# ziniuwan/maed

Hardware: AMD Instinct MI355X
Metric: video-clips/sec (BxT frames) train step (higher is better)
Workload: dtype bf16

## Files before the change

### include/maed_hip.h

```cpp
#ifndef MAED_HIP_H
#define MAED_HIP_H

#include <stddef.h>
#include <stdint.h>

#ifdef __cplusplus
extern "C" {
#endif

typedef enum { MAED_F32 = 0, MAED_BF16 = 1,
               MAED_F32X3 = 2, MAED_F32X6 = 3,
               MAED_F32X1 = 4 } maed_dtype;

typedef enum {
    MAED_OK = 0,
    MAED_ERR_ARG = -1,
    MAED_ERR_SHAPE = -2,
    MAED_ERR_ALIGN = -3,
    MAED_ERR_LAUNCH = -4,
    MAED_ERR_UNSUPPORTED = -5
} maed_status;

typedef enum {
    MAED_EPI_STORE = 0,
    MAED_EPI_GELU = 1,
    MAED_EPI_RESID_F32 = 2,
    MAED_EPI_MUL_DGELU = 3,
    MAED_EPI_ATOMIC_F32 = 4,
    MAED_EPI_STORE_F32 = 5,
    MAED_EPI_TANH = 6,
    MAED_EPI_ADD = 7
} maed_epilogue;

typedef enum { MAED_IMPL_AUTO = 0, MAED_IMPL_VALU = 1, MAED_IMPL_MFMA = 2,
               MAED_IMPL_MFMA_GLDS1 = 3, MAED_IMPL_MFMA_GLDS2 = 4,
               MAED_IMPL_MFMA_LONG = 5,
               MAED_IMPL_MFMA_256 = 6,
               MAED_IMPL_X1 = 9,
               MAED_IMPL_MFMA_SK = 10,
               MAED_IMPL_X3 = 7, MAED_IMPL_X6 = 8
} maed_impl;

const char* maed_last_error(void);
int maed_version(void);

typedef enum {
    MAED_OPT_F32_MATMUL = 0,
    MAED_OPT_SIDE_STREAM = 1,
    MAED_OPT_TN_TARGET_WGS = 2,
    MAED_OPT_ABLATE = 3,
    MAED_OPT_GN_BWD_ONEPASS = 4,
    MAED_OPT_F32_BWD_X1 = 5,
    MAED_OPT_ST_FUSED = 6,
    MAED_OPT_CONV3X3_ROWS_WGS = 7,
    MAED_OPT_STEM_WGRAD_WGS = 8,
    MAED_OPT_LBS_FRAMES = 9,
    MAED_OPT_TN_DMA = 10,
    MAED_OPT_X3_PLANES = 11,
    MAED_OPT_X3_PLANES_LN = 12,
    MAED_OPT_SK = 13,
    MAED_OPT_SK_GRID = 14,
    MAED_OPT_TN_SK = 15,
    MAED_OPT_CONV3X3_NARROW_WGS = 16,
    MAED_OPT_CONV3X3_FRAME = 17,
    MAED_OPT_COUNT
} maed_option;
int maed_init(int device);
int maed_device_faults(void);
int maed_device_faults_clear(void);
int maed_set_option(int key, int value);
int maed_get_option(int key);

int maed_layernorm_fwd(const float* x, int64_t x_row_stride, const float* gamma, const float* beta,
                       void* y, int dtype, float* mean, float* rstd,
                       int64_t rows, int C, float eps, void* stream);
int maed_layernorm_bwd(const void* dy, int dtype, const float* x, int64_t x_row_stride,
                       const float* gamma, const float* mean, const float* rstd,
                       const float* dres_in, float* dx_out, void* dx_twin, float* dgamma, float* dbeta,
                       int64_t rows, int C, void* stream);

int maed_gemm_nt(const void* A, int64_t lda, const void* B, int64_t ldb,
                 int64_t M, int64_t N, int64_t K, int dtype, int epilogue,
                 const float* bias, void* out, int64_t ldo, void* out2,
                 const void* aux, int64_t ldaux, int splitk, int impl, void* stream);

int maed_gemm_nt_planes(const void* a_hi, const void* a_lo, int64_t lda, const void* b_hi, const void* b_lo, int64_t ldb, int64_t M, int64_t N, int64_t K,
                        int epilogue, const float* bias, void* out, int64_t ldo, void* out2_bf16, const void* aux, int64_t ldaux, void* out_hi, void* out_lo,
                        int variant, void* stream);
int maed_split_planes(const float* x, void* hi, void* lo, int64_t n, void* stream);

int maed_gemm_tn_wgrad(const void* Y, int64_t ldy, const void* X, int64_t ldx, int64_t M, int N, int K,
                       float* dW, int64_t ldw, float* dbias, int dtype, void* stream);

int maed_transpose_cast(const void* in, int in_dtype, int64_t ldi, int64_t M, int64_t N,
                        void* out_t, int64_t ldt, void* out_c, int64_t ldc, float* colsum,
                        int dtype, void* stream);

int maed_attn_spatial_fwd(const void* qkv, void* o, float* lse, int F, int P, int H, float scale,
                          int dtype, int impl, void* stream);
int maed_attn_spatial_bwd(const void* qkv, const void* o, const void* d_o, const float* lse,
                          void* dqkv, int accumulate, int F, int P, int H, float scale,
                          int dtype, int impl, void* stream);

int maed_attn_temporal_fwd(const void* qkv, void* o, float* lse, int F, int P, int H, int T,
                           float scale, int dtype, void* stream);
int maed_attn_temporal_bwd(const void* qkv, const void* o, const void* d_o, const float* lse,
                           void* dqkv, int accumulate, int F, int P, int H, int T, float scale,
                           int dtype, void* stream);

int maed_st_colmean(const void* x_s, const void* x_t, void* means, float* ws, int F, int P, int C, int dtype, void* stream);
int maed_st_mix_fwd(const void* x_s, const void* x_t, const float* logits, void* mix,
                    int F, int P, int C, int dtype, void* stream);
int maed_st_mix_bwd_reduce(const void* dmix, const void* x_s, const void* x_t, const float* logits,
                           void* dlogits, float* ws, int F, int P, int C, int dtype, void* stream);
int maed_st_mix_bwd_apply(const void* dmix, const float* logits, const void* dmeans, void* dx_s, void* dx_t,
                          int F, int P, int C, int dtype, void* stream);
int maed_st_fused_supported(int P, int C, int dtype);
int maed_st_fused_fwd(const void* x_s, const void* x_t, const void* w_ts, const float* b_ts, void* means, float* logits, void* mix,
                      uint32_t* sync, float* ex, int F, int P, int C, int dtype, void* stream);
int maed_st_fused_bwd(const void* dmix, const void* x_s, const void* x_t, const float* logits, const void* wt_ts, void* dlogits, void* dx_s,
                      void* dx_t, uint32_t* sync, float* ex, int F, int P, int C, int dtype, void* stream);


int maed_embed_add_fwd(const void* patch, int dtype, const float* cls, const float* pos, const float* temp,
                       float* tokens, int F, int P, int C, int T, void* stream);
int maed_embed_add_bwd(const float* dtokens, void* dpatch, int dtype, float* dpos, float* dtemp, int F, int P, int C, int T, void* stream);

int maed_dropout(const float* x, float* y, int64_t n, float p, uint64_t seed, void* stream);
typedef struct { float lr, bias_corr1, bias_corr2, reserved0; uint64_t seed; uint64_t reserved1; } maed_train_state;
int maed_dropout_dev(const float* x, float* y, int64_t n, float p, const maed_train_state* state, uint64_t call_id, void* stream);
int maed_tanh_bwd(const float* dy, const void* y, void* dx, int64_t n, int dtype, void* stream);

typedef struct {
    int F, P, C, H, T, hidden;
    int dtype;
    int impl;
    float eps;
} maed_block_dims;

typedef struct {
    const float *ln1_g, *ln1_b, *ln2_g, *ln2_b;
    const void *w_qkv, *w_ts, *w_proj, *w_fc1, *w_fc2;
    const float *b_qkv, *b_ts, *b_proj, *b_fc1, *b_fc2;
    const void *wt_qkv, *wt_ts, *wt_proj, *wt_fc1, *wt_fc2;
} maed_block_params;

typedef struct {
    float *ln1_g, *ln1_b, *ln2_g, *ln2_b;
    float *w_qkv, *w_ts, *w_proj, *w_fc1, *w_fc2;
    float *b_qkv, *b_ts, *b_proj, *b_fc1, *b_fc2;
} maed_block_grads;

size_t maed_ste_block_saved_bytes(const maed_block_dims* d);
size_t maed_ste_block_scratch_bytes(const maed_block_dims* d);
int maed_ste_block_fwd(const maed_block_dims* d, const maed_block_params* p, const float* x_in,
                       float* x_out, void* saved, void* stream);
size_t maed_ste_block_twin_work_bytes(const maed_block_dims* d);
int maed_ste_block_fwd_twin(const maed_block_dims* d, const maed_block_params* p, const float* x_in, float* x_out, void* saved_bf16, void* work_f32, int work_slot,
                            void* stream);
int maed_ste_block_twin_join(void* stream);
int maed_ste_block_infer(const maed_block_dims* d, const maed_block_params* p, const float* x_in,
                         float* x_out, void* work, void* stream);
int maed_ste_block_bwd(const maed_block_dims* d, const maed_block_params* p, const maed_block_grads* g,
                       const float* x_in, const float* dx_out, float* dx_in, void* saved, void* scratch,
                       const void* dx_out_twin, void* dx_in_twin, void* stream);

int maed_stream_fence(void* from_stream, void* to_stream);

int maed_prof_enable(int on);
int maed_prof_ntags(void);
int maed_prof_collect(double* ms_total_host, int* count_host);
int maed_prof_flops(double* flops_host);
int maed_prof_records(int tag, double* us_host, double* flops_host, double* bytes_host, int cap);

int maed_ktd_chain_fwd(const float* base, const float* w_anc, float* pose, int F, void* stream);

int maed_rot6d_pose_fwd(const float* pose6d, float* rotmat, float* angle_axis, int64_t n_joints, void* stream);

typedef struct {
    const float* v_template;
    const float* shapedirs;
    const float* posedirs;
    const float* J_template;
    const float* J_shapedirs;
    const float* lbs_weights;
    const int32_t* parents;
} maed_smpl_params;
int maed_smpl_lbs_fwd(const maed_smpl_params* sp, const float* betas, const float* rotmat,
                      float* verts, float* joints24, float* scratch_A, float* v_posed, int F, void* stream);
int maed_joint_regress_fwd(const float* Jreg, int J, const float* verts, float* out, int F, void* stream);
int maed_joint_regress_csr_fwd(const int32_t* rowptr, const int32_t* cols, const float* vals, int J, const float* verts, float* out, int F, void* stream);
int maed_smpl_joints_project_fwd(const float* joints24, const float* verts, const int64_t* extra_vertex_ids,
                                 const float* extra9, const int64_t* joint_map, const float* cam,
                                 const float* joints_override, int Jo, float* kp3d, float* kp2d, int F, void* stream);


int maed_smpl_joints_project_bwd(const float* kp3d, const float* cam, const int64_t* joint_map, const float* d_kp3d,
                                 const float* d_kp2d, const float* d_cam_in, int64_t cam_in_stride, float* d_joints24,
                                 float* d_extra21, float* d_extra9, float* d_cam, int F, void* stream);
int maed_smpl_skin_bwd(const maed_smpl_params* sp, const float* A, const float* v_posed, const float* d_verts,
                       const float* d_extra21, const int64_t* extra_vertex_ids, const float* d_extra9, const float* Jextra,
                       float* d_vposed, float* dA, int F, void* stream);
int maed_smpl_skin_bwd_sparse(const maed_smpl_params* sp, const float* A, const float* v_posed, const int32_t* active, int n_active,
                              const float* d_extra21, const int64_t* extra_vertex_ids, const float* d_extra9, const float* Jextra,
                              float* d_vposed_active, float* dA, int F, void* stream);
int maed_smpl_chain_bwd(const maed_smpl_params* sp, const float* betas, const float* rotmat, const float* dA,
                        const float* d_joints24, const float* dpf_dbeta, const float* d_rotmat_in, const float* d_betas_in,
                        int64_t betas_in_stride, float* d_rotmat, float* d_betas, int F, void* stream);
int maed_rot6d_pose_bwd(const float* pose6d, const float* d_rotmat, const float* d_aa, int64_t aa_stride,
                        float* d_pose6d, int64_t n_joints, void* stream);
int maed_ktd_chain_bwd(const float* pose, const float* w_anc, const float* d_pose, const float* d_shape, const float* d_cam,
                       float* d_out, int64_t ld_out, float* d_w_anc, float* d_b_feat, int F, void* stream);
#define MAED_KTD_W_ANC 3420
typedef struct { const float* w[26]; const float* b[26]; float* gw[26]; float* gb[26]; } maed_ktd_ptrs;
int maed_ktd_pack(const maed_ktd_ptrs* t, int hidden, float* w_feat, float* b_feat, float* w_anc, void* stream);
int maed_ktd_unpack_add(const maed_ktd_ptrs* t, int hidden, const float* d_w_feat, const float* d_b_feat, const float* d_w_anc, void* stream);

typedef struct { float w_kp2d, w_kp3d, w_pose, w_shape, w_norm; } maed_loss_weights;
int maed_loss_fwd_bwd(const float* pred_kp2d, const float* gt_kp2d, int M2, const float* pred_kp3d, const float* gt_kp3d,
                      const float* pred_theta, const float* gt_theta, const uint8_t* w_smpl, int M3,
                      const maed_loss_weights* w, float* losses, float* d_kp2d, float* d_kp3d, float* d_theta,
                      double* partials, void* stream);

int maed_loss_accl_fwd_bwd(const float* pred_kp3d, const float* gt_kp3d, int N, int T, float weight, double* loss, float* d_kp3d, void* stream);

typedef struct {
    const float* w;
    float* gw;
    const void* gout;
    int64_t dst_off;
    int64_t dst_t_off;
    int32_t O, I, KHW, fstart;
    int32_t gout_f32;
    int32_t pad_;
} maed_ws_conv;
int maed_weight_std_fwd(const void* conv_table, int n_convs, int n_filters, void* out, int dtype, float* stats, float eps, int transpose_tiles, void* stream);
int maed_weight_std_bwd(const void* conv_table, int n_convs, int n_filters, int dtype, const float* stats, float eps, void* stream);
int maed_groupnorm_fwd(const void* x, const void* residual, const float* gamma, const float* beta, void* y, double* sums,
                       uint8_t* relu_mask, int N, int HW, int C, float eps, int relu, int dtype, int sums_zeroed, void* stream);
int maed_groupnorm_fwd_twin(const void* x, const void* residual, const float* gamma, const float* beta, void* y, double* sums,
                            uint8_t* relu_mask, int N, int HW, int C, float eps, int relu, int sums_zeroed, void* twin_x, void* twin_y, void* stream);
#define MAED_GN_SYNC_WORDS 80
int maed_groupnorm_bwd(const void* x, const uint8_t* relu_mask, const void* dy, const double* sums, const float* gamma, const float* beta,
                       void* dx, void* dres, float* dgamma, float* dbeta, float* ab_scratch, int N, int HW, int C, float eps,
                       int relu, int dtype, int ab_zeroed, uint32_t* frame_sync, void* aux_stream, void* stream);
typedef struct { const float* ab; float* dgamma; float* dbeta; int N; int C; } maed_gn_affine_item;
int maed_gn_affine_grad_batch(const maed_gn_affine_item* items, int count, void* stream);

int maed_maxpool3s2_same_fwd(const void* x, void* y, uint8_t* idx, int N, int H, int W, int C, int dtype, void* stream);
int maed_maxpool3s2_same_bwd(const void* dy, const uint8_t* idx, void* dx, int N, int H, int W, int C, int dtype, void* stream);

int maed_stem_input(const float* x, void* y, int N, int C, int H, int W, int pad_top, int pad_bottom, int pad_left, int pad_right, int c_stride, int dtype,
                    void* stream);

int maed_conv3x3_wgrad_rows64_scratch_floats(int F, int H, int W, int Cin, int Cout);
int maed_conv3x3_wgrad_rows64(const void* dy, const void* x, float* dW, void* scratch, int F, int H, int W, int dtype, void* stream);

int maed_stem7x7s2_supported(int H, int W);
int maed_stem7x7s2_fwd(const void* xp, const void* w, void* wimg, void* y, double* gn_sums, int F, int H, int W, int dtype, void* stream);
int maed_stem7x7s2_wgrad_scratch_floats(int F, int H, int W);
int maed_stem7x7s2_wgrad(const void* dy, const void* xp, float* dW, void* scratch, int F, int H, int W, int dtype, void* stream);

int maed_subsample2_fwd(const void* x, void* y, int F, int H, int W, int C, int dtype, void* stream);
int maed_subsample2_bwd(const void* g, void* dx, int F, int H, int W, int C, int dtype, void* stream);

typedef struct { const float* src; void* dst_c; void* dst_t; int32_t rows, cols, tile0, tiles_n; } maed_wt_entry;
int maed_weight_refresh(const void* table, int n_entries, int n_tiles, int dtype, void* stream);

int maed_adam_step(float* p, const float* g, float* m, float* v, void* shadow_bf16, int64_t n,
                   float lr, float beta1, float beta2, float eps, float weight_decay,
                   float bias_corr1, float bias_corr2, float gscale, void* stream);
int maed_adam_step_dev(float* p, const float* g, float* m, float* v, void* shadow_bf16, int64_t n, const maed_train_state* state,
                       float beta1, float beta2, float eps, float weight_decay, float gscale, void* stream);

#define MAED_COMM_ID_BYTES 128
int maed_comm_load(const char* librccl_path);
int maed_comm_unique_id(void* id128);
int maed_comm_init(int rank, int world, const void* unique_id);
int maed_comm_allreduce_async(void* buf, size_t n, int dtype, void* compute_stream);
int maed_comm_wait(void* compute_stream);
int maed_comm_world(void);
int maed_comm_destroy(void);

int maed_conv3x3_fwd(const void* x, const void* w_taps, const void* zero_page, void* y, int F, int H, int W, int Cin, int Cout,
                     int stride, int pad_top, int pad_left, int Ho, int Wo, const void* add, int w_layout, int dtype, double* gn_sums,
                     void* stream);

int maed_conv1x1_fwd(const void* x, int64_t ldx, const void* w, int64_t ldw, int64_t M, int Cout, int Cin, void* y, int64_t ldy, int hw,
                     double* gn_sums, int dtype, void* stream);

int maed_conv3x3_s2_dgrad(const void* dy, const void* wt_image, const void* zero_page, void* dx, int F, int H, int W, int Cin, int Cout,
                          int pad_top, int pad_left, int Ho, int Wo, int dtype, void* stream);
int maed_conv3x3_s2_tables(void* tapmask, int* rowtab, int F, int H, int W, int pad_top, int pad_left, int Ho, int Wo, void* stream);
int maed_conv3x3_s2_wgrad(const void* dy, const void* x, const void* tapmask, const int* rowtab, const void* zero_page, float* dW, int F, int H, int W,
                          int Cin, int Cout, int Ho, int Wo, int dtype, void* stream);
int maed_conv3x3_tapmask(void* tapmask, int F, int H, int W, void* stream);
int maed_conv3x3_wgrad(const void* dy, const void* x, const void* tapmask, const void* zero_page, float* dW, int F, int H, int W, int Cin,
                       int Cout, int dtype, void* stream);

int maed_eval_pose_errors(const float* pred, const float* target, int N, int J, float* mpjpe, float* pa_mpjpe,
                          float* pred_centred, float* target_centred, void* stream);
int maed_similarity_transform(const float* S1, const float* S2, int N, int J, float* S1_hat, void* stream);
int maed_eval_accel(const float* joints, const float* joints_gt, int N, int J, float* out, void* stream);
int maed_eval_vertex_error(const float* pred_verts, const float* target_verts, int N, int V, float* out, void* stream);

size_t maed_clip_preprocess_workspace(int F, int H, int W);
int maed_clip_preprocess(const uint8_t* src, int64_t src_bytes, const int32_t* frame_i, const float* frame_minv, const int32_t* clip_i,
                         const float* clip_f, int F, int N, int H, int W, const float* norm_host, int has_contrast, int form, float* out,
                         void* workspace, size_t workspace_bytes, void* stream);

#ifdef __cplusplus
}
#endif
#endif
```

### maed_amd/_lib.py

```python
import ctypes as C
import os

HERE = os.path.dirname(os.path.abspath(__file__))
LIB_PATH = os.environ.get("MAED_HIP_LIB") or os.path.join(HERE, "libmaed_hip.so")

F32, BF16 = 0, 1
F32X3, F32X6, F32X1 = 2, 3, 4
EPI_STORE, EPI_GELU, EPI_RESID_F32, EPI_MUL_DGELU, EPI_ATOMIC_F32, EPI_STORE_F32, EPI_TANH, EPI_ADD = range(8)
IMPL_AUTO, IMPL_VALU, IMPL_MFMA = 0, 1, 2
IMPL_MFMA_256 = 6
IMPL_MFMA_LONG = 5
IMPL_MFMA_SK = 10
IMPL_X3, IMPL_X6, IMPL_X1 = 7, 8, 9
(OPT_F32_MATMUL, OPT_SIDE_STREAM, OPT_TN_TARGET_WGS, OPT_ABLATE, OPT_GN_BWD_ONEPASS, OPT_F32_BWD_X1, OPT_ST_FUSED, OPT_CONV3X3_ROWS_WGS, OPT_STEM_WGRAD_WGS,
 OPT_LBS_FRAMES, OPT_TN_DMA, OPT_X3_PLANES, OPT_X3_PLANES_LN, OPT_SK, OPT_SK_GRID, OPT_TN_SK, OPT_CONV3X3_NARROW_WGS, OPT_CONV3X3_FRAME) = range(18)

vp, i64, i32, f32 = C.c_void_p, C.c_int64, C.c_int, C.c_float


class GnAffineItem(C.Structure):
    _fields_ = [("ab", C.c_void_p), ("dgamma", C.c_void_p), ("dbeta", C.c_void_p), ("N", C.c_int), ("C", C.c_int)]


class BlockDims(C.Structure):
    _fields_ = [("F", i32), ("P", i32), ("C", i32), ("H", i32), ("T", i32), ("hidden", i32),
                ("dtype", i32), ("impl", i32), ("eps", f32)]


_PARAM_FIELDS = ["ln1_g", "ln1_b", "ln2_g", "ln2_b", "w_qkv", "w_ts", "w_proj", "w_fc1", "w_fc2",
                 "b_qkv", "b_ts", "b_proj", "b_fc1", "b_fc2", "wt_qkv", "wt_ts", "wt_proj", "wt_fc1", "wt_fc2"]
_GRAD_FIELDS = _PARAM_FIELDS[:14]


class BlockParams(C.Structure):
    _fields_ = [(n, vp) for n in _PARAM_FIELDS]


class BlockGrads(C.Structure):
    _fields_ = [(n, vp) for n in _GRAD_FIELDS]


class SmplParams(C.Structure):
    _fields_ = [(n, vp) for n in ["v_template", "shapedirs", "posedirs", "J_template", "J_shapedirs", "lbs_weights", "parents"]]


class KtdPtrs(C.Structure):
    _fields_ = [("w", vp * 26), ("b", vp * 26), ("gw", vp * 26), ("gb", vp * 26)]


class LossWeights(C.Structure):
    _fields_ = [(n, f32) for n in ["w_kp2d", "w_kp3d", "w_pose", "w_shape", "w_norm"]]


KTD_W_ANC = 3420

SIGNATURES = {
    "maed_last_error": (C.c_char_p, []),
    "maed_version": (i32, []),
    "maed_init": (i32, [i32]),
    "maed_device_faults": (i32, []),
    "maed_device_faults_clear": (i32, []),
    "maed_set_option": (i32, [i32, i32]),
    "maed_get_option": (i32, [i32]),
    "maed_layernorm_fwd": (i32, [vp, i64, vp, vp, vp, i32, vp, vp, i64, i32, f32, vp]),
    "maed_layernorm_bwd": (i32, [vp, i32, vp, i64, vp, vp, vp, vp, vp, vp, vp, vp, i64, i32, vp]),
    "maed_gemm_tn_wgrad": (i32, [vp, i64, vp, i64, i64, i32, i32, vp, i64, vp, i32, vp]),
    "maed_gemm_nt": (i32, [vp, i64, vp, i64, i64, i64, i64, i32, i32, vp, vp, i64, vp, vp, i64, i32, i32, vp]),
    "maed_transpose_cast": (i32, [vp, i32, i64, i64, i64, vp, i64, vp, i64, vp, i32, vp]),
    "maed_attn_spatial_fwd": (i32, [vp, vp, vp, i32, i32, i32, f32, i32, i32, vp]),
    "maed_attn_spatial_bwd": (i32, [vp, vp, vp, vp, vp, i32, i32, i32, i32, f32, i32, i32, vp]),
    "maed_attn_temporal_fwd": (i32, [vp, vp, vp, i32, i32, i32, i32, f32, i32, vp]),
    "maed_attn_temporal_bwd": (i32, [vp, vp, vp, vp, vp, i32, i32, i32, i32, i32, f32, i32, vp]),
    "maed_st_colmean": (i32, [vp, vp, vp, vp, i32, i32, i32, i32, vp]),
    "maed_st_mix_fwd": (i32, [vp, vp, vp, vp, i32, i32, i32, i32, vp]),
    "maed_st_mix_bwd_reduce": (i32, [vp, vp, vp, vp, vp, vp, i32, i32, i32, i32, vp]),
    "maed_st_mix_bwd_apply": (i32, [vp, vp, vp, vp, vp, i32, i32, i32, i32, vp]),
    "maed_st_fused_supported": (i32, [i32, i32, i32]),
    "maed_st_fused_fwd": (i32, [vp, vp, vp, vp, vp, vp, vp, vp, vp, i32, i32, i32, i32, vp]),
    "maed_st_fused_bwd": (i32, [vp, vp, vp, vp, vp, vp, vp, vp, vp, vp, i32, i32, i32, i32, vp]),
    "maed_embed_add_fwd": (i32, [vp, i32, vp, vp, vp, vp, i32, i32, i32, i32, vp]),
    "maed_embed_add_bwd": (i32, [vp, vp, i32, vp, vp, i32, i32, i32, i32, vp]),
    "maed_ste_block_saved_bytes": (C.c_size_t, [C.POINTER(BlockDims)]),
    "maed_ste_block_scratch_bytes": (C.c_size_t, [C.POINTER(BlockDims)]),
    "maed_gemm_nt_planes": (i32, [vp, vp, i64, vp, vp, i64, i64, i64, i64, i32, vp, vp, i64, vp, vp, i64, vp, vp, i32, vp]),
    "maed_split_planes": (i32, [vp, vp, vp, i64, vp]),
    "maed_ste_block_twin_work_bytes": (C.c_size_t, [C.POINTER(BlockDims)]),
    "maed_ste_block_fwd_twin": (i32, [C.POINTER(BlockDims), C.POINTER(BlockParams), vp, vp, vp, vp, i32, vp]),
    "maed_ste_block_twin_join": (i32, [vp]),
    "maed_ste_block_fwd": (i32, [C.POINTER(BlockDims), C.POINTER(BlockParams), vp, vp, vp, vp]),
    "maed_ste_block_infer": (i32, [C.POINTER(BlockDims), C.POINTER(BlockParams), vp, vp, vp, vp]),
    "maed_ste_block_bwd": (i32, [C.POINTER(BlockDims), C.POINTER(BlockParams), C.POINTER(BlockGrads), vp, vp, vp, vp, vp, vp, vp, vp]),
    "maed_loss_accl_fwd_bwd": (i32, [vp, vp, i32, i32, f32, vp, vp, vp]),
    "maed_dropout": (i32, [vp, vp, i64, f32, C.c_uint64, vp]),
    "maed_dropout_dev": (i32, [vp, vp, i64, f32, vp, C.c_uint64, vp]),
    "maed_tanh_bwd": (i32, [vp, vp, vp, i64, i32, vp]),
    "maed_stream_fence": (i32, [vp, vp]),
    "maed_prof_enable": (i32, [i32]),
    "maed_prof_ntags": (i32, []),
    "maed_prof_collect": (i32, [C.POINTER(C.c_double), C.POINTER(i32)]),
    "maed_prof_flops": (i32, [C.POINTER(C.c_double)]),
    "maed_prof_records": (i32, [i32, C.POINTER(C.c_double), C.POINTER(C.c_double), C.POINTER(C.c_double), i32]),
    "maed_ktd_chain_fwd": (i32, [vp, vp, vp, i32, vp]),
    "maed_rot6d_pose_fwd": (i32, [vp, vp, vp, i64, vp]),
    "maed_smpl_lbs_fwd": (i32, [C.POINTER(SmplParams), vp, vp, vp, vp, vp, vp, i32, vp]),
    "maed_joint_regress_fwd": (i32, [vp, i32, vp, vp, i32, vp]),
    "maed_joint_regress_csr_fwd": (i32, [vp, vp, vp, i32, vp, vp, i32, vp]),
    "maed_smpl_joints_project_fwd": (i32, [vp, vp, vp, vp, vp, vp, vp, i32, vp, vp, i32, vp]),
    "maed_smpl_joints_project_bwd": (i32, [vp, vp, vp, vp, vp, vp, i64, vp, vp, vp, vp, i32, vp]),
    "maed_smpl_skin_bwd": (i32, [C.POINTER(SmplParams), vp, vp, vp, vp, vp, vp, vp, vp, vp, i32, vp]),
    "maed_smpl_skin_bwd_sparse": (i32, [C.POINTER(SmplParams), vp, vp, vp, i32, vp, vp, vp, vp, vp, vp, i32, vp]),
    "maed_smpl_chain_bwd": (i32, [C.POINTER(SmplParams), vp, vp, vp, vp, vp, vp, vp, i64, vp, vp, i32, vp]),
    "maed_rot6d_pose_bwd": (i32, [vp, vp, vp, i64, vp, i64, vp]),
    "maed_ktd_chain_bwd": (i32, [vp, vp, vp, vp, vp, vp, i64, vp, vp, i32, vp]),
    "maed_ktd_pack": (i32, [C.POINTER(KtdPtrs), i32, vp, vp, vp, vp]),
    "maed_ktd_unpack_add": (i32, [C.POINTER(KtdPtrs), i32, vp, vp, vp, vp]),
    "maed_loss_fwd_bwd": (i32, [vp, vp, i32, vp, vp, vp, vp, vp, i32, C.POINTER(LossWeights), vp, vp, vp, vp, vp, vp]),
    "maed_weight_std_fwd": (i32, [vp, i32, i32, vp, i32, vp, f32, i32, vp]),
    "maed_weight_std_bwd": (i32, [vp, i32, i32, i32, vp, f32, vp]),
    "maed_groupnorm_fwd": (i32, [vp, vp, vp, vp, vp, vp, vp, i32, i32, i32, f32, i32, i32, i32, vp]),
    "maed_groupnorm_fwd_twin": (i32, [vp, vp, vp, vp, vp, vp, vp, i32, i32, i32, f32, i32, i32, vp, vp, vp]),
    "maed_groupnorm_bwd": (i32, [vp, vp, vp, vp, vp, vp, vp, vp, vp, vp, vp, i32, i32, i32, f32, i32, i32, i32, vp, vp, vp]),
    "maed_gn_affine_grad_batch": (i32, [vp, i32, vp]),
    "maed_comm_load": (i32, [C.c_char_p]),
    "maed_comm_unique_id": (i32, [vp]),
    "maed_comm_init": (i32, [i32, i32, vp]),
    "maed_comm_allreduce_async": (i32, [vp, C.c_size_t, i32, vp]),
    "maed_comm_wait": (i32, [vp]),
    "maed_comm_world": (i32, []),
    "maed_comm_destroy": (i32, []),
    "maed_conv3x3_fwd": (i32, [vp, vp, vp, vp, i32, i32, i32, i32, i32, i32, i32, i32, i32, i32, vp, i32, i32, vp, vp]),
    "maed_conv1x1_fwd": (i32, [vp, i64, vp, i64, i64, i32, i32, vp, i64, i32, vp, i32, vp]),
    "maed_conv3x3_tapmask": (i32, [vp, i32, i32, i32, vp]),
    "maed_conv3x3_s2_dgrad": (i32, [vp, vp, vp, vp, i32, i32, i32, i32, i32, i32, i32, i32, i32, i32, vp]),
    "maed_conv3x3_s2_tables": (i32, [vp, vp, i32, i32, i32, i32, i32, i32, i32, vp]),
    "maed_conv3x3_s2_wgrad": (i32, [vp, vp, vp, vp, vp, vp, i32, i32, i32, i32, i32, i32, i32, i32, vp]),
    "maed_conv3x3_wgrad": (i32, [vp, vp, vp, vp, vp, i32, i32, i32, i32, i32, i32, vp]),
    "maed_eval_pose_errors": (i32, [vp, vp, i32, i32, vp, vp, vp, vp, vp]),
    "maed_similarity_transform": (i32, [vp, vp, i32, i32, vp, vp]),
    "maed_eval_accel": (i32, [vp, vp, i32, i32, vp, vp]),
    "maed_eval_vertex_error": (i32, [vp, vp, i32, i32, vp, vp]),
    "maed_maxpool3s2_same_fwd": (i32, [vp, vp, vp, i32, i32, i32, i32, i32, vp]),
    "maed_maxpool3s2_same_bwd": (i32, [vp, vp, vp, i32, i32, i32, i32, i32, vp]),
    "maed_stem_input": (i32, [vp, vp, i32, i32, i32, i32, i32, i32, i32, i32, i32, i32, vp]),
    "maed_conv3x3_wgrad_rows64_scratch_floats": (i32, [i32, i32, i32, i32, i32]),
    "maed_conv3x3_wgrad_rows64": (i32, [vp, vp, vp, vp, i32, i32, i32, i32, vp]),
    "maed_stem7x7s2_supported": (i32, [i32, i32]),
    "maed_stem7x7s2_fwd": (i32, [vp, vp, vp, vp, vp, i32, i32, i32, i32, vp]),
    "maed_stem7x7s2_wgrad_scratch_floats": (i32, [i32, i32, i32]),
    "maed_stem7x7s2_wgrad": (i32, [vp, vp, vp, vp, i32, i32, i32, i32, vp]),
    "maed_subsample2_fwd": (i32, [vp, vp, i32, i32, i32, i32, i32, vp]),
    "maed_subsample2_bwd": (i32, [vp, vp, i32, i32, i32, i32, i32, vp]),
    "maed_weight_refresh": (i32, [vp, i32, i32, i32, vp]),
    "maed_adam_step": (i32, [vp, vp, vp, vp, vp, i64, f32, f32, f32, f32, f32, f32, f32, f32, vp]),
    "maed_adam_step_dev": (i32, [vp, vp, vp, vp, vp, i64, vp, f32, f32, f32, f32, f32, vp]),
    "maed_clip_preprocess_workspace": (C.c_size_t, [i32, i32, i32]),
    "maed_clip_preprocess": (i32, [vp, i64, vp, vp, vp, vp, i32, i32, i32, i32, C.POINTER(f32), i32, i32, vp, vp, C.c_size_t, vp]),
}

_lib = None
_init_pending = False


class MaedHipError(RuntimeError):
    pass


def lib():
    global _lib, _init_pending
    if _lib is None:
        if not os.path.exists(LIB_PATH):
            raise MaedHipError(f"{LIB_PATH} is missing: build it with `python -m maed_amd.build` "
                               "(hipcc --offload-arch=gfx950).  maed_amd has no non-HIP fallback.")
        handle = C.CDLL(LIB_PATH)
        for name, (res, args) in SIGNATURES.items():
            fn = getattr(handle, name)
            fn.restype, fn.argtypes = res, args
        _lib = handle
        apply_options(handle)
        _init_pending = True
    if _init_pending:
        import torch
        if torch.cuda.is_available() and torch.cuda.is_initialized():
            _init_pending = False
            check(_lib.maed_init(torch.cuda.current_device()), "maed_init")
    return _lib


_OPTIONS = {
    OPT_F32_MATMUL: {"exact": 0, "0": 0, "bf16x3": 1, "1": 1, "bf16x6": 2, "2": 2}[os.environ.get("MAED_F32_MATMUL", "exact")],
    OPT_SIDE_STREAM: int(os.environ.get("MAED_WGRAD_SIDE_STREAM", "1") == "1"),
    OPT_TN_TARGET_WGS: int(os.environ.get("MAED_TN_TARGET_WGS", "0")),
    OPT_ABLATE: int(os.environ.get("MAED_GEMM_ABLATE", "0")),
    OPT_F32_BWD_X1: int(os.environ.get("MAED_F32_BWD", "") == "bf16x1"),
    OPT_ST_FUSED: int(os.environ.get("MAED_ST_FUSED", "1")),
    OPT_GN_BWD_ONEPASS: int(os.environ.get("MAED_GN_BWD_ONEPASS", "1")),
    OPT_CONV3X3_ROWS_WGS: 0 if os.environ.get("MAED_CONV3X3_WGRAD_ROWS", "1") == "0" else int(os.environ.get("MAED_CONV3X3_ROWS_WGS", "256")),
    OPT_STEM_WGRAD_WGS: int(os.environ.get("MAED_STEM_WGS", "512")),
    OPT_LBS_FRAMES: int(os.environ.get("MAED_LBS_FB", "0")),
    OPT_TN_DMA: int(os.environ.get("MAED_TN_DMA", "1")),
    OPT_X3_PLANES: int(os.environ.get("MAED_X3_PLANES", "6")),
    OPT_SK: int(os.environ.get("MAED_SK", "1")),
    OPT_SK_GRID: int(os.environ.get("MAED_SK_GRID", "0")),
    OPT_CONV3X3_FRAME: int(os.environ.get("MAED_CONV3X3_FRAME", "1")),
    OPT_CONV3X3_NARROW_WGS: int(os.environ.get("MAED_CONV3X3_NARROW_WGS", "0")),
    OPT_TN_SK: int(os.environ.get("MAED_TN_SK", "1")),
    OPT_X3_PLANES_LN: int(os.environ.get("MAED_X3_PLANES_LN", "0")),
}


def apply_options(handle):
    for k, v in _OPTIONS.items():
        if handle.maed_set_option(k, v) != 0:
            raise MaedHipError(f"maed_set_option({k}, {v}) failed")


def set_option(key, value):
    _OPTIONS[key] = int(value)
    if _lib is not None:
        check(_lib.maed_set_option(key, int(value)), "set_option")


def get_option(key):
    return _OPTIONS[key]


def check(rc, what=""):
    if rc != 0:
        msg = lib().maed_last_error().decode("utf-8", "replace")
        raise MaedHipError(f"{what or 'libmaed_hip'} failed with status {rc}: {msg}")


def device_faults():
    return 0 if _lib is None else int(_lib.maed_device_faults())


def loaded_path():
    return LIB_PATH if _lib is not None else None
```

### maed_amd/csrc/attn_long.hip

```cpp
#include "attn_mfma.cuh"

#define D HEAD_DIM

namespace {

constexpr int LT = 64;
constexpr int LVLD = LT + 4;
constexpr int WG_ROWS = 128;

__device__ __forceinline__ int long_xcd_remap(int bid, int nwg) {
    const int xcd = bid & 7, q = nwg >> 3, r = nwg & 7;
    const int base = (xcd < r) ? xcd * (q + 1) : r * (q + 1) + (xcd - r) * q;
    return base + (bid >> 3);
}

struct TileRegs { uint4 a, b; };

__device__ __forceinline__ uint4 tile_load1(const bf16* src, int64_t ld, int r0, int L, int idx) {
    int row = r0 + (idx >> 3);
    if (row > L - 1) row = L - 1;
    return *reinterpret_cast<const uint4*>(src + (int64_t)row * ld + (idx & 7) * 8);
}
__device__ __forceinline__ void tile_load(TileRegs& t, const bf16* src, int64_t ld, int r0, int L, int tid) {
    t.a = tile_load1(src, ld, r0, L, tid);
    t.b = tile_load1(src, ld, r0, L, tid + 256);
}

__device__ __forceinline__ void tile_store1(const uint4 v, unsigned short* rows, unsigned short* tr, int idx) {
    const int p = idx >> 3, c8 = (idx & 7) * 8;
    if (rows) *reinterpret_cast<uint4*>(rows + p * KLD + c8) = v;
    if (tr) {
        tr[(c8 + 0) * LVLD + p] = (unsigned short)(v.x & 0xffffu); tr[(c8 + 1) * LVLD + p] = (unsigned short)(v.x >> 16);
        tr[(c8 + 2) * LVLD + p] = (unsigned short)(v.y & 0xffffu); tr[(c8 + 3) * LVLD + p] = (unsigned short)(v.y >> 16);
        tr[(c8 + 4) * LVLD + p] = (unsigned short)(v.z & 0xffffu); tr[(c8 + 5) * LVLD + p] = (unsigned short)(v.z >> 16);
        tr[(c8 + 6) * LVLD + p] = (unsigned short)(v.w & 0xffffu); tr[(c8 + 7) * LVLD + p] = (unsigned short)(v.w >> 16);
    }
}
__device__ __forceinline__ void tile_store(const TileRegs& t, unsigned short* rows, unsigned short* tr, int tid) {
    tile_store1(t.a, rows, tr, tid);
    tile_store1(t.b, rows, tr, tid + 256);
}

__global__ __launch_bounds__(256, 4) void attn_long_fwd_mfma(const bf16* __restrict__ qkv, bf16* __restrict__ o, float* __restrict__ lse,
                                                          int L, int H, int ntile, float scale_log2e) {
    __shared__ __attribute__((aligned(16))) unsigned short Ks[LT * KLD];
    __shared__ __attribute__((aligned(16))) unsigned short Vs[LT * KLD];
    const int bid = long_xcd_remap(blockIdx.x, gridDim.x);
    const int item = bid / ntile, tile = bid - item * ntile;
    const int f = item / H, h = item - f * H, C = H * D;
    const int64_t ld = 3 * (int64_t)C;
    const bf16* base = qkv + (int64_t)f * L * ld + h * D;
    const int tid = threadIdx.x, lane = tid & 63, wave = tid >> 6, l31 = lane & 31, hi = lane >> 5;
    const int q0 = tile * WG_ROWS + wave * 32, q = q0 + l31;
    const bool active = q0 < L;
    const int qc = q < L ? q : L - 1;
    bf16x8_t qf[4];
#pragma unroll
    for (int t = 0; t < 4; ++t) qf[t] = *reinterpret_cast<const bf16x8_t*>(base + (int64_t)qc * ld + t * 16 + hi * 8);
    f32x16_t oacc[2];
#pragma unroll
    for (int r = 0; r < 16; ++r) { oacc[0][r] = 0.f; oacc[1][r] = 0.f; }
    float m = -INFINITY, l = 0.f;
    const int nkt = (L + LT - 1) / LT;
    TileRegs kreg, vreg;
    tile_load(kreg, base + C, ld, 0, L, tid);
    tile_load(vreg, base + 2 * C, ld, 0, L, tid);
    for (int kt = 0; kt < nkt; ++kt) {
        __syncthreads();
        tile_store(kreg, Ks, nullptr, tid);
        tile_store(vreg, Vs, nullptr, tid);
        __syncthreads();
        if (kt + 1 < nkt) {
            tile_load(kreg, base + C, ld, (kt + 1) * LT, L, tid);
            tile_load(vreg, base + 2 * C, ld, (kt + 1) * LT, L, tid);
        }
        if (!active) continue;
#pragma unroll
        for (int sub = 0; sub < 2; ++sub) {
            const int k0 = kt * LT + sub * 32;
            if (k0 >= L) break;
            f32x16_t s;
#pragma unroll
            for (int r = 0; r < 16; ++r) s[r] = 0.f;
            const unsigned short* kp = Ks + (sub * 32 + l31) * KLD + hi * 8;
#pragma unroll
            for (int t = 0; t < 4; ++t)
                s = __builtin_amdgcn_mfma_f32_32x32x16_bf16(*reinterpret_cast<const bf16x8_t*>(kp + t * 16), qf[t], s, 0, 0, 0);
            if (k0 + 32 > L) {
#pragma unroll
                for (int r = 0; r < 16; ++r) s[r] = (k0 + (r & 3) + 8 * (r >> 2) + 4 * hi < L) ? s[r] : -INFINITY;
            }
            float mt = s[0];
#pragma unroll
            for (int r = 1; r < 16; ++r) mt = fmaxf(mt, s[r]);
            mt = fmaxf(mt, __shfl_xor(mt, 32, 64)) * scale_log2e;
            const bool grow = mt > m + 8.0f;
            if (__any(grow)) {
                const float mn = grow ? mt : m;
                const float alpha = __builtin_amdgcn_exp2f(m - mn);
                l *= alpha;
                m = mn;
#pragma unroll
                for (int r = 0; r < 16; ++r) { oacc[0][r] *= alpha; oacc[1][r] *= alpha; }
            }
            float ps = 0.f;
#pragma unroll
            for (int r = 0; r < 16; ++r) { s[r] = __builtin_amdgcn_exp2f(fmaf(s[r], scale_log2e, -m)); ps += s[r]; }
            l += ps;
#pragma unroll
            for (int st = 0; st < 2; ++st) {
                const bf16x8_t pf = pack_frag(s, st);
#pragma unroll
                for (int et = 0; et < 2; ++et)
                    oacc[et] = __builtin_amdgcn_mfma_f32_32x32x16_bf16(lds_frag_tr_rm(Vs, sub * 32 + 16 * st, et * 32, lane), pf, oacc[et], 0, 0, 0);
            }
        }
    }
    l += __shfl_xor(l, 32, 64);
    __syncthreads();
    if (active) {
        const float inv = 1.f / l;
#pragma unroll
        for (int r = 0; r < 16; ++r) { oacc[0][r] *= inv; oacc[1][r] *= inv; }
        store_tile_lines((wave < 2 ? Ks : Vs) + (wave & 1) * 2048, o + ((int64_t)f * L + q0) * C + h * D, C, L - q0, oacc, lane, 0);
    }
    if (active && q < L) {
        if (hi == 0) lse[((int64_t)f * H + h) * L + q] = (m + log2f(l)) * 0.69314718055994530942f;
    }
}

__global__ __launch_bounds__(256, 3) void attn_long_bwd_dq_mfma(const bf16* __restrict__ qkv, const bf16* __restrict__ o, const bf16* __restrict__ d_o,
                                                             const float* __restrict__ lse, bf16* __restrict__ dqkv, int accumulate, int L, int H,
                                                             int ntile, float scale) {
    __shared__ __attribute__((aligned(16))) unsigned short Ks[LT * KLD];
    __shared__ __attribute__((aligned(16))) unsigned short Vs[LT * KLD];
    const int bid = long_xcd_remap(blockIdx.x, gridDim.x);
    const int item = bid / ntile, tile = bid - item * ntile;
    const int f = item / H, h = item - f * H, C = H * D;
    const int64_t ld = 3 * (int64_t)C;
    const bf16* base = qkv + (int64_t)f * L * ld + h * D;
    const int tid = threadIdx.x, lane = tid & 63, wave = tid >> 6, l31 = lane & 31, hi = lane >> 5;
    const int q0 = tile * WG_ROWS + wave * 32, q = q0 + l31;
    const bool active = q0 < L;
    const int qc = q < L ? q : L - 1;
    const bf16* orow = o + ((int64_t)f * L + qc) * C + h * D;
    const bf16* dorow = d_o + ((int64_t)f * L + qc) * C + h * D;
    bf16x8_t qf[4], dof[4];
    float Dq = 0.f;
#pragma unroll
    for (int t = 0; t < 4; ++t) {
        qf[t] = *reinterpret_cast<const bf16x8_t*>(base + (int64_t)qc * ld + t * 16 + hi * 8);
        dof[t] = *reinterpret_cast<const bf16x8_t*>(dorow + t * 16 + hi * 8);
        float a[8], b[8];
        ld8(dorow + t * 16 + hi * 8, a); ld8(orow + t * 16 + hi * 8, b);
#pragma unroll
        for (int j = 0; j < 8; ++j) Dq = fmaf(a[j], b[j], Dq);
    }
    Dq += __shfl_xor(Dq, 32, 64);
    const float l2e = 1.44269504088896340736f;
    const float L2 = lse[((int64_t)f * H + h) * L + qc] * l2e, sl2e = scale * l2e;
    f32x16_t dq[2];
#pragma unroll
    for (int r = 0; r < 16; ++r) { dq[0][r] = 0.f; dq[1][r] = 0.f; }
    const int nkt = (L + LT - 1) / LT;
    TileRegs kreg, vreg;
    tile_load(kreg, base + C, ld, 0, L, tid);
    tile_load(vreg, base + 2 * C, ld, 0, L, tid);
    for (int kt = 0; kt < nkt; ++kt) {
        __syncthreads();
        tile_store(kreg, Ks, nullptr, tid);
        tile_store(vreg, Vs, nullptr, tid);
        __syncthreads();
        if (kt + 1 < nkt) {
            tile_load(kreg, base + C, ld, (kt + 1) * LT, L, tid);
            tile_load(vreg, base + 2 * C, ld, (kt + 1) * LT, L, tid);
        }
        if (!active) continue;
#pragma unroll
        for (int sub = 0; sub < 2; ++sub) {
            const int k0 = kt * LT + sub * 32;
            if (k0 >= L) break;
            f32x16_t s, dp;
#pragma unroll
            for (int r = 0; r < 16; ++r) { s[r] = 0.f; dp[r] = -Dq; }
            const int off = (sub * 32 + l31) * KLD + hi * 8;
#pragma unroll
            for (int t = 0; t < 4; ++t) {
                s = __builtin_amdgcn_mfma_f32_32x32x16_bf16(*reinterpret_cast<const bf16x8_t*>(Ks + off + t * 16), qf[t], s, 0, 0, 0);
                dp = __builtin_amdgcn_mfma_f32_32x32x16_bf16(*reinterpret_cast<const bf16x8_t*>(Vs + off + t * 16), dof[t], dp, 0, 0, 0);
            }
#pragma unroll
            for (int r = 0; r < 16; ++r) s[r] = __builtin_amdgcn_exp2f(fmaf(s[r], sl2e, -L2)) * dp[r];
            if (k0 + 32 > L) {
#pragma unroll
                for (int r = 0; r < 16; ++r) s[r] = (k0 + (r & 3) + 8 * (r >> 2) + 4 * hi < L) ? s[r] : 0.f;
            }
#pragma unroll
            for (int st = 0; st < 2; ++st) {
                const bf16x8_t dsf = pack_frag(s, st);
#pragma unroll
                for (int et = 0; et < 2; ++et)
                    dq[et] = __builtin_amdgcn_mfma_f32_32x32x16_bf16(lds_frag_tr_rm(Ks, sub * 32 + 16 * st, et * 32, lane), dsf, dq[et], 0, 0, 0);
            }
        }
    }
#pragma unroll
    for (int r = 0; r < 16; ++r) { dq[0][r] *= scale; dq[1][r] *= scale; }
    __syncthreads();
    if (active) store_tile_lines((wave < 2 ? Ks : Vs) + (wave & 1) * 2048, dqkv + ((int64_t)f * L + q0) * ld + h * D, ld, L - q0, dq, lane, accumulate);
}

__global__ __launch_bounds__(256, 2) void attn_long_bwd_dkv_mfma(const bf16* __restrict__ qkv, const bf16* __restrict__ o, const bf16* __restrict__ d_o,
                                                              const float* __restrict__ lse, bf16* __restrict__ dqkv, int accumulate, int L, int H,
                                                              int ntile, float scale) {
    __shared__ __attribute__((aligned(16))) unsigned short Qs[LT * KLD];
    __shared__ __attribute__((aligned(16))) unsigned short dOs[LT * KLD];
    __shared__ float Ls[LT], Ds[LT];
    const int bid = long_xcd_remap(blockIdx.x, gridDim.x);
    const int item = bid / ntile, tile = bid - item * ntile;
    const int f = item / H, h = item - f * H, C = H * D;
    const int64_t ld = 3 * (int64_t)C;
    const bf16* base = qkv + (int64_t)f * L * ld + h * D;
    const bf16* obase = o + (int64_t)f * L * C + h * D;
    const bf16* dobase = d_o + (int64_t)f * L * C + h * D;
    const int tid = threadIdx.x, lane = tid & 63, wave = tid >> 6, l31 = lane & 31, hi = lane >> 5;
    const int k0w = tile * WG_ROWS + wave * 32, k = k0w + l31;
    const bool active = k0w < L;
    const int kc = k < L ? k : L - 1;
    bf16x8_t kf[4], vf[4];
#pragma unroll
    for (int t = 0; t < 4; ++t) {
        kf[t] = *reinterpret_cast<const bf16x8_t*>(base + C + (int64_t)kc * ld + t * 16 + hi * 8);
        vf[t] = *reinterpret_cast<const bf16x8_t*>(base + 2 * C + (int64_t)kc * ld + t * 16 + hi * 8);
    }
    const float l2e = 1.44269504088896340736f, sl2e = scale * l2e;
    f32x16_t dk[2], dv[2];
#pragma unroll
    for (int r = 0; r < 16; ++r) { dk[0][r] = 0.f; dk[1][r] = 0.f; dv[0][r] = 0.f; dv[1][r] = 0.f; }
    const int nqt = (L + LT - 1) / LT;
    TileRegs qreg, doreg, oreg;
    float lreg = 0.f;
    auto load_stats = [&](int qt_) {
        tile_load(oreg, obase, C, qt_ * LT, L, tid);
        if (tid < LT) { int qi = qt_ * LT + tid; if (qi > L - 1) qi = L - 1; lreg = lse[((int64_t)f * H + h) * L + qi] * l2e; }
    };
    auto chunk_dot = [](const uint4& a, const uint4& b) {
        const uint32_t x[4] = {a.x, a.y, a.z, a.w}, y[4] = {b.x, b.y, b.z, b.w};
        float d = 0.f;
#pragma unroll
        for (int j = 0; j < 4; ++j) {
            d = fmaf(__uint_as_float(x[j] << 16), __uint_as_float(y[j] << 16), d);
            d = fmaf(__uint_as_float(x[j] & 0xffff0000u), __uint_as_float(y[j] & 0xffff0000u), d);
        }
        return d;
    };
    tile_load(qreg, base, ld, 0, L, tid);
    tile_load(doreg, dobase, C, 0, L, tid);
    load_stats(0);
    for (int qt = 0; qt < nqt; ++qt) {
        __syncthreads();
        tile_store(qreg, Qs, nullptr, tid);
        tile_store(doreg, dOs, nullptr, tid);
        {
            float d0 = chunk_dot(doreg.a, oreg.a), d1 = chunk_dot(doreg.b, oreg.b);
#pragma unroll
            for (int m = 1; m < 8; m <<= 1) { d0 += __shfl_xor(d0, m, 64); d1 += __shfl_xor(d1, m, 64); }
            if ((tid & 7) == 0) { Ds[tid >> 3] = d0; Ds[32 + (tid >> 3)] = d1; }
            if (tid < LT) Ls[tid] = lreg;
        }
        __syncthreads();
        if (qt + 1 < nqt) {
            tile_load(qreg, base, ld, (qt + 1) * LT, L, tid);
            tile_load(doreg, dobase, C, (qt + 1) * LT, L, tid);
            load_stats(qt + 1);
        }
        if (!active) continue;
#pragma unroll
        for (int sub = 0; sub < 2; ++sub) {
            const int q0 = qt * LT + sub * 32;
            if (q0 >= L) break;
            f32x16_t s, dp;
#pragma unroll
            for (int r = 0; r < 16; ++r) { s[r] = 0.f; dp[r] = -Ds[sub * 32 + (r & 3) + 8 * (r >> 2) + 4 * hi]; }
            const int off = (sub * 32 + l31) * KLD + hi * 8;
#pragma unroll
            for (int t = 0; t < 4; ++t) {
                s = __builtin_amdgcn_mfma_f32_32x32x16_bf16(*reinterpret_cast<const bf16x8_t*>(Qs + off + t * 16), kf[t], s, 0, 0, 0);
                dp = __builtin_amdgcn_mfma_f32_32x32x16_bf16(*reinterpret_cast<const bf16x8_t*>(dOs + off + t * 16), vf[t], dp, 0, 0, 0);
            }
#pragma unroll
            for (int r = 0; r < 16; ++r) {
                const int ql = sub * 32 + (r & 3) + 8 * (r >> 2) + 4 * hi;
                s[r] = __builtin_amdgcn_exp2f(fmaf(s[r], sl2e, -Ls[ql]));
                dp[r] *= s[r];
            }
            if (q0 + 32 > L) {
#pragma unroll
                for (int r = 0; r < 16; ++r) {
                    const bool ok = q0 + (r & 3) + 8 * (r >> 2) + 4 * hi < L;
                    s[r] = ok ? s[r] : 0.f; dp[r] = ok ? dp[r] : 0.f;
                }
            }
#pragma unroll
            for (int st = 0; st < 2; ++st) {
                const bf16x8_t pf = pack_frag(s, st), dsf = pack_frag(dp, st);
#pragma unroll
                for (int et = 0; et < 2; ++et) {
                    dv[et] = __builtin_amdgcn_mfma_f32_32x32x16_bf16(lds_frag_tr_rm(dOs, sub * 32 + 16 * st, et * 32, lane), pf, dv[et], 0, 0, 0);
                    dk[et] = __builtin_amdgcn_mfma_f32_32x32x16_bf16(lds_frag_tr_rm(Qs, sub * 32 + 16 * st, et * 32, lane), dsf, dk[et], 0, 0, 0);
                }
            }
        }
    }
#pragma unroll
    for (int r = 0; r < 16; ++r) { dk[0][r] *= scale; dk[1][r] *= scale; }
    __syncthreads();
    if (active) {
        unsigned short* patch = (wave < 2 ? Qs : dOs) + (wave & 1) * 2048;
        bf16* drow0 = dqkv + ((int64_t)f * L + k0w) * ld + h * D;
        store_tile_lines(patch, drow0 + C, ld, L - k0w, dk, lane, accumulate);
        store_tile_lines(patch, drow0 + 2 * C, ld, L - k0w, dv, lane, accumulate);
    }
}

constexpr int VT = 64;
constexpr int VLDF = 65;
constexpr int VROWS = 256;

template <typename T>
__device__ __forceinline__ void stage_tile_f32(float* dst, const T* src, int64_t ld, int r0, int L, int tid) {
    for (int idx = tid; idx < VT * (D / 4); idx += 256) {
        const int p = idx / (D / 4), c = (idx % (D / 4)) * 4;
        int row = r0 + p;
        if (row > L - 1) row = L - 1;
        float v[4];
        ld4(src + (int64_t)row * ld + c, v);
#pragma unroll
        for (int j = 0; j < 4; ++j) dst[p * VLDF + c + j] = v[j];
    }
}

template <typename T>
__global__ __launch_bounds__(256) void attn_long_fwd_valu(const T* __restrict__ qkv, T* __restrict__ o, float* __restrict__ lse, int L, int H,
                                                          int ntile, float scale) {
    __shared__ float Ks[VT * VLDF], Vs[VT * VLDF];
    const int item = blockIdx.x / ntile, tile = blockIdx.x - item * ntile;
    const int f = item / H, h = item - f * H, C = H * D;
    const int64_t ld = 3 * (int64_t)C;
    const T* base = qkv + (int64_t)f * L * ld + h * D;
    const int tid = threadIdx.x, q = tile * VROWS + tid;
    const int qc = q < L ? q : L - 1;
    float qv[D], acc[D];
#pragma unroll
    for (int c = 0; c < D; c += 4) { float v[4]; ld4(base + (int64_t)qc * ld + c, v); qv[c] = v[0]; qv[c + 1] = v[1]; qv[c + 2] = v[2]; qv[c + 3] = v[3]; }
#pragma unroll
    for (int c = 0; c < D; ++c) acc[c] = 0.f;
    float m = -INFINITY, l = 0.f;
    for (int k0 = 0; k0 < L; k0 += VT) {
        __syncthreads();
        stage_tile_f32(Ks, base + C, ld, k0, L, tid);
        stage_tile_f32(Vs, base + 2 * C, ld, k0, L, tid);
        __syncthreads();
        const int kn = (L - k0 < VT) ? L - k0 : VT;
        for (int k = 0; k < kn; ++k) {
            float s = 0.f;
#pragma unroll
            for (int c = 0; c < D; ++c) s = fmaf(qv[c], Ks[k * VLDF + c], s);
            s *= scale;
            const float mn = fmaxf(m, s);
            const float a = __expf(m - mn), p = __expf(s - mn);
            l = l * a + p;
#pragma unroll
            for (int c = 0; c < D; ++c) acc[c] = fmaf(p, Vs[k * VLDF + c], acc[c] * a);
            m = mn;
        }
    }
    if (q < L) {
        const float inv = 1.f / l;
        T* orow = o + ((int64_t)f * L + q) * C + h * D;
#pragma unroll
        for (int c = 0; c < D; c += 4) { float v[4] = {acc[c] * inv, acc[c + 1] * inv, acc[c + 2] * inv, acc[c + 3] * inv}; st4(orow + c, v); }
        lse[((int64_t)f * H + h) * L + q] = m + __logf(l);
    }
}

template <typename T>
__device__ __forceinline__ void store_row_acc(T* dst, const float (&acc)[D], int accumulate) {
#pragma unroll
    for (int c = 0; c < D; c += 4) {
        float v[4] = {acc[c], acc[c + 1], acc[c + 2], acc[c + 3]};
        if (accumulate) { float old[4]; ld4(dst + c, old); v[0] += old[0]; v[1] += old[1]; v[2] += old[2]; v[3] += old[3]; }
        st4(dst + c, v);
    }
}

template <typename T>
__global__ __launch_bounds__(256) void attn_long_bwd_dq_valu(const T* __restrict__ qkv, const T* __restrict__ o, const T* __restrict__ d_o,
                                                             const float* __restrict__ lse, T* __restrict__ dqkv, int accumulate, int L, int H,
                                                             int ntile, float scale) {
    __shared__ float Ks[VT * VLDF], Vs[VT * VLDF];
    const int item = blockIdx.x / ntile, tile = blockIdx.x - item * ntile;
    const int f = item / H, h = item - f * H, C = H * D;
    const int64_t ld = 3 * (int64_t)C;
    const T* base = qkv + (int64_t)f * L * ld + h * D;
    const int tid = threadIdx.x, q = tile * VROWS + tid;
    const int qc = q < L ? q : L - 1;
    const T* orow = o + ((int64_t)f * L + qc) * C + h * D;
    const T* dorow = d_o + ((int64_t)f * L + qc) * C + h * D;
    float qv[D], dov[D], dq[D];
    float Dq = 0.f;
#pragma unroll
    for (int c = 0; c < D; c += 4) {
        float v[4], w[4], u[4];
        ld4(base + (int64_t)qc * ld + c, v); ld4(dorow + c, w); ld4(orow + c, u);
#pragma unroll
        for (int j = 0; j < 4; ++j) { qv[c + j] = v[j]; dov[c + j] = w[j]; Dq = fmaf(w[j], u[j], Dq); dq[c + j] = 0.f; }
    }
    const float Lq = lse[((int64_t)f * H + h) * L + qc];
    for (int k0 = 0; k0 < L; k0 += VT) {
        __syncthreads();
        stage_tile_f32(Ks, base + C, ld, k0, L, tid);
        stage_tile_f32(Vs, base + 2 * C, ld, k0, L, tid);
        __syncthreads();
        const int kn = (L - k0 < VT) ? L - k0 : VT;
        for (int k = 0; k < kn; ++k) {
            float s = 0.f, dp = 0.f;
#pragma unroll
            for (int c = 0; c < D; ++c) { s = fmaf(qv[c], Ks[k * VLDF + c], s); dp = fmaf(dov[c], Vs[k * VLDF + c], dp); }
            const float ds = __expf(s * scale - Lq) * (dp - Dq) * scale;
#pragma unroll
            for (int c = 0; c < D; ++c) dq[c] = fmaf(ds, Ks[k * VLDF + c], dq[c]);
        }
    }
    if (q < L) store_row_acc(dqkv + ((int64_t)f * L + q) * ld + h * D, dq, accumulate);
}

template <typename T>
__global__ __launch_bounds__(256) void attn_long_bwd_dkv_valu(const T* __restrict__ qkv, const T* __restrict__ o, const T* __restrict__ d_o,
                                                              const float* __restrict__ lse, T* __restrict__ dqkv, int accumulate, int L, int H,
                                                              int ntile, float scale) {
    __shared__ float Qs[VT * VLDF], dOs[VT * VLDF], Ls[VT], Ds[VT];
    const int item = blockIdx.x / ntile, tile = blockIdx.x - item * ntile;
    const int f = item / H, h = item - f * H, C = H * D;
    const int64_t ld = 3 * (int64_t)C;
    const T* base = qkv + (int64_t)f * L * ld + h * D;
    const T* obase = o + (int64_t)f * L * C + h * D;
    const T* dobase = d_o + (int64_t)f * L * C + h * D;
    const int tid = threadIdx.x, k = tile * VROWS + tid;
    const int kc = k < L ? k : L - 1;
    float kv[D], vv[D], acc[D];
#pragma unroll
    for (int c = 0; c < D; c += 4) {
        float a[4], b[4];
        ld4(base + C + (int64_t)kc * ld + c, a); ld4(base + 2 * C + (int64_t)kc * ld + c, b);
#pragma unroll
        for (int j = 0; j < 4; ++j) { kv[c + j] = a[j]; vv[c + j] = b[j]; }
    }
    for (int sweep = 0; sweep < 2; ++sweep) {
#pragma unroll
        for (int c = 0; c < D; ++c) acc[c] = 0.f;
        for (int q0 = 0; q0 < L; q0 += VT) {
            __syncthreads();
            stage_tile_f32(Qs, base, ld, q0, L, tid);
            stage_tile_f32(dOs, dobase, (int64_t)C, q0, L, tid);
            if (tid < VT) {
                int qi = q0 + tid;
                if (qi > L - 1) qi = L - 1;
                float dsum = 0.f;
#pragma unroll
                for (int c = 0; c < D; c += 4) {
                    float a[4], b[4];
                    ld4(dobase + (int64_t)qi * C + c, a); ld4(obase + (int64_t)qi * C + c, b);
#pragma unroll
                    for (int j = 0; j < 4; ++j) dsum = fmaf(a[j], b[j], dsum);
                }
                Ds[tid] = dsum;
                Ls[tid] = lse[((int64_t)f * H + h) * L + qi];
            }
            __syncthreads();
            const int qn = (L - q0 < VT) ? L - q0 : VT;
            for (int qq = 0; qq < qn; ++qq) {
                float s = 0.f, dp = 0.f;
#pragma unroll
                for (int c = 0; c < D; ++c) { s = fmaf(Qs[qq * VLDF + c], kv[c], s); dp = fmaf(dOs[qq * VLDF + c], vv[c], dp); }
                const float p = __expf(s * scale - Ls[qq]);
                const float w = sweep == 0 ? p : p * (dp - Ds[qq]) * scale;
                const float* src = sweep == 0 ? dOs + qq * VLDF : Qs + qq * VLDF;
#pragma unroll
                for (int c = 0; c < D; ++c) acc[c] = fmaf(w, src[c], acc[c]);
            }
        }
        if (k < L) store_row_acc(dqkv + ((int64_t)f * L + k) * ld + (sweep == 0 ? 2 * C : C) + h * D, acc, accumulate);
    }
}

}

int maed_attn_long_fwd_launch(const void* qkv, void* o, float* lse, int F, int L, int H, float scale, hipStream_t s) {
    const int ntile = (L + WG_ROWS - 1) / WG_ROWS;
    MAED_CHECK_ARG((int64_t)F * H * ntile < (1ll << 31), MAED_ERR_SHAPE, "attn_long_fwd: grid too large");
    hipLaunchKernelGGL(attn_long_fwd_mfma, dim3((unsigned)(F * H * ntile)), dim3(256), 0, s, (const bf16*)qkv, (bf16*)o, lse, L, H, ntile,
                       scale * 1.44269504088896340736f);
    MAED_CHECK_LAUNCH("attn_long_fwd");
    return MAED_OK;
}

int maed_attn_long_bwd_launch(const void* qkv, const void* o, const void* d_o, const float* lse, void* dqkv, int accumulate, int F, int L, int H,
                              float scale, hipStream_t s) {
    const int ntile = (L + WG_ROWS - 1) / WG_ROWS;
    MAED_CHECK_ARG((int64_t)F * H * ntile < (1ll << 31), MAED_ERR_SHAPE, "attn_long_bwd: grid too large");
    const dim3 grid((unsigned)(F * H * ntile));
    hipLaunchKernelGGL(attn_long_bwd_dq_mfma, grid, dim3(256), 0, s, (const bf16*)qkv, (const bf16*)o, (const bf16*)d_o, lse, (bf16*)dqkv, accumulate,
                       L, H, ntile, scale);
    hipLaunchKernelGGL(attn_long_bwd_dkv_mfma, grid, dim3(256), 0, s, (const bf16*)qkv, (const bf16*)o, (const bf16*)d_o, lse, (bf16*)dqkv, accumulate,
                       L, H, ntile, scale);
    MAED_CHECK_LAUNCH("attn_long_bwd");
    return MAED_OK;
}

int maed_attn_long_fwd_valu_launch(const void* qkv, void* o, float* lse, int F, int L, int H, float scale, int dtype, hipStream_t s) {
    const int ntile = (L + VROWS - 1) / VROWS;
    const dim3 grid((unsigned)(F * H * ntile));
    MAED_DISPATCH_DTYPE(dtype, T, hipLaunchKernelGGL((attn_long_fwd_valu<T>), grid, dim3(256), 0, s, (const T*)qkv, (T*)o, lse, L, H, ntile, scale));
    MAED_CHECK_LAUNCH("attn_long_fwd(valu)");
    return MAED_OK;
}

int maed_attn_long_bwd_valu_launch(const void* qkv, const void* o, const void* d_o, const float* lse, void* dqkv, int accumulate, int F, int L,
                                   int H, float scale, int dtype, hipStream_t s) {
    const int ntile = (L + VROWS - 1) / VROWS;
    const dim3 grid((unsigned)(F * H * ntile));
    MAED_DISPATCH_DTYPE(dtype, T, {
        hipLaunchKernelGGL((attn_long_bwd_dq_valu<T>), grid, dim3(256), 0, s, (const T*)qkv, (const T*)o, (const T*)d_o, lse, (T*)dqkv, accumulate, L, H,
                           ntile, scale);
        hipLaunchKernelGGL((attn_long_bwd_dkv_valu<T>), grid, dim3(256), 0, s, (const T*)qkv, (const T*)o, (const T*)d_o, lse, (T*)dqkv, accumulate, L, H,
                           ntile, scale);
    });
    MAED_CHECK_LAUNCH("attn_long_bwd(valu)");
    return MAED_OK;
}
```

### maed_amd/csrc/attn_temporal.hip

```cpp
#include "common.cuh"
#include "attn_mfma.cuh"
#include "gemm_x3.h"
#include <stdlib.h>

#define D HEAD_DIM

template <typename T>
__device__ __forceinline__ void load_row(const T* p, float (&v)[D]) {
#pragma unroll
    for (int c = 0; c < D; c += 8) {
        float t[8];
        ld8(p + c, t);
#pragma unroll
        for (int j = 0; j < 8; ++j) v[c + j] = t[j];
    }
}
template <typename T>
__device__ __forceinline__ float dot_row(const T* p, const float (&v)[D]) {
    float s = 0.f;
#pragma unroll
    for (int c = 0; c < D; c += 8) {
        float t[8];
        ld8(p + c, t);
#pragma unroll
        for (int j = 0; j < 8; ++j) s = fmaf(v[c + j], t[j], s);
    }
    return s;
}
template <typename T>
__device__ __forceinline__ void axpy_row(const T* p, float a, float (&acc)[D]) {
#pragma unroll
    for (int c = 0; c < D; c += 8) {
        float t[8];
        ld8(p + c, t);
#pragma unroll
        for (int j = 0; j < 8; ++j) acc[c + j] = fmaf(a, t[j], acc[c + j]);
    }
}
template <typename T>
__device__ __forceinline__ void store_row(T* p, const float (&v)[D], float mul, int accumulate) {
#pragma unroll
    for (int c = 0; c < D; c += 8) {
        float t[8];
#pragma unroll
        for (int j = 0; j < 8; ++j) t[j] = v[c + j] * mul;
        if (accumulate) { float o[8]; ld8(p + c, o);
#pragma unroll
            for (int j = 0; j < 8; ++j) t[j] += o[j]; }
        st8(p + c, t);
    }
}

template <typename T>
__global__ __launch_bounds__(256) void attn_tm_fwd_kernel(const T* __restrict__ qkv, T* __restrict__ o, float* __restrict__ lse,
                                                          int64_t total, int P, int H, int Tn, float scale) {
    const int64_t gid = (int64_t)blockIdx.x * 256 + threadIdx.x;
    if (gid >= total) return;
    const int t = (int)(gid % Tn); int64_t r = gid / Tn;
    const int p = (int)(r % P); r /= P;
    const int h = (int)(r % H); const int64_t n = r / H;
    const int C = H * D; const int64_t ld = 3 * (int64_t)C;
    const int64_t f = n * Tn + t;
    const T* qrow = qkv + (f * P + p) * ld + h * D;
    float qv[D], acc[D];
    load_row(qrow, qv);
#pragma unroll
    for (int c = 0; c < D; ++c) acc[c] = 0.f;
    float m = -INFINITY, l = 0.f;
    for (int t2 = 0; t2 < Tn; ++t2) {
        const T* krow = qkv + ((n * Tn + t2) * P + p) * ld + C + h * D;
        const float s = dot_row(krow, qv) * scale;
        const float mn = fmaxf(m, s);
        const float a = __expf(m - mn), pr = __expf(s - mn);
        l = l * a + pr;
#pragma unroll
        for (int c = 0; c < D; ++c) acc[c] *= a;
        axpy_row(krow + C, pr, acc);
        m = mn;
    }
    store_row(o + (f * P + p) * C + h * D, acc, 1.f / l, 0);
    lse[(f * H + h) * P + p] = m + __logf(l);
}

template <typename T>
__global__ __launch_bounds__(256) void attn_tm_bwd_kernel(const T* __restrict__ qkv, const T* __restrict__ o, const T* __restrict__ d_o,
                                                          const float* __restrict__ lse, T* __restrict__ dqkv, int accumulate,
                                                          int64_t total, int P, int H, int Tn, float scale) {
    const int64_t gid = (int64_t)blockIdx.x * 256 + threadIdx.x;
    if (gid >= total) return;
    const int t = (int)(gid % Tn); int64_t r = gid / Tn;
    const int p = (int)(r % P); r /= P;
    const int h = (int)(r % H); const int64_t n = r / H;
    const int C = H * D; const int64_t ld = 3 * (int64_t)C;
    const int64_t f = n * Tn + t;
    const int64_t row = f * P + p;
    float a[D], b[D], acc[D];
    load_row(qkv + row * ld + h * D, a);
    load_row(d_o + row * C + h * D, b);
    const float Dq = dot_row(o + row * C + h * D, b);
    const float L = lse[(f * H + h) * P + p];
#pragma unroll
    for (int c = 0; c < D; ++c) acc[c] = 0.f;
    for (int t2 = 0; t2 < Tn; ++t2) {
        const T* krow = qkv + ((n * Tn + t2) * P + p) * ld + C + h * D;
        const float pr = __expf(dot_row(krow, a) * scale - L);
        const float ds = pr * (dot_row(krow + C, b) - Dq) * scale;
        axpy_row(krow, ds, acc);
    }
    store_row(dqkv + row * ld + h * D, acc, 1.f, accumulate);
    load_row(qkv + row * ld + C + h * D, a);
#pragma unroll
    for (int c = 0; c < D; ++c) acc[c] = 0.f;
    for (int t1 = 0; t1 < Tn; ++t1) {
        const int64_t row1 = (n * Tn + t1) * P + p;
        const float pr = __expf(dot_row(qkv + row1 * ld + h * D, a) * scale - lse[((n * Tn + t1) * H + h) * P + p]);
        axpy_row(d_o + row1 * C + h * D, pr, acc);
    }
    store_row(dqkv + row * ld + 2 * C + h * D, acc, 1.f, accumulate);
    const T* vrow = qkv + row * ld + 2 * C + h * D;
#pragma unroll
    for (int c = 0; c < D; ++c) acc[c] = 0.f;
    for (int t1 = 0; t1 < Tn; ++t1) {
        const int64_t row1 = (n * Tn + t1) * P + p;
        const T* q1 = qkv + row1 * ld + h * D;
        const T* do1 = d_o + row1 * C + h * D;
        const float pr = __expf(dot_row(q1, a) * scale - lse[((n * Tn + t1) * H + h) * P + p]);
        float d1[D];
        load_row(do1, d1);
        const float dp = dot_row(vrow, d1);
        const float D1 = dot_row(o + row1 * C + h * D, d1);
        const float ds = pr * (dp - D1) * scale;
        axpy_row(q1, ds, acc);
    }
    store_row(dqkv + row * ld + C + h * D, acc, 1.f, accumulate);
}

template <typename T> struct RowGeom { static constexpr int RS = D * (int)sizeof(T); };

template <typename T>
__device__ __forceinline__ T* lds_row(char* base, int r, int gp) { return reinterpret_cast<T*>(base + (size_t)r * RowGeom<T>::RS + gp * 16); }

template <typename T>
__device__ __forceinline__ void stage_group_rows(char* dst, const T* src_base, int64_t ld, int64_t n, int Tn, int P, int p0, int GP, int nthr) {
    constexpr int CH = RowGeom<T>::RS / 16;
    constexpr int EPC = 16 / (int)sizeof(T);
    const int c = threadIdx.x % CH, rstep = nthr / CH;
    int r = threadIdx.x / CH;
    int gp = r / Tn, t = r - gp * Tn;
    for (; r < GP * Tn; r += rstep) {
        int p = p0 + gp; if (p > P - 1) p = P - 1;
        const uint4 v = *reinterpret_cast<const uint4*>(src_base + ((n * Tn + t) * P + p) * ld + c * EPC);
        *reinterpret_cast<uint4*>(reinterpret_cast<char*>(lds_row<T>(dst, r, gp)) + c * 16) = v;
        t += rstep;
        while (t >= Tn) { t -= Tn; ++gp; }
    }
}

template <typename T>
__global__ __launch_bounds__(256) void attn_tm_fwd_lds(const T* __restrict__ qkv, T* __restrict__ o, float* __restrict__ lse,
                                                       int P, int H, int Tn, int GP, float scale) {
    MAED_DYN_SHARED(char, sm);
    const int C = H * D; const int64_t ld = 3 * (int64_t)C;
    const int chunks = (P + GP - 1) / GP;
    const int pc = blockIdx.x % chunks; int r0 = blockIdx.x / chunks;
    const int h = r0 % H; const int64_t n = r0 / H;
    const int p0 = pc * GP, nthr = GP * Tn;
    const size_t arr = (size_t)GP * Tn * RowGeom<T>::RS + GP * 16;
    char* Ks = sm; char* Vs = sm + arr;
    stage_group_rows<T>(Ks, qkv + C + h * D, ld, n, Tn, P, p0, GP, nthr);
    stage_group_rows<T>(Vs, qkv + 2 * C + h * D, ld, n, Tn, P, p0, GP, nthr);
    __syncthreads();
    const int gp = threadIdx.x / Tn, t = threadIdx.x % Tn;
    const int p = p0 + gp;
    if (p >= P) return;
    const int64_t f = n * Tn + t;
    float qv[D], acc[D];
    load_row(qkv + (f * P + p) * ld + h * D, qv);
#pragma unroll
    for (int c = 0; c < D; ++c) acc[c] = 0.f;
    float m = -INFINITY, l = 0.f;
    for (int t2 = 0; t2 < Tn; ++t2) {
        const float s = dot_row(lds_row<T>(Ks, gp * Tn + t2, gp), qv) * scale;
        const float mn = fmaxf(m, s);
        const float a = __expf(m - mn), pr = __expf(s - mn);
        l = l * a + pr;
#pragma unroll
        for (int c = 0; c < D; ++c) acc[c] *= a;
        axpy_row(lds_row<T>(Vs, gp * Tn + t2, gp), pr, acc);
        m = mn;
    }
    store_row(o + (f * P + p) * C + h * D, acc, 1.f / l, 0);
    lse[(f * H + h) * P + p] = m + __logf(l);
}

#define DH 32
template <typename T>
__device__ __forceinline__ void load_half(const T* p, float (&v)[DH]) {
#pragma unroll
    for (int c = 0; c < DH; c += 8) { float t[8]; ld8(p + c, t);
#pragma unroll
        for (int j = 0; j < 8; ++j) v[c + j] = t[j]; }
}
template <typename T>
__device__ __forceinline__ float dot_half(const T* p, const float (&v)[DH]) {
    float s = 0.f;
#pragma unroll
    for (int c = 0; c < DH; c += 8) { float t[8]; ld8(p + c, t);
#pragma unroll
        for (int j = 0; j < 8; ++j) s = fmaf(v[c + j], t[j], s); }
    return s + __shfl_xor(s, 1, 64);
}
template <typename T>
__device__ __forceinline__ void axpy_half(const T* p, float a, float (&acc)[DH]) {
#pragma unroll
    for (int c = 0; c < DH; c += 8) { float t[8]; ld8(p + c, t);
#pragma unroll
        for (int j = 0; j < 8; ++j) acc[c + j] = fmaf(a, t[j], acc[c + j]); }
}
template <typename T>
__device__ __forceinline__ void store_half(T* p, const float (&v)[DH], int accumulate) {
#pragma unroll
    for (int c = 0; c < DH; c += 8) {
        float t[8];
#pragma unroll
        for (int j = 0; j < 8; ++j) t[j] = v[c + j];
        if (accumulate) { float o[8]; ld8(p + c, o);
#pragma unroll
            for (int j = 0; j < 8; ++j) t[j] += o[j]; }
        st8(p + c, t);
    }
}

template <typename T>
__global__ __launch_bounds__(256) void attn_tm_bwd_lds(const T* __restrict__ qkv, const T* __restrict__ o, const T* __restrict__ d_o,
                                                       const float* __restrict__ lse, T* __restrict__ dqkv, int accumulate,
                                                       int P, int H, int Tn, int GP, float scale) {
    MAED_DYN_SHARED(char, sm);
    const int C = H * D; const int64_t ld = 3 * (int64_t)C;
    const int chunks = (P + GP - 1) / GP;
    const int pc = blockIdx.x % chunks; int r0 = blockIdx.x / chunks;
    const int h = r0 % H; const int64_t n = r0 / H;
    const int p0 = pc * GP, nrows = GP * Tn;
    const size_t arr = (size_t)nrows * RowGeom<T>::RS + GP * 16;
    char* Qs = sm; char* Ks = sm + arr; char* Vs = sm + 2 * arr; char* dOs = sm + 3 * arr;
    float* Ls = reinterpret_cast<float*>(sm + 4 * arr); float* Ds = Ls + nrows;
    stage_group_rows<T>(Qs, qkv + h * D, ld, n, Tn, P, p0, GP, 256);
    stage_group_rows<T>(Ks, qkv + C + h * D, ld, n, Tn, P, p0, GP, 256);
    stage_group_rows<T>(Vs, qkv + 2 * C + h * D, ld, n, Tn, P, p0, GP, 256);
    stage_group_rows<T>(dOs, d_o + h * D, (int64_t)C, n, Tn, P, p0, GP, 256);
    const int h2 = threadIdx.x & 1, rt = threadIdx.x >> 1;
    const int gp = rt / Tn, t = rt - gp * Tn;
    const int p = p0 + gp;
    const int pcl = p < P ? p : P - 1;
    const int64_t f = n * Tn + t;
    const int64_t row = f * P + pcl;
    const int g0 = gp * Tn, ho = h2 * DH;
    float a[DH], b[DH], acc[DH];
    load_half(d_o + row * C + h * D + ho, b);
    const float Dq = dot_half(o + row * C + h * D + ho, b);
    const float L = lse[(f * H + h) * P + pcl];
    if (h2 == 0) { Ds[rt] = Dq; Ls[rt] = L; }
    __syncthreads();
    if (p >= P) return;
    load_half(lds_row<T>(Qs, g0 + t, gp) + ho, a);
#pragma unroll
    for (int c = 0; c < DH; ++c) acc[c] = 0.f;
    for (int t2 = 0; t2 < Tn; ++t2) {
        const T* kr = lds_row<T>(Ks, g0 + t2, gp) + ho;
        const float pr = __expf(dot_half(kr, a) * scale - L);
        const float ds = pr * (dot_half(lds_row<T>(Vs, g0 + t2, gp) + ho, b) - Dq) * scale;
        axpy_half(kr, ds, acc);
    }
    store_half(dqkv + row * ld + h * D + ho, acc, accumulate);
    load_half(lds_row<T>(Ks, g0 + t, gp) + ho, a);
#pragma unroll
    for (int c = 0; c < DH; ++c) acc[c] = 0.f;
    for (int t1 = 0; t1 < Tn; ++t1) {
        const float pr = __expf(dot_half(lds_row<T>(Qs, g0 + t1, gp) + ho, a) * scale - Ls[g0 + t1]);
        axpy_half(lds_row<T>(dOs, g0 + t1, gp) + ho, pr, acc);
    }
    store_half(dqkv + row * ld + 2 * C + h * D + ho, acc, accumulate);
    load_half(lds_row<T>(Vs, g0 + t, gp) + ho, b);
#pragma unroll
    for (int c = 0; c < DH; ++c) acc[c] = 0.f;
    for (int t1 = 0; t1 < Tn; ++t1) {
        const T* q1 = lds_row<T>(Qs, g0 + t1, gp) + ho;
        const float pr = __expf(dot_half(q1, a) * scale - Ls[g0 + t1]);
        const float ds = pr * (dot_half(lds_row<T>(dOs, g0 + t1, gp) + ho, b) - Ds[g0 + t1]) * scale;
        axpy_half(q1, ds, acc);
    }
    store_half(dqkv + row * ld + C + h * D + ho, acc, accumulate);
}

template <typename T>
static bool launch_tm_fwd_lds(const void* qkv, void* o, float* lse, int F, int P, int H, int Tn, float scale, hipStream_t s) {
    if (Tn > 256 || 256 % Tn != 0) return false;
    const int GP = 256 / Tn;
    const size_t lds = 2 * ((size_t)256 * RowGeom<T>::RS + GP * 16);
    if (lds > 160 * 1024) return false;
    static bool attr = false;
    if (!attr) { (void)hipFuncSetAttribute((const void*)attn_tm_fwd_lds<T>, hipFuncAttributeMaxDynamicSharedMemorySize, 160 * 1024); attr = true; }
    const int chunks = (P + GP - 1) / GP;
    hipLaunchKernelGGL((attn_tm_fwd_lds<T>), dim3((unsigned)((F / Tn) * H * chunks)), dim3(256), lds, s, (const T*)qkv, (T*)o, lse, P, H, Tn, GP, scale);
    return true;
}
template <typename T>
static bool launch_tm_bwd_lds(const void* qkv, const void* o, const void* d_o, const float* lse, void* dqkv, int accumulate, int F, int P,
                              int H, int Tn, float scale, hipStream_t s) {
    if (Tn > 128 || 128 % Tn != 0) return false;
    const int GP = 128 / Tn;
    const size_t lds = 4 * ((size_t)128 * RowGeom<T>::RS + GP * 16) + 2 * 128 * sizeof(float);
    if (lds > 160 * 1024) return false;
    static bool attr = false;
    if (!attr) { (void)hipFuncSetAttribute((const void*)attn_tm_bwd_lds<T>, hipFuncAttributeMaxDynamicSharedMemorySize, 160 * 1024); attr = true; }
    const int chunks = (P + GP - 1) / GP;
    hipLaunchKernelGGL((attn_tm_bwd_lds<T>), dim3((unsigned)((F / Tn) * H * chunks)), dim3(256), lds, s, (const T*)qkv, (const T*)o, (const T*)d_o,
                       lse, (T*)dqkv, accumulate, P, H, Tn, GP, scale);
    return true;
}

__global__ __launch_bounds__(1024) void attn_tm_fwd_mfma(const bf16* __restrict__ qkv, bf16* __restrict__ o, float* __restrict__ lse,
                                                         int P, int H, int Tn, int G, int ngroups, float scale_log2e) {
    MAED_DYN_SHARED(unsigned short, smem);
    const int L = G * Tn, Lk = (L + 31) & ~31, VLD = Lk + 4;
    unsigned short* Ks = smem;
    unsigned short* Vt = smem + (size_t)Lk * 64;
    const int C = H * D;
    const int64_t ld = 3 * (int64_t)C;
    const int tid = threadIdx.x, nthr = blockDim.x;
    const int lane = tid & 63, wave = tid >> 6, l31 = lane & 31, hi = lane >> 5;
    int bid = blockIdx.x;
    const int tg = bid % ngroups; bid /= ngroups;
    const int h = bid % H, n = bid / H;
    const int p0 = tg * G;
#define TM_ROW_OK(r) ((r) < L && p0 + (r) / Tn < P)
#define TM_ROW_OFF(r) ((((int64_t)n * Tn + (r) % Tn) * P + p0 + (r) / Tn) * ld + h * D)
    const int q = wave * 32 + l31;
    const bool q_ok = TM_ROW_OK(q);
    const int qg = q / Tn;
    bf16x8_t qf[4];
    {
        const int qc = q_ok ? q : 0;
        const bf16* qp = qkv + TM_ROW_OFF(qc);
#pragma unroll
        for (int t = 0; t < 4; ++t) qf[t] = *reinterpret_cast<const bf16x8_t*>(qp + t * 16 + hi * 8);
    }
    for (int idx = tid; idx < Lk * 8; idx += nthr) {
        const int r = idx >> 3, c8 = (idx & 7) * 8;
        uint4 kv = make_uint4(0u, 0u, 0u, 0u), vv = kv;
        if (TM_ROW_OK(r)) {
            const bf16* rp = qkv + TM_ROW_OFF(r);
            kv = *reinterpret_cast<const uint4*>(rp + C + c8);
            vv = *reinterpret_cast<const uint4*>(rp + 2 * C + c8);
        }
        *reinterpret_cast<uint4*>(Ks + r * 64 + (((c8 >> 3) ^ ((r >> 1) & 7)) << 3)) = kv;
        const uint32_t w[4] = {vv.x, vv.y, vv.z, vv.w};
#pragma unroll
        for (int j = 0; j < 4; ++j) {
            Vt[(c8 + 2 * j) * VLD + r] = (unsigned short)(w[j] & 0xffffu);
            Vt[(c8 + 2 * j + 1) * VLD + r] = (unsigned short)(w[j] >> 16);
        }
    }
    for (int i = tid; i < D * 4; i += nthr) Vt[(i >> 2) * VLD + Lk + (i & 3)] = 0;
    __syncthreads();

    f32x16_t oacc[2];
#pragma unroll
    for (int r = 0; r < 16; ++r) { oacc[0][r] = 0.f; oacc[1][r] = 0.f; }
    float m = -INFINITY, l = 0.f;
    const int nkt = Lk / 32;
    for (int kt = 0; kt < nkt; ++kt) {
        f32x16_t s;
#pragma unroll
        for (int r = 0; r < 16; ++r) s[r] = 0.f;
        const int krow = kt * 32 + l31;
        const unsigned short* kp = Ks + krow * 64;
        const int swz = (krow >> 1) & 7;
#pragma unroll
        for (int t = 0; t < 4; ++t) {
            const bf16x8_t kf = *reinterpret_cast<const bf16x8_t*>(kp + (((2 * t + hi) ^ swz) << 3));
            s = __builtin_amdgcn_mfma_f32_32x32x16_bf16(kf, qf[t], s, 0, 0, 0);
        }
        bool any = false;
#pragma unroll
        for (int r = 0; r < 16; ++r) {
            const int k = kt * 32 + (r & 3) + 8 * (r >> 2) + 4 * hi;
            const bool ok = TM_ROW_OK(k) && (k / Tn == qg);
            s[r] = ok ? s[r] : -INFINITY;
            any |= ok;
        }
        float mt = s[0];
#pragma unroll
        for (int r = 1; r < 16; ++r) mt = fmaxf(mt, s[r]);
        mt = fmaxf(mt, __shfl_xor(mt, 32, 64)) * scale_log2e;
        const float mn = fmaxf(m, mt);
        const float msafe = (mn == -INFINITY) ? 0.f : mn;
        const float alpha = (m == -INFINITY) ? 0.f : __builtin_amdgcn_exp2f(m - msafe);
        float ps = 0.f;
#pragma unroll
        for (int r = 0; r < 16; ++r) { s[r] = __builtin_amdgcn_exp2f(fmaf(s[r], scale_log2e, -msafe)); ps += s[r]; }
        l = l * alpha + ps;
        m = mn;
#pragma unroll
        for (int r = 0; r < 16; ++r) { oacc[0][r] *= alpha; oacc[1][r] *= alpha; }
#pragma unroll
        for (int st = 0; st < 2; ++st) {
            union { bf16x8_t v; uint32_t u[4]; } pf;
#pragma unroll
            for (int j = 0; j < 4; ++j) pf.u[j] = pack_bf2(s[8 * st + 2 * j], s[8 * st + 2 * j + 1]);
#pragma unroll
            for (int et = 0; et < 2; ++et) {
                const unsigned short* vp = Vt + (et * 32 + l31) * VLD + kt * 32 + 16 * st + 4 * hi;
                union { bf16x8_t v; uint2 u[2]; } vf;
                vf.u[0] = *reinterpret_cast<const uint2*>(vp);
                vf.u[1] = *reinterpret_cast<const uint2*>(vp + 8);
                oacc[et] = __builtin_amdgcn_mfma_f32_32x32x16_bf16(vf.v, pf.v, oacc[et], 0, 0, 0);
            }
        }
        (void)any;
    }
    l += __shfl_xor(l, 32, 64);
    if (Lk == 32) {
        const float inv = q_ok ? 1.f / l : 0.f;
#pragma unroll
        for (int r = 0; r < 16; ++r) { oacc[0][r] *= inv; oacc[1][r] *= inv; }
        store_tile_lines_at(Ks, [&](int r) -> bf16* { return TM_ROW_OK(r) ? o + (((int64_t)n * Tn + r % Tn) * P + p0 + r / Tn) * C + h * D : nullptr; }, oacc, lane, 0);
        if (q_ok && hi == 0) lse[(((int64_t)n * Tn + q % Tn) * H + h) * P + p0 + qg] = (m + log2f(l)) * 0.69314718055994530942f;
    } else if (q_ok) {
        const float inv = 1.f / l;
        const int t = q % Tn, p = p0 + qg;
        const int64_t f = (int64_t)n * Tn + t;
        bf16* orow = o + (f * P + p) * C + h * D;
#pragma unroll
        for (int et = 0; et < 2; ++et)
#pragma unroll
            for (int g = 0; g < 4; ++g) {
                const int e0 = et * 32 + 8 * g + 4 * hi;
                const uint2 w = make_uint2(pack_bf2(oacc[et][4 * g] * inv, oacc[et][4 * g + 1] * inv),
                                           pack_bf2(oacc[et][4 * g + 2] * inv, oacc[et][4 * g + 3] * inv));
                *reinterpret_cast<uint2*>(orow + e0) = w;
            }
        if (hi == 0) lse[(f * H + h) * P + p] = (m + log2f(l)) * 0.69314718055994530942f;
    }
#undef TM_ROW_OK
#undef TM_ROW_OFF
}

template <int MAX_THREADS, int MIN_BLOCKS>
__global__ __launch_bounds__(MAX_THREADS, MIN_BLOCKS) void attn_tm_bwd_mfma(const bf16* __restrict__ qkv, const bf16* __restrict__ o, const bf16* __restrict__ d_o,
                                                         const float* __restrict__ lse, bf16* __restrict__ dqkv, int accumulate, int P, int H,
                                                         int Tn, int G, int ngroups, float scale) {
    MAED_DYN_SHARED(unsigned short, smem);
    const int L = G * Tn, Lk = (L + 31) & ~31, VLD = Lk + 4;
    unsigned short* Qs = smem;
    unsigned short* Ks = Qs + (size_t)Lk * KLD;
    unsigned short* Vs = Ks + (size_t)Lk * KLD;
    unsigned short* dOs = Vs + (size_t)Lk * KLD;
    unsigned short* Qt = dOs + (size_t)Lk * KLD;
    unsigned short* Kt = Qt + (size_t)D * VLD;
    unsigned short* dOt = Kt + (size_t)D * VLD;
    float* Ls = reinterpret_cast<float*>(dOt + (size_t)D * VLD);
    float* Ds = Ls + Lk;
    const int C = H * D;
    const int64_t ld = 3 * (int64_t)C;
    const int tid = threadIdx.x, nthr = blockDim.x;
    const int lane = tid & 63, wave = tid >> 6, l31 = lane & 31, hi = lane >> 5;
    int bid = blockIdx.x;
    const int tg = bid % ngroups; bid /= ngroups;
    const int h = bid % H, n = bid / H;
    const int p0 = tg * G;
#define TM_ROW_OK(r) ((r) < L && p0 + (r) / Tn < P)
#define TM_TOK(r) (((int64_t)n * Tn + (r) % Tn) * P + p0 + (r) / Tn)
    const float l2e = 1.44269504088896340736f;
    for (int idx = tid; idx < Lk * 8; idx += nthr) {
        const int r = idx >> 3, c8 = (idx & 7) * 8;
        uint4 qv = make_uint4(0u, 0u, 0u, 0u), kv = qv, vv = qv, gv = qv;
        if (TM_ROW_OK(r)) {
            const int64_t tok = TM_TOK(r);
            const bf16* rp = qkv + tok * ld + h * D;
            qv = *reinterpret_cast<const uint4*>(rp + c8);
            kv = *reinterpret_cast<const uint4*>(rp + C + c8);
            vv = *reinterpret_cast<const uint4*>(rp + 2 * C + c8);
            gv = *reinterpret_cast<const uint4*>(d_o + tok * C + h * D + c8);
        }
        *reinterpret_cast<uint4*>(Qs + r * KLD + c8) = qv;
        *reinterpret_cast<uint4*>(Ks + r * KLD + c8) = kv;
        *reinterpret_cast<uint4*>(Vs + r * KLD + c8) = vv;
        *reinterpret_cast<uint4*>(dOs + r * KLD + c8) = gv;
        const uint32_t wq[4] = {qv.x, qv.y, qv.z, qv.w}, wk[4] = {kv.x, kv.y, kv.z, kv.w}, wg[4] = {gv.x, gv.y, gv.z, gv.w};
#pragma unroll
        for (int j = 0; j < 4; ++j) {
            const int e0 = (c8 + 2 * j) * VLD + r, e1 = (c8 + 2 * j + 1) * VLD + r;
            Qt[e0] = (unsigned short)(wq[j] & 0xffffu); Qt[e1] = (unsigned short)(wq[j] >> 16);
            Kt[e0] = (unsigned short)(wk[j] & 0xffffu); Kt[e1] = (unsigned short)(wk[j] >> 16);
            dOt[e0] = (unsigned short)(wg[j] & 0xffffu); dOt[e1] = (unsigned short)(wg[j] >> 16);
        }
    }
    for (int i = tid; i < D * 4; i += nthr) {
        const int e = (i >> 2) * VLD + Lk + (i & 3);
        Qt[e] = 0; Kt[e] = 0; dOt[e] = 0;
    }
    for (int r = tid; r < Lk; r += nthr) {
        float dsum = 0.f, Lv = 0.f;
        if (TM_ROW_OK(r)) {
            const int64_t tok = TM_TOK(r);
#pragma unroll
            for (int c = 0; c < D; c += 8) {
                float a[8], b[8];
                ld8(d_o + tok * C + h * D + c, a); ld8(o + tok * C + h * D + c, b);
#pragma unroll
                for (int j = 0; j < 8; ++j) dsum = fmaf(a[j], b[j], dsum);
            }
            Lv = lse[(((int64_t)n * Tn + r % Tn) * H + h) * P + p0 + r / Tn] * l2e;
        }
        Ds[r] = dsum; Ls[r] = Lv;
    }
    __syncthreads();

    const int row = wave * 32 + l31;
    const bool row_ok = TM_ROW_OK(row);
    const int rg = row / Tn;
    const float sl2e = scale * l2e;
    const int nt = Lk / 32;
    bf16* drow = dqkv + (row_ok ? TM_TOK(row) : 0) * ld + h * D;
    {
        bf16x8_t qf[4], dof[4];
#pragma unroll
        for (int t = 0; t < 4; ++t) {
            qf[t] = *reinterpret_cast<const bf16x8_t*>(Qs + row * KLD + t * 16 + hi * 8);
            dof[t] = *reinterpret_cast<const bf16x8_t*>(dOs + row * KLD + t * 16 + hi * 8);
        }
        const float Dq = Ds[row], L2 = Ls[row];
        f32x16_t dq[2];
#pragma unroll
        for (int r = 0; r < 16; ++r) { dq[0][r] = 0.f; dq[1][r] = 0.f; }
        for (int kt = 0; kt < nt; ++kt) {
            f32x16_t sa, dp;
#pragma unroll
            for (int r = 0; r < 16; ++r) { sa[r] = 0.f; dp[r] = 0.f; }
            const int krow = kt * 32 + l31;
#pragma unroll
            for (int t = 0; t < 4; ++t) {
                const bf16x8_t kf = *reinterpret_cast<const bf16x8_t*>(Ks + krow * KLD + t * 16 + hi * 8);
                const bf16x8_t vf = *reinterpret_cast<const bf16x8_t*>(Vs + krow * KLD + t * 16 + hi * 8);
                sa = __builtin_amdgcn_mfma_f32_32x32x16_bf16(kf, qf[t], sa, 0, 0, 0);
                dp = __builtin_amdgcn_mfma_f32_32x32x16_bf16(vf, dof[t], dp, 0, 0, 0);
            }
#pragma unroll
            for (int r = 0; r < 16; ++r) {
                const int k = kt * 32 + (r & 3) + 8 * (r >> 2) + 4 * hi;
                const bool ok = row_ok && TM_ROW_OK(k) && (k / Tn == rg);
                const float pr = ok ? __builtin_amdgcn_exp2f(fmaf(sa[r], sl2e, -L2)) : 0.f;
                sa[r] = pr * (dp[r] - Dq) * scale;
            }
#pragma unroll
            for (int st = 0; st < 2; ++st) {
                const bf16x8_t dsf = pack_frag(sa, st);
#pragma unroll
                for (int et = 0; et < 2; ++et) {
                    const bf16x8_t ktf = lds_frag_tr(Kt + (et * 32 + l31) * VLD + kt * 32 + 16 * st + 4 * hi);
                    dq[et] = __builtin_amdgcn_mfma_f32_32x32x16_bf16(ktf, dsf, dq[et], 0, 0, 0);
                }
            }
        }
        if (row_ok) store_rowT(drow, dq, hi, accumulate);
    }
    {
        bf16x8_t kf[4], vf[4];
#pragma unroll
        for (int t = 0; t < 4; ++t) {
            kf[t] = *reinterpret_cast<const bf16x8_t*>(Ks + row * KLD + t * 16 + hi * 8);
            vf[t] = *reinterpret_cast<const bf16x8_t*>(Vs + row * KLD + t * 16 + hi * 8);
        }
        f32x16_t dk[2], dv[2];
#pragma unroll
        for (int r = 0; r < 16; ++r) { dk[0][r] = 0.f; dk[1][r] = 0.f; dv[0][r] = 0.f; dv[1][r] = 0.f; }
        for (int qt = 0; qt < nt; ++qt) {
            f32x16_t sb, dp;
#pragma unroll
            for (int r = 0; r < 16; ++r) { sb[r] = 0.f; dp[r] = 0.f; }
            const int qrow = qt * 32 + l31;
#pragma unroll
            for (int t = 0; t < 4; ++t) {
                const bf16x8_t qfr = *reinterpret_cast<const bf16x8_t*>(Qs + qrow * KLD + t * 16 + hi * 8);
                const bf16x8_t dofr = *reinterpret_cast<const bf16x8_t*>(dOs + qrow * KLD + t * 16 + hi * 8);
                sb = __builtin_amdgcn_mfma_f32_32x32x16_bf16(qfr, kf[t], sb, 0, 0, 0);
                dp = __builtin_amdgcn_mfma_f32_32x32x16_bf16(dofr, vf[t], dp, 0, 0, 0);
            }
#pragma unroll
            for (int r = 0; r < 16; ++r) {
                const int qq = qt * 32 + (r & 3) + 8 * (r >> 2) + 4 * hi;
                const bool ok = row_ok && TM_ROW_OK(qq) && (qq / Tn == rg);
                const float pr = ok ? __builtin_amdgcn_exp2f(fmaf(sb[r], sl2e, -Ls[qq])) : 0.f;
                dp[r] = pr * (dp[r] - Ds[qq]) * scale;
                sb[r] = pr;
            }
#pragma unroll
            for (int st = 0; st < 2; ++st) {
                const bf16x8_t pf = pack_frag(sb, st), dsf = pack_frag(dp, st);
#pragma unroll
                for (int et = 0; et < 2; ++et) {
                    const int off = (et * 32 + l31) * VLD + qt * 32 + 16 * st + 4 * hi;
                    dv[et] = __builtin_amdgcn_mfma_f32_32x32x16_bf16(lds_frag_tr(dOt + off), pf, dv[et], 0, 0, 0);
                    dk[et] = __builtin_amdgcn_mfma_f32_32x32x16_bf16(lds_frag_tr(Qt + off), dsf, dk[et], 0, 0, 0);
                }
            }
        }
        if (row_ok) {
            store_rowT(drow + C, dk, hi, accumulate);
            store_rowT(drow + 2 * C, dv, hi, accumulate);
        }
    }
#undef TM_ROW_OK
#undef TM_TOK
}

__global__ __launch_bounds__(64, 3) void attn_tm_bwd_mfma_l32(const bf16* __restrict__ qkv, const bf16* __restrict__ o, const bf16* __restrict__ d_o,
                                                               const float* __restrict__ lse, bf16* __restrict__ dqkv, int accumulate, int P, int H,
                                                               int Tn, int G, int ngroups, float scale) {
    __shared__ __attribute__((aligned(16))) unsigned short Qs[32 * KLD], Ks[32 * KLD], dOs[32 * KLD];
    __shared__ float Ls[32], Ds[32];
    const int L = G * Tn, C = H * D;
    const int64_t ld = 3 * (int64_t)C;
    const int lane = threadIdx.x, l31 = lane & 31, hi = lane >> 5;
    int bid = blockIdx.x;
    const int tg = bid % ngroups; bid /= ngroups;
    const int h = bid % H, n = bid / H;
    const int p0 = tg * G;
#define TM_ROW_OK(r) ((r) < L && p0 + (r) / Tn < P)
#define TM_TOK(r) (((int64_t)n * Tn + (r) % Tn) * P + p0 + (r) / Tn)
    const int row = l31;
    const bool row_ok = TM_ROW_OK(row);
    const int64_t tok = row_ok ? TM_TOK(row) : 0;
    const bf16* rp = qkv + tok * ld + h * D;
    const bf16* gp = d_o + tok * C + h * D;
    const bf16* op = o + tok * C + h * D;
    const float l2e = 1.44269504088896340736f;
    union Frag { bf16x8_t v; uint4 u; };
    Frag qf[4], kf[4], vf[4], dof[4];
    float dsum = 0.f;
#pragma unroll
    for (int t = 0; t < 4; ++t) {
        const int e0 = t * 16 + hi * 8;
        qf[t].u = kf[t].u = vf[t].u = dof[t].u = make_uint4(0u, 0u, 0u, 0u);
        if (row_ok) {
            qf[t].u = *reinterpret_cast<const uint4*>(rp + e0);
            kf[t].u = *reinterpret_cast<const uint4*>(rp + C + e0);
            vf[t].u = *reinterpret_cast<const uint4*>(rp + 2 * C + e0);
            dof[t].u = *reinterpret_cast<const uint4*>(gp + e0);
            float a[8], b[8];
            ld8(gp + e0, a); ld8(op + e0, b);
#pragma unroll
            for (int j = 0; j < 8; ++j) dsum = fmaf(a[j], b[j], dsum);
        }
        *reinterpret_cast<uint4*>(Qs + row * KLD + e0) = qf[t].u;
        *reinterpret_cast<uint4*>(Ks + row * KLD + e0) = kf[t].u;
        *reinterpret_cast<uint4*>(dOs + row * KLD + e0) = dof[t].u;
    }
    dsum += __shfl_xor(dsum, 32, 64);
    const float Dq = dsum;
    const float L2 = row_ok ? lse[(((int64_t)n * Tn + row % Tn) * H + h) * P + p0 + row / Tn] * l2e : 0.f;
    if (hi == 0) { Ds[row] = Dq; Ls[row] = L2; }
    __syncthreads();

    const int rg = row / Tn;
    const float sl2e = scale * l2e;
    bf16* drow = dqkv + tok * ld + h * D;
    {
        f32x16_t sa, dp, dq[2];
#pragma unroll
        for (int r = 0; r < 16; ++r) { sa[r] = 0.f; dp[r] = -Dq; dq[0][r] = 0.f; dq[1][r] = 0.f; }
#pragma unroll
        for (int t = 0; t < 4; ++t) {
            sa = __builtin_amdgcn_mfma_f32_32x32x16_bf16(kf[t].v, qf[t].v, sa, 0, 0, 0);
            dp = __builtin_amdgcn_mfma_f32_32x32x16_bf16(vf[t].v, dof[t].v, dp, 0, 0, 0);
        }
#pragma unroll
        for (int r = 0; r < 16; ++r) {
            const int k = (r & 3) + 8 * (r >> 2) + 4 * hi;
            const bool ok = row_ok && TM_ROW_OK(k) && (k / Tn == rg);
            const float pr = ok ? __builtin_amdgcn_exp2f(fmaf(sa[r], sl2e, -L2)) : 0.f;
            sa[r] = pr * dp[r];
        }
#pragma unroll
        for (int st = 0; st < 2; ++st) {
            const bf16x8_t dsf = pack_frag(sa, st);
#pragma unroll
            for (int et = 0; et < 2; ++et)
                dq[et] = __builtin_amdgcn_mfma_f32_32x32x16_bf16(lds_frag_tr_rm(Ks, 16 * st, et * 32, lane), dsf, dq[et], 0, 0, 0);
        }
#pragma unroll
        for (int r = 0; r < 16; ++r) { dq[0][r] *= scale; dq[1][r] *= scale; }
        store_tile_lines_at(Ks, [&](int r) -> bf16* { return TM_ROW_OK(r) ? dqkv + TM_TOK(r) * ld + h * D : nullptr; }, dq, lane, accumulate);
    }
    {
        f32x16_t sb, dp, dk[2], dv[2];
#pragma unroll
        for (int r = 0; r < 16; ++r) { sb[r] = 0.f; dp[r] = -Ds[(r & 3) + 8 * (r >> 2) + 4 * hi]; dk[0][r] = 0.f; dk[1][r] = 0.f; dv[0][r] = 0.f; dv[1][r] = 0.f; }
#pragma unroll
        for (int t = 0; t < 4; ++t) {
            sb = __builtin_amdgcn_mfma_f32_32x32x16_bf16(qf[t].v, kf[t].v, sb, 0, 0, 0);
            dp = __builtin_amdgcn_mfma_f32_32x32x16_bf16(dof[t].v, vf[t].v, dp, 0, 0, 0);
        }
#pragma unroll
        for (int r = 0; r < 16; ++r) {
            const int qq = (r & 3) + 8 * (r >> 2) + 4 * hi;
            const bool ok = row_ok && TM_ROW_OK(qq) && (qq / Tn == rg);
            const float pr = ok ? __builtin_amdgcn_exp2f(fmaf(sb[r], sl2e, -Ls[qq])) : 0.f;
            dp[r] *= pr;
            sb[r] = pr;
        }
#pragma unroll
        for (int st = 0; st < 2; ++st) {
            const bf16x8_t pf = pack_frag(sb, st), dsf = pack_frag(dp, st);
#pragma unroll
            for (int et = 0; et < 2; ++et) {
                dv[et] = __builtin_amdgcn_mfma_f32_32x32x16_bf16(lds_frag_tr_rm(dOs, 16 * st, et * 32, lane), pf, dv[et], 0, 0, 0);
                dk[et] = __builtin_amdgcn_mfma_f32_32x32x16_bf16(lds_frag_tr_rm(Qs, 16 * st, et * 32, lane), dsf, dk[et], 0, 0, 0);
            }
        }
#pragma unroll
        for (int r = 0; r < 16; ++r) { dk[0][r] *= scale; dk[1][r] *= scale; }
        store_tile_lines_at(Ks, [&](int r) -> bf16* { return TM_ROW_OK(r) ? dqkv + TM_TOK(r) * ld + h * D + C : nullptr; }, dk, lane, accumulate);
        store_tile_lines_at(Ks, [&](int r) -> bf16* { return TM_ROW_OK(r) ? dqkv + TM_TOK(r) * ld + h * D + 2 * C : nullptr; }, dv, lane, accumulate);
    }
#undef TM_ROW_OK
#undef TM_TOK
}


static bool launch_tm_bwd_mfma(const void* qkv, const void* o, const void* d_o, const float* lse, void* dqkv, int accumulate, int F, int P, int H,
                               int Tn, float scale, hipStream_t s) {
    const int G = Tn >= 32 ? 1 : 32 / Tn;
    const int L = G * Tn, Lk = (L + 31) & ~31;
    if (Lk / 32 > 16) return false;
    const size_t lds = ((size_t)4 * Lk * KLD + (size_t)3 * D * (Lk + 4)) * 2 + (size_t)2 * Lk * sizeof(float);
    if (lds > 160 * 1024) return false;
    static bool attr = false;
    if (!attr) {
        (void)hipFuncSetAttribute((const void*)attn_tm_bwd_mfma<256, 2>, hipFuncAttributeMaxDynamicSharedMemorySize, 160 * 1024);
        (void)hipFuncSetAttribute((const void*)attn_tm_bwd_mfma<1024, 1>, hipFuncAttributeMaxDynamicSharedMemorySize, 160 * 1024);
        attr = true;
    }
    const int ngroups = (P + G - 1) / G;
    const dim3 grid((unsigned)((F / Tn) * H * ngroups)), block(64 * (Lk / 32));
    if (Lk == 32) {
        hipLaunchKernelGGL(attn_tm_bwd_mfma_l32, grid, dim3(64), 0, s, (const bf16*)qkv, (const bf16*)o, (const bf16*)d_o, lse, (bf16*)dqkv, accumulate,
                           P, H, Tn, G, ngroups, scale);
// ... 72 lines not shown
```

### maed_amd/csrc/block.hip

```cpp
#include "common.cuh"
#include "gemm_x3.h"
#include "prof.h"
#include <hip/hip_runtime.h>
#include <atomic>
#include <mutex>
#include <utility>
#include <vector>

static bool g_prof = false;
struct ProfRec { hipEvent_t a, b; double flops, bytes; };
static std::vector<ProfRec> g_prof_ev[PROF_NTAGS];
bool maed_prof_on() { return g_prof; }
void maed_prof_open(int tag, hipStream_t s, hipEvent_t* a) { (void)tag; (void)hipEventCreate(a); (void)hipEventRecord(*a, s); }
void maed_prof_close(int tag, hipStream_t s, hipEvent_t a, double flops, double bytes) {
    hipEvent_t b;
    (void)hipEventCreate(&b); (void)hipEventRecord(b, s);
    g_prof_ev[tag].push_back(ProfRec{a, b, flops, bytes});
}
extern "C" int maed_prof_enable(int on) { g_prof = on != 0; return MAED_OK; }
extern "C" int maed_prof_ntags(void) { return PROF_NTAGS; }
extern "C" int maed_prof_flops(double* flops) {
    for (int t = 0; t < PROF_NTAGS; ++t) {
        double tot = 0.0;
        for (auto& r : g_prof_ev[t]) tot += r.flops;
        if (flops) flops[t] = tot;
    }
    return MAED_OK;
}
extern "C" int maed_prof_records(int tag, double* us, double* flops, double* bytes, int cap) {
    if (tag < 0 || tag >= PROF_NTAGS) return 0;
    int i = 0;
    for (auto& r : g_prof_ev[tag]) {
        if (i < cap) {
            (void)hipEventSynchronize(r.b);
            float ms = 0.f;
            (void)hipEventElapsedTime(&ms, r.a, r.b);
            if (us) us[i] = 1e3 * (double)ms;
            if (flops) flops[i] = r.flops;
            if (bytes) bytes[i] = r.bytes;
        }
        ++i;
    }
    return i;
}
extern "C" int maed_prof_collect(double* ms_total, int* count) {
    for (int t = 0; t < PROF_NTAGS; ++t) {
        double tot = 0.0;
        for (auto& r : g_prof_ev[t]) {
            (void)hipEventSynchronize(r.b);
            float ms = 0.f;
            (void)hipEventElapsedTime(&ms, r.a, r.b);
            tot += ms;
            (void)hipEventDestroy(r.a); (void)hipEventDestroy(r.b);
        }
        if (ms_total) ms_total[t] = tot;
        if (count) count[t] = (int)g_prof_ev[t].size();
        g_prof_ev[t].clear();
    }
    return MAED_OK;
}
#define PROF(tag, expr) do { ProfScope ps__(tag, stream); MAED_PROPAGATE(expr); } while (0)

struct SideStream {
    hipStream_t s = nullptr;
    hipStream_t s2 = nullptr;
    hipEvent_t ev[64];
    hipEvent_t cast_ev[2];
    bool cast_pending[2] = {false, false};
    int next = 0;
    bool ok = false;
    void fence(hipStream_t from, hipStream_t to) {
        hipEvent_t e = ev[next]; next = (next + 1) % 62;
        (void)hipEventRecord(e, from);
        (void)hipStreamWaitEvent(to, e, 0);
    }
};
static SideStream g_side;
static hipEvent_t g_fence_ring[64];
static bool g_fence_ok = false;
static std::once_flag g_runtime_once;
int maed_sk_init(void);
int maed_init_runtime(void) {
    std::call_once(g_runtime_once, [] {
        SideStream& ss = g_side;
        bool ok = hipStreamCreateWithFlags(&ss.s, hipStreamNonBlocking) == hipSuccess && hipStreamCreateWithFlags(&ss.s2, hipStreamNonBlocking) == hipSuccess;
        for (int i = 0; ok && i < 64; ++i) ok = hipEventCreateWithFlags(&ss.ev[i], hipEventDisableTiming) == hipSuccess;
        for (int i = 0; ok && i < 2; ++i) ok = hipEventCreateWithFlags(&ss.cast_ev[i], hipEventDisableTiming) == hipSuccess;
        ss.ok = ok;
        g_fence_ok = true;
        for (int i = 0; i < 64; ++i) if (hipEventCreateWithFlags(&g_fence_ring[i], hipEventDisableTiming) != hipSuccess) { g_fence_ok = false; break; }
        if (!ok || !g_fence_ok) (void)hipGetLastError();
        (void)maed_sk_init();
    });
    return (g_side.ok && g_fence_ok) ? MAED_OK : MAED_ERR_LAUNCH;
}
static SideStream* side_stream() {
    if (!maed_opt(MAED_OPT_SIDE_STREAM) || g_prof) return nullptr;
    (void)maed_init_runtime();
    return g_side.ok ? &g_side : nullptr;
}

extern "C" int maed_ste_block_twin_join(void* stream) {
    (void)maed_init_runtime();
    SideStream& ss = g_side;
    if (!ss.ok) return MAED_OK;
    for (int k = 0; k < 2; ++k)
        if (ss.cast_pending[k]) { MAED_HIP(hipStreamWaitEvent((hipStream_t)stream, ss.cast_ev[k], 0), "ste_block_twin_join: stream wait"); ss.cast_pending[k] = false; }
    return MAED_OK;
}

extern "C" int maed_stream_fence(void* from_stream, void* to_stream) {
    static std::atomic<unsigned> next{0};
    (void)maed_init_runtime();
    MAED_CHECK_ARG(g_fence_ok, MAED_ERR_LAUNCH, "stream_fence: event ring could not be created");
    if (from_stream == to_stream) return MAED_OK;
    hipEvent_t e = g_fence_ring[next.fetch_add(1, std::memory_order_relaxed) & 63];
    MAED_HIP(hipEventRecord(e, (hipStream_t)from_stream), "stream_fence: record");
    MAED_HIP(hipStreamWaitEvent((hipStream_t)to_stream, e, 0), "stream_fence: wait");
    return MAED_OK;
}

namespace {

inline size_t al(size_t x) { return (x + 255) & ~(size_t)255; }

struct SavedLayout {
    size_t ln1, mean1, rstd1, qkv, xs, xt, lse_s, lse_t, means, logits, mix, xmid, mean2, rstd2, ln2, hpre, hact, st_sync, st_ex, total;
};
struct ScratchLayout {
    size_t dyc, dyt, bigA, bigT, xT, act, dxs, dxt, dxmid, dlog, dmeans, dlogT, meansT, ws, total;
    int64_t Mp, Fp;
};

SavedLayout saved_layout(const maed_block_dims& d) {
    const size_t es = dtype_size(d.dtype);
    const size_t M = (size_t)d.F * d.P, C = d.C, Hd = d.hidden;
    SavedLayout s{};
    size_t o = 0;
    auto take = [&](size_t bytes) { size_t r = o; o += al(bytes); return r; };
    s.ln1 = take(M * C * es); s.mean1 = take(M * 4); s.rstd1 = take(M * 4);
    s.qkv = take(M * 3 * C * es); s.xs = take(M * C * es); s.xt = take(M * C * es);
    s.lse_s = take((size_t)d.F * d.H * d.P * 4); s.lse_t = take((size_t)d.F * d.H * d.P * 4);
    s.means = take((size_t)d.F * 2 * C * es); s.logits = take((size_t)d.F * 2 * C * 4);
    s.mix = take(M * C * es); s.xmid = take(M * C * 4);
    s.mean2 = take(M * 4); s.rstd2 = take(M * 4); s.ln2 = take(M * C * es);
    s.hpre = take(M * Hd * es); s.hact = take(M * Hd * es);
    s.st_sync = take((size_t)d.F * 16 * 4); s.st_ex = take((size_t)d.F * 2 * C * 4);
    s.total = o;
    return s;
}

ScratchLayout scratch_layout(const maed_block_dims& d) {
    const size_t es = dtype_size(d.dtype);
    const size_t M = (size_t)d.F * d.P, C = d.C, Hd = d.hidden;
    ScratchLayout s{};
    s.Mp = (int64_t)((M + 63) / 64 * 64);
    s.Fp = (int64_t)(((size_t)d.F + 63) / 64 * 64);
    const size_t big = Hd > 3 * C ? Hd : 3 * C;
    size_t o = 0;
    auto take = [&](size_t bytes) { size_t r = o; o += al(bytes); return r; };
    s.dyc = take(M * C * es); s.dyt = take(C * (size_t)s.Mp * es);
    s.bigA = take(M * big * es); s.bigT = take(big * (size_t)s.Mp * es);
    s.xT = take(C * (size_t)s.Mp * es); s.act = take(M * C * es);
    s.dxs = take(M * C * es); s.dxt = take(M * C * es); s.dxmid = take(M * C * 4);
    s.dlog = take((size_t)d.F * 2 * C * es); s.dmeans = take((size_t)d.F * 2 * C * es);
    s.dlogT = take(2 * C * (size_t)s.Fp * es); s.meansT = take(2 * C * (size_t)s.Fp * es);
    s.ws = take((size_t)d.F * 2 * C * 4);
    s.total = o;
    return s;
}

}
size_t maed_layernorm_bwd_partials_bytes(int64_t rows, int C);
int maed_layernorm_bwd_ws(const void* dy, int dtype, const float* x, int64_t x_row_stride, const float* gamma, const float* mean, const float* rstd,
                          const float* dres_in, float* dx_out, void* dx_twin, float* dgamma, float* dbeta, int64_t rows, int C, float* partials,
                          void* stream, bool finish = true, uint32_t* clear = nullptr, int clear_words = 0);
int maed_layernorm_affine_finish(const float* partials, int64_t rows, int C, float* dgamma, float* dbeta, void* stream);
int maed_layernorm_fwd_ws(const float* x, int64_t x_row_stride, const float* gamma, const float* beta, void* y, int dtype, float* mean, float* rstd, int64_t rows,
                          int C, float eps, uint32_t* clear, int clear_words, void* stream, void* y_lo = nullptr);
int maed_st_fused_fwd_ws(const void* x_s, const void* x_t, const void* w_ts, const float* b_ts, void* means, float* logits, void* mix,
                         uint32_t* sync, float* ex, int F, int P, int C, int dtype, bool clear_sync, uint32_t arrive_base, void* stream);
int maed_st_fused_bwd_ws(const void* dmix, const void* x_s, const void* x_t, const float* logits, const void* wt_ts, void* dlogits, void* dx_s,
                         void* dx_t, uint32_t* sync, float* ex, int F, int P, int C, int dtype, bool clear_sync, uint32_t arrive_base, void* stream);
namespace {

int check_dims(const maed_block_dims* d, const char* who) {
    MAED_CHECK_ARG(d, MAED_ERR_ARG, "%s: null dims", who);
    MAED_CHECK_ARG(d->dtype == MAED_F32 || d->dtype == MAED_BF16, MAED_ERR_ARG, "%s: bad dtype %d", who, d->dtype);
    MAED_CHECK_ARG(d->F > 0 && d->P > 0 && d->H > 0 && d->T > 0 && d->hidden > 0, MAED_ERR_SHAPE, "%s: non-positive extent", who);
    MAED_CHECK_ARG(d->C == d->H * HEAD_DIM, MAED_ERR_SHAPE, "%s: C=%d must equal 64*H (H=%d)", who, d->C, d->H);
    MAED_CHECK_ARG(d->F % d->T == 0, MAED_ERR_SHAPE, "%s: F=%d not a multiple of T=%d", who, d->F, d->T);
    MAED_CHECK_ARG(d->hidden % 64 == 0, MAED_ERR_SHAPE, "%s: hidden=%d must be a multiple of 64", who, d->hidden);
    return MAED_OK;
}

bool st_fused(const maed_block_dims& d) {
    return d.impl != MAED_IMPL_VALU && maed_opt(MAED_OPT_ST_FUSED) && d.P <= 224 && maed_st_fused_supported(d.P, d.C, d.dtype);
}

int pick_splitk(int64_t Mo, int64_t No, int64_t K, int dtype) {
    const int64_t tile = (dtype == MAED_BF16) ? 128 : 64;
    const int64_t kt = (dtype == MAED_BF16) ? 64 : 16;
    const int64_t tiles = ((Mo + tile - 1) / tile) * ((No + tile - 1) / tile);
    int64_t s = (1024 + tiles - 1) / tiles;
    const int64_t maxs = K / (kt * 4) > 0 ? K / (kt * 4) : 1;
    if (s > maxs) s = maxs;
    if (s < 1) s = 1;
    return (int)s;
}

int wgrad(const void* Yt, const void* Xt, int64_t No, int64_t Ko, int64_t Mp, float* dW, const maed_block_dims& d, void* st) {
    return maed_gemm_nt(Yt, Mp, Xt, Mp, No, Ko, Mp, d.dtype, MAED_EPI_ATOMIC_F32, nullptr, dW, Ko, nullptr, nullptr, 0,
                        pick_splitk(No, Ko, Mp, d.dtype), d.impl == MAED_IMPL_VALU ? MAED_IMPL_VALU : MAED_IMPL_AUTO, st);
}

}

extern "C" size_t maed_ste_block_saved_bytes(const maed_block_dims* d) { return d ? saved_layout(*d).total : 0; }
extern "C" size_t maed_ste_block_scratch_bytes(const maed_block_dims* d) { return d ? scratch_layout(*d).total : 0; }

struct FwdBufs { char *ln1, *mean1, *rstd1, *qkv, *xs, *xt, *lse_s, *lse_t, *means, *logits, *mix, *xmid, *mean2, *rstd2, *ln2, *hpre, *hact, *st_sync, *st_ex;
                 char *tw_qkv = nullptr, *tw_hact = nullptr; bool hpre_bf16 = false;
                 char *hact_lo = nullptr, *wfc2_hi = nullptr, *wfc2_lo = nullptr; int planes_variant = 0;
                 char *ln1_hi = nullptr, *ln1_lo = nullptr, *ln2_hi = nullptr, *ln2_lo = nullptr, *wqkv_hi = nullptr, *wqkv_lo = nullptr, *wfc1_hi = nullptr, *wfc1_lo = nullptr; };
static FwdBufs fwd_bufs(char* act_base, const SavedLayout& A, char* f32_base, const SavedLayout& Fl) {
    FwdBufs b;
    b.ln1 = act_base + A.ln1; b.qkv = act_base + A.qkv; b.xs = act_base + A.xs; b.xt = act_base + A.xt; b.means = act_base + A.means; b.mix = act_base + A.mix;
    b.ln2 = act_base + A.ln2; b.hpre = act_base + A.hpre; b.hact = act_base + A.hact;
    b.mean1 = f32_base + Fl.mean1; b.rstd1 = f32_base + Fl.rstd1; b.lse_s = f32_base + Fl.lse_s; b.lse_t = f32_base + Fl.lse_t; b.logits = f32_base + Fl.logits;
    b.xmid = f32_base + Fl.xmid; b.mean2 = f32_base + Fl.mean2; b.rstd2 = f32_base + Fl.rstd2; b.st_sync = f32_base + Fl.st_sync; b.st_ex = f32_base + Fl.st_ex;
    return b;
}

int maed_gemm_nt_twin(const void* A, int64_t lda, const void* B, int64_t ldb, int64_t M, int64_t N, int64_t K, int dtype, int epilogue, const float* bias, void* out,
                      int64_t ldo, void* out2, const void* aux, int64_t ldaux, int splitk, int impl, void* stream, void* twin, bool out2_bf16, void* lo);
static int block_fwd_bufs(const maed_block_dims* d, const maed_block_params* p, const float* x_in, float* x_out, const FwdBufs& B, bool for_backward, void* stream) {
    const int64_t M = (int64_t)d->F * d->P;
    const int C = d->C, Hd = d->hidden, dt = d->dtype;
    const int gi = d->impl == MAED_IMPL_VALU ? MAED_IMPL_VALU : MAED_IMPL_AUTO;
    const float scale = 1.0f / sqrtf((float)HEAD_DIM);
    float* logits = (float*)B.logits;

    const bool stf = st_fused(*d);
    const bool piggy = stf && maed_opt(MAED_OPT_ST_FUSED) != 2 && (int64_t)d->F * 16 <= 256 * ((M + 31) / 32);
    if (B.ln1_lo) {
        const float* wsrc[3] = {(const float*)p->w_fc2, (const float*)p->w_qkv, (const float*)p->w_fc1};
        void* wh[3] = {B.wfc2_hi, B.wqkv_hi, B.wfc1_hi}; void* wl[3] = {B.wfc2_lo, B.wqkv_lo, B.wfc1_lo};
        const int64_t wn[3] = {(int64_t)C * Hd, (int64_t)3 * C * C, (int64_t)C * Hd};
        MAED_PROPAGATE(maed_split_planes_launch(3, wsrc, wh, wl, wn, (hipStream_t)stream));
        MAED_CHECK_LAUNCH("ste_block_fwd_twin: weight planes");
        MAED_PROPAGATE(maed_layernorm_fwd_ws(x_in, C, p->ln1_g, p->ln1_b, B.ln1_hi, MAED_BF16, (float*)(B.mean1), (float*)(B.rstd1), M, C, d->eps,
                                             piggy ? (uint32_t*)(B.st_sync) : nullptr, piggy ? d->F * 16 : 0, stream, B.ln1_lo));
        EpiArgs eq{};
        eq.bias = p->b_qkv; eq.out = B.qkv; eq.ldo = 3 * C; eq.twin = B.tw_qkv;
        PROF(PROF_GEMM_QKV, maed_gemm_nt_x3p_launch(MAED_EPI_STORE, 2, B.ln1_hi, B.ln1_lo, C, B.wqkv_hi, B.wqkv_lo, C, M, 3 * C, C, eq, (hipStream_t)stream));
        MAED_CHECK_LAUNCH("ste_block_fwd_twin: qkv on planes");
    } else {
    MAED_PROPAGATE(maed_layernorm_fwd_ws(x_in, C, p->ln1_g, p->ln1_b, B.ln1, dt, (float*)(B.mean1), (float*)(B.rstd1), M, C, d->eps,
                                         piggy ? (uint32_t*)(B.st_sync) : nullptr, piggy ? d->F * 16 : 0, stream));
    PROF(PROF_GEMM_QKV, maed_gemm_nt_twin(B.ln1, C, p->w_qkv, C, M, 3 * C, C, dt, MAED_EPI_STORE, p->b_qkv, B.qkv, 3 * C, nullptr, nullptr, 0, 1, gi, stream, B.tw_qkv, false, nullptr));
    }
    {
        SideStream* ss = (d->impl != MAED_IMPL_VALU && (dt == MAED_BF16 || maed_x3_planes())) ? side_stream() : nullptr;
        void* tst = ss ? (void*)ss->s : stream;
        if (ss) ss->fence((hipStream_t)stream, ss->s);
        { ProfScope ps__(PROF_ATTN_TM_FWD, tst); MAED_PROPAGATE(maed_attn_temporal_fwd(B.qkv, B.xt, (float*)(B.lse_t), d->F, d->P, d->H, d->T, scale, dt, tst)); }
        PROF(PROF_ATTN_SP_FWD, maed_attn_spatial_fwd(B.qkv, B.xs, (float*)(B.lse_s), d->F, d->P, d->H, scale, dt, d->impl, stream));
        if (ss) ss->fence(ss->s, (hipStream_t)stream);
    }
    if (stf) {
        PROF(PROF_ST_FWD, maed_st_fused_fwd_ws(B.xs, B.xt, p->w_ts, p->b_ts, B.means, logits, B.mix, (uint32_t*)(B.st_sync), (float*)(B.st_ex),
                                               d->F, d->P, C, dt, !piggy, 0u, stream));
    } else {
        MAED_PROPAGATE(maed_st_colmean(B.xs, B.xt, B.means, logits , d->F, d->P, C, dt, stream));
        MAED_PROPAGATE(maed_gemm_nt(B.means, 2 * C, p->w_ts, 2 * C, d->F, 2 * C, 2 * C, dt, MAED_EPI_STORE_F32, p->b_ts, logits, 2 * C, nullptr, nullptr, 0, 1, gi, stream));
        MAED_PROPAGATE(maed_st_mix_fwd(B.xs, B.xt, logits, B.mix, d->F, d->P, C, dt, stream));
    }
    PROF(PROF_GEMM_PROJ, maed_gemm_nt(B.mix, C, p->w_proj, C, M, C, C, dt, MAED_EPI_RESID_F32, p->b_proj, B.xmid, C, nullptr, x_in, C, 1, gi, stream));
    if (B.ln2_lo) MAED_PROPAGATE(maed_layernorm_fwd_ws((const float*)(B.xmid), C, p->ln2_g, p->ln2_b, B.ln2_hi, MAED_BF16, (float*)(B.mean2), (float*)(B.rstd2), M, C, d->eps,
                                                       nullptr, 0, stream, B.ln2_lo));
    else MAED_PROPAGATE(maed_layernorm_fwd((const float*)(B.xmid), C, p->ln2_g, p->ln2_b, B.ln2, dt, (float*)(B.mean2), (float*)(B.rstd2), M, C, d->eps, stream));
    if (B.hact_lo) {
        if (!B.ln1_lo) {
            const float* wsrc[1] = {(const float*)p->w_fc2}; void* wh[1] = {B.wfc2_hi}; void* wl[1] = {B.wfc2_lo}; const int64_t wn[1] = {(int64_t)C * Hd};
            MAED_PROPAGATE(maed_split_planes_launch(1, wsrc, wh, wl, wn, (hipStream_t)stream));
            MAED_CHECK_LAUNCH("ste_block_fwd_twin: weight planes");
        }
        if (B.ln2_lo) {
            EpiArgs e1{};
            e1.bias = p->b_fc1; e1.ldo = Hd; e1.out2 = B.hpre; e1.out2_bf16 = true; e1.twin = B.tw_hact; e1.lo = B.hact_lo;
            PROF(PROF_GEMM_FC1, maed_gemm_nt_x3p_launch(MAED_EPI_GELU, 2, B.ln2_hi, B.ln2_lo, C, B.wfc1_hi, B.wfc1_lo, C, M, Hd, C, e1, (hipStream_t)stream));
            MAED_CHECK_LAUNCH("ste_block_fwd_twin: fc1 on planes");
        } else
        PROF(PROF_GEMM_FC1, maed_gemm_nt_twin(B.ln2, C, p->w_fc1, C, M, Hd, C, dt, MAED_EPI_GELU, p->b_fc1, nullptr, Hd, B.hpre, nullptr, 0, 1, gi, stream, B.tw_hact, true, B.hact_lo));
        EpiArgs e2{};
        e2.bias = p->b_fc2; e2.out = x_out; e2.ldo = C; e2.aux = B.xmid; e2.ldaux = C;
        PROF(PROF_GEMM_FC2, maed_gemm_nt_x3p_launch(MAED_EPI_RESID_F32, B.planes_variant, B.tw_hact, B.hact_lo, Hd, B.wfc2_hi, B.wfc2_lo, Hd, M, C, Hd, e2, (hipStream_t)stream));
        MAED_CHECK_LAUNCH("ste_block_fwd_twin: fc2 on planes");
        return MAED_OK;
    }
    PROF(PROF_GEMM_FC1, maed_gemm_nt_twin(B.ln2, C, p->w_fc1, C, M, Hd, C, dt, MAED_EPI_GELU, p->b_fc1, B.hact, Hd, for_backward ? B.hpre : nullptr , nullptr, 0, 1, gi,
                                          stream, B.tw_hact, B.hpre_bf16, nullptr));
    PROF(PROF_GEMM_FC2, maed_gemm_nt(B.hact, Hd, p->w_fc2, Hd, M, C, Hd, dt, MAED_EPI_RESID_F32, p->b_fc2, x_out, C, nullptr, B.xmid, C, 1, gi, stream));
    return MAED_OK;
}

static int block_fwd(const maed_block_dims* d, const maed_block_params* p, const float* x_in, float* x_out, void* saved, bool for_backward, void* stream) {
    MAED_PROPAGATE(check_dims(d, "ste_block_fwd"));
    MAED_CHECK_ARG(p && x_in && x_out && saved, MAED_ERR_ARG, "ste_block_fwd: null pointer");
    MAED_CHECK_ARG(is_aligned(saved, 256), MAED_ERR_ALIGN, "ste_block_fwd: saved buffer must be 256-B aligned");
    const SavedLayout L = saved_layout(*d);
    return block_fwd_bufs(d, p, x_in, x_out, fwd_bufs((char*)saved, L, (char*)saved, L), for_backward, stream);
}

struct CastTab { const float* src[12]; bf16* dst[12]; long long n8[12]; };
__global__ __launch_bounds__(256) void cast_table_kernel(CastTab t) {
    const float* __restrict__ src = t.src[blockIdx.y];
    bf16* __restrict__ dst = t.dst[blockIdx.y];
    const long long n8 = t.n8[blockIdx.y];
    for (long long i = (long long)blockIdx.x * 256 + threadIdx.x; i < n8; i += (long long)gridDim.x * 256) {
        float v[8];
        ld8(src + i * 8, v);
        st8_nt(dst + i * 8, v);
    }
}

extern "C" size_t maed_ste_block_twin_work_bytes(const maed_block_dims* d) {
    if (!d) return 0;
    maed_block_dims d32 = *d; d32.dtype = MAED_F32;
    return saved_layout(d32).total + ((size_t)2 * d->C * d->hidden + (size_t)3 * d->C * d->C) * 4;
}

extern "C" int maed_ste_block_fwd_twin(const maed_block_dims* d, const maed_block_params* p, const float* x_in, float* x_out, void* saved_bf16, void* work_f32,
                                       int work_slot, void* stream) {
    MAED_PROPAGATE(check_dims(d, "ste_block_fwd_twin"));
    MAED_CHECK_ARG(d->dtype == MAED_F32, MAED_ERR_ARG, "ste_block_fwd_twin: dims describe the FORWARD (dtype MAED_F32); the arena is laid out for MAED_BF16");
    MAED_CHECK_ARG(p && x_in && x_out && saved_bf16 && work_f32, MAED_ERR_ARG, "ste_block_fwd_twin: null pointer");
    MAED_CHECK_ARG(is_aligned(saved_bf16, 256) && is_aligned(work_f32, 256), MAED_ERR_ALIGN, "ste_block_fwd_twin: buffers must be 256-B aligned");
    MAED_CHECK_ARG(d->C % 8 == 0 && d->hidden % 8 == 0, MAED_ERR_SHAPE, "ste_block_fwd_twin: C and hidden must be multiples of 8");
    MAED_CHECK_ARG(work_slot == 0 || work_slot == 1, MAED_ERR_ARG, "ste_block_fwd_twin: work_slot must be 0 or 1");
    maed_block_dims d16 = *d; d16.dtype = MAED_BF16;
    const SavedLayout L32 = saved_layout(*d), L16 = saved_layout(d16);
    char* w = (char*)work_f32; char* sv = (char*)saved_bf16;
    SideStream* ss = side_stream();
    if (ss && ss->cast_pending[work_slot]) MAED_HIP(hipStreamWaitEvent((hipStream_t)stream, ss->cast_ev[work_slot], 0), "ste_block_fwd_twin: stream wait");
    FwdBufs fb = fwd_bufs(w, L32, sv, L16);
    fb.tw_qkv = sv + L16.qkv; fb.tw_hact = sv + L16.hact; fb.hpre = sv + L16.hpre; fb.hpre_bf16 = true;
    const int pv = maed_opt(MAED_OPT_X3_PLANES);
    char* const wpl = w + L32.total;
    if (pv && maed_x3_planes() == 2 && d->impl != MAED_IMPL_VALU
        && maed_x3p_shape_ok(fb.tw_hact, w + L32.hact, d->hidden, wpl, wpl + (size_t)d->C * d->hidden * 2, d->hidden, (int64_t)d->F * d->P, d->C, d->hidden)) {
        fb.hact_lo = w + L32.hact; fb.wfc2_hi = wpl; fb.wfc2_lo = wpl + (size_t)d->C * d->hidden * 2; fb.planes_variant = pv;
        if (maed_opt(MAED_OPT_X3_PLANES_LN) && d->C % 32 == 0) {
            const size_t CH2 = (size_t)d->C * d->hidden * 2, CC2 = (size_t)3 * d->C * d->C * 2;
            fb.ln1_hi = sv + L16.ln1; fb.ln1_lo = w + L32.ln1; fb.ln2_hi = sv + L16.ln2; fb.ln2_lo = w + L32.ln2;
            fb.wqkv_hi = wpl + 2 * CH2; fb.wqkv_lo = fb.wqkv_hi + CC2; fb.wfc1_hi = fb.wqkv_lo + CC2; fb.wfc1_lo = fb.wfc1_hi + CH2;
        }
    }
    MAED_PROPAGATE(block_fwd_bufs(d, p, x_in, x_out, fb, true, stream));
    const long long M = (long long)d->F * d->P, C = d->C;
    CastTab t{};
    int k = 0;
    auto add = [&](size_t o32, size_t o16, long long n) { t.src[k] = (const float*)(w + o32); t.dst[k] = (bf16*)(sv + o16); t.n8[k] = n / 8; ++k; };
    if (!fb.ln1_lo) add(L32.ln1, L16.ln1, M * C);
    add(L32.xs, L16.xs, M * C); add(L32.xt, L16.xt, M * C);
    add(L32.means, L16.means, (long long)d->F * 2 * C); add(L32.mix, L16.mix, M * C);
    if (!fb.ln2_lo) add(L32.ln2, L16.ln2, M * C);
    hipStream_t cs = (hipStream_t)stream;
    if (ss) { ss->fence((hipStream_t)stream, ss->s2); cs = ss->s2; }
    hipLaunchKernelGGL(cast_table_kernel, dim3(1024, k), dim3(256), 0, cs, t);
    MAED_CHECK_LAUNCH("ste_block_fwd_twin: cast");
    if (ss) { MAED_HIP(hipEventRecord(ss->cast_ev[work_slot], ss->s2), "ste_block_fwd_twin: event"); ss->cast_pending[work_slot] = true; }
    return MAED_OK;
}

extern "C" int maed_ste_block_fwd(const maed_block_dims* d, const maed_block_params* p, const float* x_in, float* x_out, void* saved, void* stream) {
    return block_fwd(d, p, x_in, x_out, saved, true, stream);
}
extern "C" int maed_ste_block_infer(const maed_block_dims* d, const maed_block_params* p, const float* x_in, float* x_out, void* work, void* stream) {
    return block_fwd(d, p, x_in, x_out, work, false, stream);
}

extern "C" int maed_ste_block_bwd(const maed_block_dims* d, const maed_block_params* p, const maed_block_grads* g,
                                  const float* x_in, const float* dx_out, float* dx_in, void* saved, void* scratch,
                                  const void* dx_out_twin, void* dx_in_twin, void* stream) {
    MAED_PROPAGATE(check_dims(d, "ste_block_bwd"));
    MAED_CHECK_ARG(p && g && x_in && dx_out && dx_in && saved && scratch, MAED_ERR_ARG, "ste_block_bwd: null pointer");
    MAED_CHECK_ARG(p->wt_qkv && p->wt_ts && p->wt_proj && p->wt_fc1 && p->wt_fc2, MAED_ERR_ARG, "ste_block_bwd: transposed weights missing");
    MAED_CHECK_ARG(is_aligned(saved, 256) && is_aligned(scratch, 256), MAED_ERR_ALIGN, "ste_block_bwd: saved/scratch must be 256-B aligned");
    const SavedLayout L = saved_layout(*d);
    const ScratchLayout S = scratch_layout(*d);
    char* sv = (char*)saved; char* sc = (char*)scratch;
    if (d->dtype == MAED_BF16) {
        SideStream* ssc = side_stream();
        for (int k = 0; ssc && k < 2; ++k)
            if (ssc->cast_pending[k]) { MAED_HIP(hipStreamWaitEvent((hipStream_t)stream, ssc->cast_ev[k], 0), "ste_block_bwd: stream wait"); ssc->cast_pending[k] = false; }
    }
    const int64_t M = (int64_t)d->F * d->P, Mp = S.Mp, Fp = S.Fp;
    const int C = d->C, Hd = d->hidden, dt = d->dtype;
    const int gi = d->impl == MAED_IMPL_VALU ? MAED_IMPL_VALU : MAED_IMPL_AUTO;
    const float scale = 1.0f / sqrtf((float)HEAD_DIM);
    const float* logits = (const float*)(sv + L.logits);
    float* dxmid = (float*)(sc + S.dxmid);

    if (d->impl != MAED_IMPL_VALU && (dt == MAED_BF16 || (maed_x3_planes() && d->hidden % 4 == 0))) {
        const void* dyc = dt == MAED_F32 ? (const void*)dx_out : dx_out_twin;
        if (!dyc) {
            MAED_PROPAGATE(maed_transpose_cast(dx_out, MAED_F32, C, M, C, nullptr, 0, sc + S.dyc, C, nullptr, dt, stream));
            dyc = sc + S.dyc;
        }
        void* dxmid_tw = dt == MAED_F32 ? (void*)dxmid : (void*)(sc + S.dyt);
        SideStream* ss = side_stream();
        hipStream_t main_s = (hipStream_t)stream;
        void* wst = ss ? (void*)ss->s : stream;
#define TO_SIDE() do { if (ss) ss->fence(main_s, ss->s); } while (0)
#define FROM_SIDE() do { if (ss) ss->fence(ss->s, main_s); } while (0)
#define WGRAD(expr) do { ProfScope ps__(PROF_GEMM_WGRAD, wst); MAED_PROPAGATE(expr); } while (0)
        const int dmm = (dt == MAED_F32 && maed_opt(MAED_OPT_F32_BWD_X1)) ? MAED_F32X1 : dt;
        TO_SIDE();
        WGRAD(maed_gemm_tn_wgrad(dyc, C, sv + L.hact, Hd, M, C, Hd, g->w_fc2, Hd, g->b_fc2, dmm, wst));
        PROF(PROF_GEMM_DGRAD, maed_gemm_nt(dyc, C, p->wt_fc2, C, M, Hd, C, dmm, MAED_EPI_MUL_DGELU, nullptr, sc + S.bigA, Hd, nullptr, sv + L.hpre, Hd, 1, gi, stream));
        TO_SIDE();
        WGRAD(maed_gemm_tn_wgrad(sc + S.bigA, Hd, sv + L.ln2, C, M, Hd, C, g->w_fc1, C, g->b_fc1, dmm, wst));
        if (ss) MAED_HIP(hipEventRecord(ss->ev[63], ss->s), "ste_block_bwd: event");
        PROF(PROF_GEMM_DGRAD, maed_gemm_nt(sc + S.bigA, Hd, p->wt_fc1, Hd, M, C, Hd, dmm, MAED_EPI_STORE, nullptr, sc + S.act, C, nullptr, nullptr, 0, 1, gi, stream));
        const size_t big_t_bytes = (size_t)(Hd > 3 * C ? Hd : 3 * C) * (size_t)Mp * dtype_size(dt);
        const size_t ln_pb = (maed_layernorm_bwd_partials_bytes(M, C) + 255) & ~(size_t)255;
        float* ln_part = 2 * ln_pb <= big_t_bytes ? (float*)(sc + S.bigT) : nullptr;
        float* ln_part1 = ln_part ? (float*)(sc + S.bigT + ln_pb) : nullptr;
        const bool ln_side = ss != nullptr && ln_part != nullptr && maed_opt(MAED_OPT_ST_FUSED) == 4;
        const bool piggy = st_fused(*d) && maed_opt(MAED_OPT_ST_FUSED) != 2 && (int64_t)d->F * 16 <= 256 * ((M + 31) / 32);
        MAED_PROPAGATE(maed_layernorm_bwd_ws(sc + S.act, dt, (const float*)(sv + L.xmid), C, p->ln2_g, (const float*)(sv + L.mean2), (const float*)(sv + L.rstd2),
                                             dx_out, dxmid, dt == MAED_F32 ? nullptr : dxmid_tw, g->ln2_g, g->ln2_b, M, C, ln_part, stream, !ln_side,
                                             piggy ? (uint32_t*)(sv + L.st_sync) : nullptr, piggy ? d->F * 16 : 0));
        if (ln_side) { TO_SIDE(); MAED_PROPAGATE(maed_layernorm_affine_finish(ln_part, M, C, g->ln2_g, g->ln2_b, wst)); }
        TO_SIDE();
        WGRAD(maed_gemm_tn_wgrad(dxmid_tw, C, sv + L.mix, C, M, C, C, g->w_proj, C, g->b_proj, dmm, wst));
        PROF(PROF_GEMM_DGRAD, maed_gemm_nt(dxmid_tw, C, p->wt_proj, C, M, C, C, dmm, MAED_EPI_STORE, nullptr, sc + S.act, C, nullptr, nullptr, 0, 1, gi, stream));
        if (st_fused(*d)) {
            PROF(PROF_ST_BWD, maed_st_fused_bwd_ws(sc + S.act, sv + L.xs, sv + L.xt, logits, p->wt_ts, sc + S.dlog, sc + S.dxs, sc + S.dxt, (uint32_t*)(sv + L.st_sync),
                                                   (float*)(sv + L.st_ex), d->F, d->P, C, dt, !piggy, 0u, stream));
            TO_SIDE();
            WGRAD(maed_gemm_tn_wgrad(sc + S.dlog, 2 * C, sv + L.means, 2 * C, d->F, 2 * C, 2 * C, g->w_ts, 2 * C, g->b_ts, dmm, wst));
        } else {
            MAED_PROPAGATE(maed_st_mix_bwd_reduce(sc + S.act, sv + L.xs, sv + L.xt, logits, sc + S.dlog, (float*)(sc + S.ws), d->F, d->P, C, dt, stream));
            TO_SIDE();
            WGRAD(maed_gemm_tn_wgrad(sc + S.dlog, 2 * C, sv + L.means, 2 * C, d->F, 2 * C, 2 * C, g->w_ts, 2 * C, g->b_ts, dmm, wst));
            MAED_PROPAGATE(maed_gemm_nt(sc + S.dlog, 2 * C, p->wt_ts, 2 * C, d->F, 2 * C, 2 * C, dmm, MAED_EPI_STORE, nullptr, sc + S.dmeans, 2 * C, nullptr, nullptr, 0, 1, gi, stream));
            MAED_PROPAGATE(maed_st_mix_bwd_apply(sc + S.act, logits, sc + S.dmeans, sc + S.dxs, sc + S.dxt, d->F, d->P, C, dt, stream));
        }
        if (ss) MAED_HIP(hipStreamWaitEvent(main_s, ss->ev[63], 0), "ste_block_bwd: stream wait");
        PROF(PROF_ATTN_TM_BWD, maed_attn_temporal_bwd(sv + L.qkv, sv + L.xt, sc + S.dxt, (const float*)(sv + L.lse_t), sc + S.bigA, 0, d->F, d->P, d->H, d->T, scale, dt, stream));
        PROF(PROF_ATTN_SP_BWD, maed_attn_spatial_bwd(sv + L.qkv, sv + L.xs, sc + S.dxs, (const float*)(sv + L.lse_s), sc + S.bigA, 1, d->F, d->P, d->H, scale, dt,
                                                     MAED_IMPL_AUTO, stream));
        TO_SIDE();
        WGRAD(maed_gemm_tn_wgrad(sc + S.bigA, 3 * C, sv + L.ln1, C, M, 3 * C, C, g->w_qkv, C, g->b_qkv, dmm, wst));
        PROF(PROF_GEMM_DGRAD, maed_gemm_nt(sc + S.bigA, 3 * C, p->wt_qkv, 3 * C, M, C, 3 * C, dmm, MAED_EPI_STORE, nullptr, sc + S.act, C, nullptr, nullptr, 0, 1, gi, stream));
        MAED_PROPAGATE(maed_layernorm_bwd_ws(sc + S.act, dt, x_in, C, p->ln1_g, (const float*)(sv + L.mean1), (const float*)(sv + L.rstd1), dxmid, dx_in,
                                             dx_in_twin, g->ln1_g, g->ln1_b, M, C, ln_part1, stream, !ln_side));
        if (ln_side) { TO_SIDE(); MAED_PROPAGATE(maed_layernorm_affine_finish(ln_part1, M, C, g->ln1_g, g->ln1_b, wst)); }
        FROM_SIDE();
#undef TO_SIDE
#undef FROM_SIDE
#undef WGRAD
        return MAED_OK;
    }
    MAED_PROPAGATE(maed_transpose_cast(dx_out, MAED_F32, C, M, C, sc + S.dyt, Mp, sc + S.dyc, C, g->b_fc2, dt, stream));
    MAED_PROPAGATE(maed_transpose_cast(sv + L.hact, dt, Hd, M, Hd, sc + S.bigT, Mp, nullptr, 0, nullptr, dt, stream));
    PROF(PROF_GEMM_WGRAD, wgrad(sc + S.dyt, sc + S.bigT, C, Hd, Mp, g->w_fc2, *d, stream));
    MAED_PROPAGATE(maed_gemm_nt(sc + S.dyc, C, p->wt_fc2, C, M, Hd, C, dt, MAED_EPI_MUL_DGELU, nullptr, sc + S.bigA, Hd, nullptr, sv + L.hpre, Hd, 1, gi, stream));
    MAED_PROPAGATE(maed_transpose_cast(sc + S.bigA, dt, Hd, M, Hd, sc + S.bigT, Mp, nullptr, 0, g->b_fc1, dt, stream));
    MAED_PROPAGATE(maed_transpose_cast(sv + L.ln2, dt, C, M, C, sc + S.xT, Mp, nullptr, 0, nullptr, dt, stream));
    PROF(PROF_GEMM_WGRAD, wgrad(sc + S.bigT, sc + S.xT, Hd, C, Mp, g->w_fc1, *d, stream));
    MAED_PROPAGATE(maed_gemm_nt(sc + S.bigA, Hd, p->wt_fc1, Hd, M, C, Hd, dt, MAED_EPI_STORE, nullptr, sc + S.act, C, nullptr, nullptr, 0, 1, gi, stream));
    MAED_PROPAGATE(maed_layernorm_bwd(sc + S.act, dt, (const float*)(sv + L.xmid), C, p->ln2_g, (const float*)(sv + L.mean2), (const float*)(sv + L.rstd2),
                                      dx_out, dxmid, nullptr, g->ln2_g, g->ln2_b, M, C, stream));
    MAED_PROPAGATE(maed_transpose_cast(dxmid, MAED_F32, C, M, C, sc + S.dyt, Mp, sc + S.dyc, C, g->b_proj, dt, stream));
    MAED_PROPAGATE(maed_transpose_cast(sv + L.mix, dt, C, M, C, sc + S.xT, Mp, nullptr, 0, nullptr, dt, stream));
    PROF(PROF_GEMM_WGRAD, wgrad(sc + S.dyt, sc + S.xT, C, C, Mp, g->w_proj, *d, stream));
    MAED_PROPAGATE(maed_gemm_nt(sc + S.dyc, C, p->wt_proj, C, M, C, C, dt, MAED_EPI_STORE, nullptr, sc + S.act, C, nullptr, nullptr, 0, 1, gi, stream));
    MAED_PROPAGATE(maed_st_mix_bwd_reduce(sc + S.act, sv + L.xs, sv + L.xt, logits, sc + S.dlog, (float*)(sc + S.ws), d->F, d->P, C, dt, stream));
    MAED_PROPAGATE(maed_transpose_cast(sc + S.dlog, dt, 2 * C, d->F, 2 * C, sc + S.dlogT, Fp, nullptr, 0, g->b_ts, dt, stream));
    MAED_PROPAGATE(maed_transpose_cast(sv + L.means, dt, 2 * C, d->F, 2 * C, sc + S.meansT, Fp, nullptr, 0, nullptr, dt, stream));
    PROF(PROF_GEMM_WGRAD, wgrad(sc + S.dlogT, sc + S.meansT, 2 * C, 2 * C, Fp, g->w_ts, *d, stream));
    MAED_PROPAGATE(maed_gemm_nt(sc + S.dlog, 2 * C, p->wt_ts, 2 * C, d->F, 2 * C, 2 * C, dt, MAED_EPI_STORE, nullptr, sc + S.dmeans, 2 * C, nullptr, nullptr, 0, 1, gi, stream));
    MAED_PROPAGATE(maed_st_mix_bwd_apply(sc + S.act, logits, sc + S.dmeans, sc + S.dxs, sc + S.dxt, d->F, d->P, C, dt, stream));
    PROF(PROF_ATTN_TM_BWD, maed_attn_temporal_bwd(sv + L.qkv, sv + L.xt, sc + S.dxt, (const float*)(sv + L.lse_t), sc + S.bigA, 0, d->F, d->P, d->H, d->T, scale, dt, stream));
    PROF(PROF_ATTN_SP_BWD, maed_attn_spatial_bwd(sv + L.qkv, sv + L.xs, sc + S.dxs, (const float*)(sv + L.lse_s), sc + S.bigA, 1, d->F, d->P, d->H, scale, dt,
                                         d->impl == MAED_IMPL_VALU ? MAED_IMPL_VALU : MAED_IMPL_AUTO, stream));
    MAED_PROPAGATE(maed_transpose_cast(sc + S.bigA, dt, 3 * C, M, 3 * C, sc + S.bigT, Mp, nullptr, 0, g->b_qkv, dt, stream));
    MAED_PROPAGATE(maed_transpose_cast(sv + L.ln1, dt, C, M, C, sc + S.xT, Mp, nullptr, 0, nullptr, dt, stream));
    PROF(PROF_GEMM_WGRAD, wgrad(sc + S.bigT, sc + S.xT, 3 * C, C, Mp, g->w_qkv, *d, stream));
    MAED_PROPAGATE(maed_gemm_nt(sc + S.bigA, 3 * C, p->wt_qkv, 3 * C, M, C, 3 * C, dt, MAED_EPI_STORE, nullptr, sc + S.act, C, nullptr, nullptr, 0, 1, gi, stream));
    MAED_PROPAGATE(maed_layernorm_bwd(sc + S.act, dt, x_in, C, p->ln1_g, (const float*)(sv + L.mean1), (const float*)(sv + L.rstd1), dxmid, dx_in, dx_in_twin,
                                      g->ln1_g, g->ln1_b, M, C, stream));
    return MAED_OK;
}

static thread_local char g_err[512] = "";
void maed_set_error(const char* fmt, ...) {
    va_list ap;
    va_start(ap, fmt);
    vsnprintf(g_err, sizeof(g_err), fmt, ap);
    va_end(ap);
}
extern "C" const char* maed_last_error(void) { return g_err; }
#ifdef MAED_HOSTSIM
extern "C" int maed_version(void) { return -100; }
#else
extern "C" int maed_version(void) { return 100; }
#endif
```

### maed_amd/csrc/options.hip

```cpp
#include "common.cuh"
#include "gemm_x3.h"
#include <atomic>
#include <string.h>

static std::atomic<int> g_opt[MAED_OPT_COUNT] = {
    {0},
    {1},
    {0},
    {0},
    {1},
    {0},
    {1},
    {256},
    {512},
    {0},
    {1},
    {6},
    {0},
    {1},
    {0},
    {1},
    {0},
    {1},
};

extern "C" int maed_init(int device) {
#ifndef MAED_HOSTSIM
    hipDeviceProp_t prop;
    if (hipGetDeviceProperties(&prop, device) != hipSuccess) { (void)hipGetLastError(); maed_set_error("init: no HIP device %d", device); return MAED_ERR_ARG; }
    if (!strstr(prop.gcnArchName, "gfx950")) {
        maed_set_error("init: device %d is %s; libmaed_hip is built for gfx950 (MI355X) only", device, prop.gcnArchName);
        return MAED_ERR_UNSUPPORTED;
    }
#else
    (void)device;
#endif
    (void)maed_fault_word();
#ifndef MAED_HOSTSIM
    if (maed_init_runtime() != MAED_OK) { maed_set_error("init: could not create the library's side streams / event rings"); return MAED_ERR_LAUNCH; }
#endif
    return MAED_OK;
}

static std::atomic<uint32_t*> g_fault{nullptr};
static std::atomic<int> g_fault_told{0};
uint32_t* maed_fault_word(void) {
    uint32_t* w = g_fault.load(std::memory_order_acquire);
    if (w) return w;
#ifdef MAED_HOSTSIM
    uint32_t* n = (uint32_t*)calloc(16, sizeof(uint32_t));
#else
    uint32_t* n = nullptr;
    if (hipHostMalloc((void**)&n, 64, hipHostMallocMapped | hipHostMallocCoherent) != hipSuccess || !n) { (void)hipGetLastError(); return nullptr; }
    memset(n, 0, 64);
#endif
    uint32_t* expected = nullptr;
    if (!g_fault.compare_exchange_strong(expected, n, std::memory_order_acq_rel)) {
#ifdef MAED_HOSTSIM
        free(n);
#else
        (void)hipHostFree(n);
#endif
        return expected;
    }
    return n;
}
bool maed_fault_seen(const char* who) {
    uint32_t* w = g_fault.load(std::memory_order_acquire);
    if (!w || *(volatile uint32_t*)w == 0) return false;
    if (!g_fault_told.exchange(1))
        maed_set_error("%s: %u frame-barrier timeout(s) on this device (workgroups of a frame were not co-resident: shared GPU / preemption); the affected results were "
                       "NaN-poisoned, the one-pass GroupNorm backward and the fused attentive addition now run as their multi-launch forms", who, *(volatile uint32_t*)w);
    return true;
}
extern "C" int maed_device_faults(void) {
    uint32_t* w = g_fault.load(std::memory_order_acquire);
    const int n = w ? (int)*(volatile uint32_t*)w : 0;
    if (n > 0)
        maed_set_error("%d frame-barrier timeout(s) on this device (workgroups of a frame were not co-resident: shared GPU / preemption); the affected results were "
                       "NaN-poisoned, the one-pass GroupNorm backward and the fused attentive addition run as their multi-launch forms from the next call on", n);
    return n;
}
extern "C" int maed_device_faults_clear(void) { uint32_t* w = g_fault.load(std::memory_order_acquire); if (w) *(volatile uint32_t*)w = 0; g_fault_told.store(0); return MAED_OK; }

extern "C" int maed_set_option(int key, int value) {
    MAED_CHECK_ARG(key >= 0 && key < MAED_OPT_COUNT, MAED_ERR_ARG, "set_option: unknown option %d", key);
    if (key == MAED_OPT_F32_MATMUL) MAED_CHECK_ARG(value >= 0 && value <= 2, MAED_ERR_ARG, "set_option: MAED_OPT_F32_MATMUL takes 0 (exact), 1 (bf16x3) or 2 (bf16x6)");
    if (key == MAED_OPT_TN_TARGET_WGS) MAED_CHECK_ARG(value == 0 || value >= 64, MAED_ERR_ARG, "set_option: MAED_OPT_TN_TARGET_WGS must be 0 (heuristic) or >= 64");
    if (key == MAED_OPT_CONV3X3_ROWS_WGS || key == MAED_OPT_STEM_WGRAD_WGS) MAED_CHECK_ARG(value >= 0 && value <= 65535, MAED_ERR_ARG, "set_option: workgroup count out of range");
    if (key == MAED_OPT_LBS_FRAMES) MAED_CHECK_ARG(value == 0 || value == 4 || value == 8 || value == 16, MAED_ERR_ARG, "set_option: MAED_OPT_LBS_FRAMES takes 0 (auto), 4, 8 or 16");
    if (key == MAED_OPT_X3_PLANES) MAED_CHECK_ARG(value == 0 || (value >= 2 && value <= 7 && value != 3), MAED_ERR_ARG, "set_option: MAED_OPT_X3_PLANES takes 0 (fp32 operands) or a kernel variant 2, 4, 5, 6, 7");
    if (key == MAED_OPT_SK) MAED_CHECK_ARG(value >= 0 && value <= 3, MAED_ERR_ARG, "set_option: MAED_OPT_SK takes 0 (off), 1 (heuristic), 2 (no K cuts) or 3 (always)");
    if (key == MAED_OPT_TN_SK) MAED_CHECK_ARG(value == 0 || value == 1, MAED_ERR_ARG, "set_option: MAED_OPT_TN_SK takes 0 or 1");
    if (key == MAED_OPT_SK_GRID) MAED_CHECK_ARG(value >= 0 && value <= 512, MAED_ERR_ARG, "set_option: MAED_OPT_SK_GRID takes 0 (one workgroup per CU) or a workgroup count <= 512");
    g_opt[key].store(value, std::memory_order_relaxed);
    return MAED_OK;
}

extern "C" int maed_get_option(int key) {
    if (key < 0 || key >= MAED_OPT_COUNT) { maed_set_error("get_option: unknown option %d", key); return MAED_ERR_ARG; }
    return g_opt[key].load(std::memory_order_relaxed);
}

int maed_opt(int key) { return g_opt[key].load(std::memory_order_relaxed); }

int maed_x3_planes(void) {
    const int v = maed_opt(MAED_OPT_F32_MATMUL);
    return v == 1 ? 2 : v == 2 ? 3 : 0;
}
```

### maed_amd/ops.py

```python
import ctypes as C
import math
import os
import threading
import weakref

import numpy as _np

import torch

from . import _lib as L
from ._lib import BF16, F32, check

WEIGHT_EPOCH = 0


def bump_weight_epoch():
    global WEIGHT_EPOCH
    WEIGHT_EPOCH += 1


def on_library_device(t):
    return t.is_cuda or (SIM_MODULE_PATHS and L._lib is not None and L._lib.maed_version() < 0)


# ... 51 lines not shown
    if not _SHADOW or t is None or t.dtype != torch.bfloat16:
        return None
    e = _SHADOW.get(t.data_ptr())
    return e[1] if e is not None and e[0].numel() == t.numel() else None


def shadow_clear():
    assert not (_UNFILLED and _SHADOW) or all(k in _SHADOW for k in _UNFILLED), "an unfilled twin lost its shadow"
    for k in list(_UNFILLED):
        e = _SHADOW.get(k)
        if e is not None:
            e[0].copy_(e[1])
    _UNFILLED.clear()
    _SHADOW.clear()


def shadow_keep_only(t16):
    e = _SHADOW.get(t16.data_ptr()) if t16 is not None else None
    for k in list(_UNFILLED):
        if k in _SHADOW:
            _SHADOW[k][0].copy_(_SHADOW[k][1])
    _UNFILLED.clear()
    _SHADOW.clear()
    if e is not None:
        _SHADOW[t16.data_ptr()] = e


def twin_of(y32):
    return shadow_put(y32.to(torch.bfloat16), y32)


_UNFILLED = set()


def twin_later(y32):
    y16 = torch.empty_like(y32, dtype=torch.bfloat16)
    _UNFILLED.add(y16.data_ptr())
    return shadow_put(y16, y32)


def twin_fill(t16):
    if t16 is not None and t16.data_ptr() in _UNFILLED:
        _UNFILLED.discard(t16.data_ptr())
        t16.copy_(shadow_of(t16))


def bwd_twin():
    return _BWD_TWIN[0] and f32_split()


def mm_code(dtype, prec=None):
    if dtype == torch.float32 and prec in ("bf16x3", "bf16x6", "bf16x1"):
        return {"bf16x3": L.F32X3, "bf16x6": L.F32X6, "bf16x1": L.F32X1}[prec]
    return dt_code(dtype)


def dt_code(dtype):
    if dtype == torch.float32:
        return F32
    if dtype == torch.bfloat16:
        return BF16
    raise TypeError(f"maed_amd: unsupported compute dtype {dtype}")


_TLS = threading.local()


def _stream():
    s = getattr(_TLS, "stream", None)
    if s is not None:
        return s
    return torch._C._cuda_getCurrentRawStream(torch._C._cuda_getDevice())


_SIDE_ON = None
_SIDE = {}


def _side_on():
    return (L.get_option(L.OPT_SIDE_STREAM) == 1) if _SIDE_ON is None else _SIDE_ON


def _join_at_end_of_backward(device, st):
    if st[1]:
        return
    try:
        torch.autograd.Variable._execution_engine.queue_callback(lambda: side_stream_join(device))
    except RuntimeError:
        pass


def side_stream_run(fn, *tensors):
    t0 = tensors[0]
    if not (t0.is_cuda and _side_on()):
        return fn()
    st = _SIDE.get(t0.device)
    if st is None:
        st = _SIDE[t0.device] = [torch.cuda.Stream(device=t0.device), False]
    side = st[0]
    raw = side.cuda_stream
    check(L.lib().maed_stream_fence(_stream(), raw), "stream_fence")
    prev = getattr(_TLS, "stream", None)
    _TLS.stream = raw
    try:
        out = fn()
    finally:
        _TLS.stream = prev
    _keep_until_join(t0.device, st, tensors)
    _join_at_end_of_backward(t0.device, st)
    st[1] = True
    return out


def side_stream_handle(device, *tensors):
    if not (device.type == "cuda" and _side_on()):
        return None
    st = _SIDE.get(device)
    if st is None:
        st = _SIDE[device] = [torch.cuda.Stream(device=device), False]
    _keep_until_join(device, st, tensors)
    _join_at_end_of_backward(device, st)
    st[1] = True
    return st[0].cuda_stream


def _keep_until_join(device, st, tensors):
    keep = _KEEP.setdefault(device, [])
    keep.extend(tensors)
    if len(keep) > 4096:
        side_stream_join(device)


_KEEP = {}


def _keep_alive_on_stream(t):
    if getattr(_TLS, "stream", None) is not None:
        _KEEP.setdefault(t.device, []).append(t)


def side_stream_join(device):
    st = _SIDE.get(device)
    if st is not None and st[1]:
        torch.cuda.current_stream(device).wait_stream(st[0])
        st[1] = False
    keep = _KEEP.get(device)
    if keep:
        keep.clear()


def _p(t):
    if t is None:
        return None
    if not t.is_cuda:
        raise L.MaedHipError("maed_amd kernels need CUDA/HIP tensors (no CPU path)")
    return t.data_ptr()


def _c(t):
    return t if t.is_contiguous() else t.contiguous()


_TABLES = {}
_CAPTURE_KEEP = None


def _upload_table(tab, dev):
    host = torch.from_numpy(tab.view(_np.uint8))
    if dev.type != "cuda":
        return host.clone()
    key = (dev, host.numpy().tobytes())
    capturing = torch.cuda.is_current_stream_capturing()
    hit = _TABLES.get(key)
    if hit is not None:
        if capturing and _CAPTURE_KEEP is not None:
            _CAPTURE_KEEP.append(hit)
        return hit
    if capturing:
        raise RuntimeError("maed_amd: a pointer table changed between the eager warm-up steps and the capture (a row points at a per-step temporary)")
    pinned = host.pin_memory()
    out = pinned.to(dev, non_blocking=True)
    if len(_TABLES) >= 64:
        _TABLES.pop(next(iter(_TABLES)))
    _TABLES[key] = out
    return out


def layernorm_fwd(x, gamma, beta, out_dtype, eps=1e-6, row_stride=None, rows=None):
    C_ = x.shape[-1]
    if rows is None:
        x = _c(x)
        rows = x.numel() // C_
        row_stride = C_
    y = torch.empty(rows, C_, dtype=out_dtype, device=x.device)
    mean = torch.empty(rows, dtype=torch.float32, device=x.device)
    rstd = torch.empty_like(mean)
    check(L.lib().maed_layernorm_fwd(_p(x), row_stride, _p(gamma), _p(beta), _p(y), dt_code(out_dtype), _p(mean), _p(rstd),
                                     rows, C_, eps, _stream()), "layernorm_fwd")
    return y, mean, rstd


def layernorm_bwd(dy, x, gamma, mean, rstd, dres=None, dgamma=None, dbeta=None, want_twin=False):
    C_ = x.shape[-1]
    x, dy = _c(x), _c(dy)
    rows = x.numel() // C_
    dx = torch.empty(rows, C_, dtype=torch.float32, device=x.device)
    twin = torch.empty(rows, C_, dtype=dy.dtype, device=x.device) if want_twin else None
    dgamma = torch.zeros(C_, dtype=torch.float32, device=x.device) if dgamma is None else dgamma
    dbeta = torch.zeros(C_, dtype=torch.float32, device=x.device) if dbeta is None else dbeta
    check(L.lib().maed_layernorm_bwd(_p(dy), dt_code(dy.dtype), _p(x), C_, _p(gamma), _p(mean), _p(rstd), _p(dres), _p(dx), _p(twin),
                                     _p(dgamma), _p(dbeta), rows, C_, _stream()), "layernorm_bwd")
    return (dx, dgamma, dbeta, twin) if want_twin else (dx, dgamma, dbeta)


def gemm_tn_wgrad(Y, X, dW=None, dbias=None, prec=None):
    M, N = Y.shape
    K = X.shape[1]
    dW = torch.zeros(N, K, dtype=torch.float32, device=Y.device) if dW is None else dW
    check(L.lib().maed_gemm_tn_wgrad(_p(Y), Y.stride(0), _p(X), X.stride(0), M, N, K, _p(dW), dW.stride(0), _p(dbias), mm_code(Y.dtype, prec), _stream()),
          "gemm_tn_wgrad")
    return dW


def gemm_nt(A, B, epilogue=L.EPI_STORE, bias=None, out=None, out2=None, aux=None, splitk=1, impl=L.IMPL_AUTO, M=None, K=None, prec=None):
    assert A.dim() == 2 and B.dim() == 2 and A.dtype == B.dtype
    M = A.shape[0] if M is None else M
    K = A.shape[1] if K is None else K
    N = B.shape[0]
    assert A.stride(1) == 1 and B.stride(1) == 1
    if out is None:
        odt = torch.float32 if epilogue in (L.EPI_RESID_F32, L.EPI_ATOMIC_F32, L.EPI_STORE_F32) else A.dtype
        out = (torch.zeros if epilogue == L.EPI_ATOMIC_F32 else torch.empty)(M, N, dtype=odt, device=A.device)
    if epilogue == L.EPI_GELU and out2 is None:
        out2 = torch.empty_like(out)
    check(L.lib().maed_gemm_nt(_p(A), A.stride(0), _p(B), B.stride(0), M, N, K, mm_code(A.dtype, prec), epilogue, _p(bias),
                               _p(out), out.stride(0), _p(out2), _p(aux), aux.stride(0) if aux is not None else 0,
                               splitk, impl, _stream()), "gemm_nt")
    return (out, out2) if epilogue == L.EPI_GELU else out


def split_planes(x):
    x = _c(x)
    assert x.dtype == torch.float32 and x.numel() % 8 == 0
    hi, lo = torch.empty_like(x, dtype=torch.bfloat16), torch.empty_like(x, dtype=torch.bfloat16)
    check(L.lib().maed_split_planes(_p(x), _p(hi), _p(lo), x.numel(), _stream()), "split_planes")
    return hi, lo


def gemm_nt_planes(A, B, epilogue=L.EPI_STORE, bias=None, aux=None, want_f32=True, want_planes=False, want_pre=False, variant=0):
    (Ah, Al), (Bh, Bl) = A, B
    assert Ah.dtype == Al.dtype == Bh.dtype == Bl.dtype == torch.bfloat16 and Ah.shape == Al.shape and Bh.shape == Bl.shape
    assert Ah.stride() == Al.stride() and Bh.stride() == Bl.stride() and Ah.stride(1) == 1 and Bh.stride(1) == 1
    M, K = Ah.shape
    N = Bh.shape[0]
    dev = Ah.device
    out = torch.empty(M, N, dtype=torch.float32, device=dev) if want_f32 else None
    oh = torch.empty(M, N, dtype=torch.bfloat16, device=dev) if want_planes else None
    ol = torch.empty(M, N, dtype=torch.bfloat16, device=dev) if want_planes else None
    pre = torch.empty(M, N, dtype=torch.bfloat16, device=dev) if (want_pre and epilogue == L.EPI_GELU) else None
    check(L.lib().maed_gemm_nt_planes(_p(Ah), _p(Al), Ah.stride(0), _p(Bh), _p(Bl), Bh.stride(0), M, N, K, epilogue, _p(bias), _p(out), N, _p(pre), _p(aux),
                                      aux.stride(0) if aux is not None else 0, _p(oh), _p(ol), variant, _stream()), "gemm_nt_planes")
    return out, ((oh, ol) if want_planes else None), pre


def transpose_cast(x, out_dtype, want_t=True, want_c=False, colsum=None, pad_to=64):
    assert x.dim() == 2 and x.stride(1) == 1
    M, N = x.shape
    Mp = (M + pad_to - 1) // pad_to * pad_to
    out_t = torch.empty(N, Mp, dtype=out_dtype, device=x.device) if want_t else None
    out_c = torch.empty(M, N, dtype=out_dtype, device=x.device) if want_c else None
    check(L.lib().maed_transpose_cast(_p(x), dt_code(x.dtype), x.stride(0), M, N, _p(out_t), Mp, _p(out_c), N, _p(colsum),
                                      dt_code(out_dtype), _stream()), "transpose_cast")
    return out_t, out_c


def attn_spatial_fwd(qkv, H, impl=L.IMPL_AUTO):
    F_, P, C3 = qkv.shape
    C_ = C3 // 3
    qkv = _c(qkv)
    o = torch.empty(F_, P, C_, dtype=qkv.dtype, device=qkv.device)
    lse = torch.empty(F_, H, P, dtype=torch.float32, device=qkv.device)
    check(L.lib().maed_attn_spatial_fwd(_p(qkv), _p(o), _p(lse), F_, P, H, 1.0 / math.sqrt(C_ // H), dt_code(qkv.dtype), impl, _stream()),
          "attn_spatial_fwd")
    return o, lse


def attn_spatial_bwd(qkv, o, d_o, lse, H, dqkv=None, accumulate=False, impl=L.IMPL_AUTO):
    F_, P, C3 = qkv.shape
    dqkv = torch.empty_like(qkv) if dqkv is None else dqkv
    check(L.lib().maed_attn_spatial_bwd(_p(_c(qkv)), _p(_c(o)), _p(_c(d_o)), _p(lse), _p(dqkv), int(accumulate), F_, P, H,
                                        1.0 / math.sqrt(C3 // 3 // H), dt_code(qkv.dtype), impl, _stream()), "attn_spatial_bwd")
    return dqkv


def attn_temporal_fwd(qkv, H, T, prec=None):
    F_, P, C3 = qkv.shape
    C_ = C3 // 3
    qkv = _c(qkv)
    o = torch.empty(F_, P, C_, dtype=qkv.dtype, device=qkv.device)
    lse = torch.empty(F_, H, P, dtype=torch.float32, device=qkv.device)
    check(L.lib().maed_attn_temporal_fwd(_p(qkv), _p(o), _p(lse), F_, P, H, T, 1.0 / math.sqrt(C_ // H), mm_code(qkv.dtype, prec), _stream()),
          "attn_temporal_fwd")
    return o, lse


def attn_temporal_bwd(qkv, o, d_o, lse, H, T, dqkv=None, accumulate=False, prec=None):
    F_, P, C3 = qkv.shape
    dqkv = torch.empty_like(qkv) if dqkv is None else dqkv
    check(L.lib().maed_attn_temporal_bwd(_p(_c(qkv)), _p(_c(o)), _p(_c(d_o)), _p(lse), _p(dqkv), int(accumulate), F_, P, H, T,
                                         1.0 / math.sqrt(C3 // 3 // H), mm_code(qkv.dtype, prec), _stream()), "attn_temporal_bwd")
    return dqkv


def st_colmean(x_s, x_t):
    F_, P, C_ = x_s.shape
    means = torch.empty(F_, 2 * C_, dtype=x_s.dtype, device=x_s.device)
    ws = torch.empty(F_, 2 * C_, dtype=torch.float32, device=x_s.device)
    check(L.lib().maed_st_colmean(_p(_c(x_s)), _p(_c(x_t)), _p(means), _p(ws), F_, P, C_, dt_code(x_s.dtype), _stream()), "st_colmean")
    return means


def st_mix_fwd(x_s, x_t, logits):
    F_, P, C_ = x_s.shape
    mix = torch.empty_like(x_s)
    check(L.lib().maed_st_mix_fwd(_p(_c(x_s)), _p(_c(x_t)), _p(_c(logits)), _p(mix), F_, P, C_, dt_code(x_s.dtype), _stream()), "st_mix_fwd")
    return mix


def st_mix_bwd(dmix, x_s, x_t, logits, dmeans_fn):
    F_, P, C_ = x_s.shape
    dlogits = torch.empty(F_, 2 * C_, dtype=x_s.dtype, device=x_s.device)
    ws = torch.empty(F_, 2 * C_, dtype=torch.float32, device=x_s.device)
    check(L.lib().maed_st_mix_bwd_reduce(_p(_c(dmix)), _p(_c(x_s)), _p(_c(x_t)), _p(logits), _p(dlogits), _p(ws), F_, P, C_,
                                         dt_code(x_s.dtype), _stream()), "st_mix_bwd_reduce")
    dmeans = dmeans_fn(dlogits)
    dx_s, dx_t = torch.empty_like(x_s), torch.empty_like(x_t)
    check(L.lib().maed_st_mix_bwd_apply(_p(_c(dmix)), _p(logits), _p(_c(dmeans)), _p(dx_s), _p(dx_t), F_, P, C_, dt_code(x_s.dtype), _stream()),
          "st_mix_bwd_apply")
    return dx_s, dx_t, dlogits


def adam_step(p, g, m, v, shadow, lr, beta1, beta2, eps, wd, step, gscale=1.0):
    bc1 = 1.0 - beta1 ** step
    bc2 = 1.0 - beta2 ** step
    check(L.lib().maed_adam_step(_p(p), _p(g), _p(m), _p(v), _p(shadow), p.numel(), lr, beta1, beta2, eps, wd, bc1, bc2, gscale, _stream()),
          "adam_step")


def adam_step_dev(p, g, m, v, shadow, state, beta1, beta2, eps, wd, gscale=1.0):
    check(L.lib().maed_adam_step_dev(_p(p), _p(g), _p(m), _p(v), _p(shadow), p.numel(), _p(state), beta1, beta2, eps, wd, gscale, _stream()), "adam_step_dev")


class DeviceTrainState:

    def __init__(self, device):
        self.dev = torch.zeros(32, dtype=torch.uint8, device=device)
        self._host = _np.zeros(32, dtype=_np.uint8)
        self.calls = 0

    def set_hyper(self, lr, bias_corr1, bias_corr2):
        self._host[:12].view(_np.float32)[:] = (lr, bias_corr1, bias_corr2)

    def begin_step(self, seed=None):
        self.calls = 0
        if seed is None:
            seed = int(torch.randint(0, 2 ** 62, (1,), dtype=torch.int64).item())
        self._host[16:24].view(_np.uint64)[0] = seed

    def upload(self):
        src = torch.from_numpy(self._host.copy())
        self.dev.copy_(src.pin_memory() if self.dev.is_cuda else src, non_blocking=True)

    def next_call_id(self):
        self.calls += 1
        return self.calls


DEVICE_STATE = None


_WT_DTYPE = _np.dtype([("src", "u8"), ("dst_c", "u8"), ("dst_t", "u8"), ("rows", "i4"), ("cols", "i4"), ("tile0", "i4"), ("tiles_n", "i4")])


class WeightCache:

    _registry = weakref.WeakSet()

    def __init__(self):
        self._key = None
        self._val = None
        self._images = None
        self._weights = None
        self._dtype = None
        WeightCache._registry.add(self)

    @staticmethod
    def _make_key(weights, dtype):
        return (WEIGHT_EPOCH, dtype, tuple((w.data_ptr(), w._version, tuple(w.shape)) for w in weights))

    def get(self, weights, dtype):
        if self._make_key(weights, dtype) != self._key:
            self._weights, self._dtype = list(weights), dtype
            WeightCache._registry.add(self)
            WeightCache._refresh_group(self)
        return self._val

    @classmethod
    def _refresh_group(cls, me):
        dev, dtype = me._weights[0].device, me._dtype
        group = [c for c in cls._registry if c._weights is not None and c._dtype == dtype and c._weights[0].device == dev]
        rows, keep = [], []
        tile0 = 0
        with torch.no_grad():
            for c in group:
                ok = c._images is not None and len(c._images) == len(c._weights) and all(
                    im[1].shape == (w.shape[1], w.shape[0]) and im[1].dtype == dtype and im[1].device == dev for im, w in zip(c._images, c._weights))
                if not ok:
                    c._images = [(None if dtype == torch.float32 else torch.empty(w.shape, dtype=dtype, device=dev),
                                  torch.empty(w.shape[1], w.shape[0], dtype=dtype, device=dev)) for w in c._weights]
                val = []
                for w, (wc, wt) in zip(c._weights, c._images):
                    src = _c(w.detach())
                    keep.append(src)
                    R, Cn = src.shape
                    tn = (Cn + 63) // 64
                    rows.append((_p(src), 0 if wc is None else _p(wc), _p(wt), R, Cn, tile0, tn))
                    tile0 += ((R + 63) // 64) * tn
                    val.append((src if dtype == torch.float32 else wc, wt))
                c._val = val
        for lo in range(0, len(rows), 256):
            chunk = rows[lo:lo + 256]
            base = chunk[0][5]
            tab = _np.array([r[:5] + (r[5] - base, r[6]) for r in chunk], dtype=_WT_DTYPE)
            ntiles = (chunk[-1][5] - base) + ((chunk[-1][3] + 63) // 64) * chunk[-1][6]
            tab_dev = _upload_table(tab, dev)
            check(L.lib().maed_weight_refresh(_p(tab_dev), len(chunk), ntiles, dt_code(dtype), _stream()), "weight_refresh")
        for c in group:
            c._key = cls._make_key(c._weights, dtype)


_SCRATCH = {}


def _aligned_bytes(nbytes, device, align=256):
    buf = torch.empty(nbytes + align, dtype=torch.uint8, device=device)
    off = (-buf.data_ptr()) % align
    return buf[off:off + nbytes]


def twin_join():
    check(L.lib().maed_ste_block_twin_join(_stream()), "ste_block_twin_join")


def _scratch(nbytes, device, tag=None):
    key = (device.index, _stream(), tag)
    buf = _SCRATCH.get(key)
    if buf is None or buf.numel() < nbytes:
        if buf is not None and isinstance(tag, tuple) and tag and tag[0] == "twin":
            twin_join()
        buf = _aligned_bytes(nbytes, device)
        _SCRATCH[key] = buf
    return buf


class LinearFn(torch.autograd.Function):

    @staticmethod
    def forward(ctx, x, weight, bias, cache, direct_w=None, direct_b=None):
        (wc, wt), = cache.get([weight], x.dtype)
        ctx.save_for_backward(x, weight, bias)
        ctx.wt = wt
        ctx.direct = None
        if direct_w is not None and LinearFn._grad_at_apply and any(ctx.needs_input_grad[1:3]):
            ctx.direct = (direct_w, direct_b)
            direct_grad_begin(direct_w, direct_b)
        x32 = shadow_of(x)
        if x32 is not None:
            return gemm_nt(_c(x32), _c(weight.detach()), L.EPI_STORE, bias=bias)
        return gemm_nt(_c(x), wc, L.EPI_STORE, bias=bias)

    @staticmethod
    def backward(ctx, dy):
        x, weight, bias = ctx.saved_tensors
        dy = _c(dy if dy.dtype == x.dtype else dy.to(x.dtype))
        if lib_matmul_dtype(dy.dtype) and weight.shape[0] % 8 == 0 and weight.shape[1] % 8 == 0:
            if ctx.direct is not None:
                gw, gb = direct_grad_slot(ctx.direct[0]), direct_grad_slot(ctx.direct[1])
                if gw is not None and (bias is None or gb is not None):
                    gemm_tn_wgrad(dy, x, dW=gw.view(weight.shape), dbias=gb)
                    dx = gemm_nt(dy, ctx.wt, L.EPI_STORE) if ctx.needs_input_grad[0] else None
                    direct_grad_done(*ctx.direct)
                    return dx, None, None, None, None, None
                direct_grad_cancel(*ctx.direct)
            db = torch.zeros_like(bias) if bias is not None else None
            dW = gemm_tn_wgrad(dy, x, dbias=db)
            dx = gemm_nt(dy, ctx.wt, L.EPI_STORE) if ctx.needs_input_grad[0] else None
            return dx, dW, db, None, None, None
        if ctx.direct is not None:
            direct_grad_cancel(*ctx.direct)
        db = torch.zeros_like(bias) if bias is not None else None
        dyt, _ = transpose_cast(dy, dy.dtype, colsum=db)
        xt, _ = transpose_cast(x, x.dtype)
        tiles = max(1, (weight.shape[0] // 128) * (weight.shape[1] // 128))
        dW = gemm_nt(dyt, xt, L.EPI_ATOMIC_F32, splitk=max(1, min(dyt.shape[1] // 256, 1024 // tiles)))
        dx = gemm_nt(dy, ctx.wt, L.EPI_STORE) if ctx.needs_input_grad[0] else None
        return dx, dW, db, None, None, None

    _grad_at_apply = True

    @classmethod
    def apply(cls, *args):
        LinearFn._grad_at_apply = torch.is_grad_enabled()
        return super().apply(*args)


class EmbedAddFn(torch.autograd.Function):

    @staticmethod
    def forward(ctx, patch, cls, pos, temp, T):
        F_, Pm1, C_ = patch.shape
        tok = torch.empty(F_, Pm1 + 1, C_, dtype=torch.float32, device=patch.device)
        check(L.lib().maed_embed_add_fwd(_p(_c(patch)), dt_code(patch.dtype), _p(_c(cls)), _p(_c(pos)), _p(_c(temp)), _p(tok),
                                         F_, Pm1 + 1, C_, T, _stream()), "embed_add_fwd")
        ctx.T, ctx.pdtype = T, patch.dtype
        ctx.temp_shape = temp.shape
        return tok

    @staticmethod
    def backward(ctx, dtok):
        dtok = _c(dtok)
        F_, P, C_ = dtok.shape
        dpatch = torch.empty(F_, P - 1, C_, dtype=ctx.pdtype, device=dtok.device)
        dpos = torch.zeros(1, P, C_, dtype=torch.float32, device=dtok.device)
        dtemp = torch.zeros(ctx.temp_shape, dtype=torch.float32, device=dtok.device)
        check(L.lib().maed_embed_add_bwd(_p(dtok), _p(dpatch), dt_code(ctx.pdtype), _p(dpos), _p(dtemp), F_, P, C_, ctx.T, _stream()), "embed_add_bwd")
        dcls = dpos[:, :1].clone()
        return dpatch, dcls, dpos, dtemp, None



_TWIN = [None, None, None]
TWIN_HITS = [0, 0]
_TWIN_WARNED = [False]


DIRECT_GRADS = os.environ.get("MAED_DIRECT_GRADS", "1") == "1"


def direct_grad_slot(p):
    if not DIRECT_GRADS or p is None or not p.is_leaf:
        return None
    g = p.grad
    if g is None or g.dtype != torch.float32 or g.shape != p.shape or g.device != p.device or not g.is_contiguous():
        return None
    return g


def direct_grad_begin(*params):
    for p in params:
        if p is not None:
            p._maed_direct = getattr(p, "_maed_direct", 0) + 1


def direct_grad_cancel(*params):
    for p in params:
        if p is not None:
            p._maed_direct = max(getattr(p, "_maed_direct", 1) - 1, 0)


def direct_grad_done(*params):
    for p in params:
        if p is None:
            continue
        n = getattr(p, "_maed_direct", 1) - 1
        p._maed_direct = max(n, 0)
        hook = getattr(p, "_maed_ready", None)
        if n <= 0 and hook is not None:
            hook(p)


class ReportingFn(torch.autograd.Function):
    _grad_mode_at_apply = True

    @classmethod
    def apply(cls, *args):
        ReportingFn._grad_mode_at_apply = torch.is_grad_enabled()
        return super().apply(*args)

    @staticmethod
    def will_run_backward(ctx):
        return ReportingFn._grad_mode_at_apply and any(ctx.needs_input_grad)


class STEBlockFn(ReportingFn):

    @staticmethod
    def forward(ctx, x, block, dims, H, T, *params):
        lib = L.lib()
        x = _c(x)
        d = L.BlockDims(*dims)
        y = torch.empty_like(x)
        twin = block.compute_dtype == torch.float32 and bwd_twin() and ReportingFn.will_run_backward(ctx) and dims[7] != L.IMPL_VALU and dims[2] % 8 == 0 and dims[5] % 8 == 0
        if twin:
            dims = dims[:6] + (BF16,) + dims[7:]
            d16 = L.BlockDims(*dims)
            pr = block._c_params_masters()
# ... 598 lines not shown
```

Baseline: 416.0.

## Merge spatial and temporal attention forward into one persistent-grid launch

Adds a single kernel that runs spatial (long) attention and temporal attention forward in one grid. Groups of workgroups are assigned to either task, and the block forward uses it by default when shapes allow, replacing the side-stream overlap of two kernels. A merged dq/dkv backward kernel is also added but stays off unless the option is set to 2. The aim is fewer launches and better CU fill by co-scheduling the two attention types, at the cost of a shared LDS budget sized to the larger of the two and a lower occupancy bound on the temporal part.

```diff
diff --git a/include/maed_hip.h b/include/maed_hip.h
--- a/include/maed_hip.h
+++ b/include/maed_hip.h
@@ -63,6 +63,7 @@
     MAED_OPT_TN_SK = 15,
     MAED_OPT_CONV3X3_NARROW_WGS = 16,
     MAED_OPT_CONV3X3_FRAME = 17,
+    MAED_OPT_ATTN_MERGE = 18,
     MAED_OPT_COUNT
 } maed_option;
 int maed_init(int device);
@@ -107,6 +108,9 @@
 int maed_attn_temporal_bwd(const void* qkv, const void* o, const void* d_o, const float* lse,
                            void* dqkv, int accumulate, int F, int P, int H, int T, float scale,
                            int dtype, void* stream);
+
+int maed_attn_st_fwd(const void* qkv, void* xs, float* lse_s, void* xt, float* lse_t, int F, int P, int H, int T,
+                     float scale, int dtype, void* stream);
 
 int maed_st_colmean(const void* x_s, const void* x_t, void* means, float* ws, int F, int P, int C, int dtype, void* stream);
 int maed_st_mix_fwd(const void* x_s, const void* x_t, const float* logits, void* mix,
diff --git a/maed_amd/_lib.py b/maed_amd/_lib.py
--- a/maed_amd/_lib.py
+++ b/maed_amd/_lib.py
@@ -13,7 +13,7 @@
 IMPL_MFMA_SK = 10
 IMPL_X3, IMPL_X6, IMPL_X1 = 7, 8, 9
 (OPT_F32_MATMUL, OPT_SIDE_STREAM, OPT_TN_TARGET_WGS, OPT_ABLATE, OPT_GN_BWD_ONEPASS, OPT_F32_BWD_X1, OPT_ST_FUSED, OPT_CONV3X3_ROWS_WGS, OPT_STEM_WGRAD_WGS,
- OPT_LBS_FRAMES, OPT_TN_DMA, OPT_X3_PLANES, OPT_X3_PLANES_LN, OPT_SK, OPT_SK_GRID, OPT_TN_SK, OPT_CONV3X3_NARROW_WGS, OPT_CONV3X3_FRAME) = range(18)
+ OPT_LBS_FRAMES, OPT_TN_DMA, OPT_X3_PLANES, OPT_X3_PLANES_LN, OPT_SK, OPT_SK_GRID, OPT_TN_SK, OPT_CONV3X3_NARROW_WGS, OPT_CONV3X3_FRAME, OPT_ATTN_MERGE) = range(19)
 
 vp, i64, i32, f32 = C.c_void_p, C.c_int64, C.c_int, C.c_float
 
@@ -70,6 +70,7 @@
     "maed_attn_spatial_fwd": (i32, [vp, vp, vp, i32, i32, i32, f32, i32, i32, vp]),
     "maed_attn_spatial_bwd": (i32, [vp, vp, vp, vp, vp, i32, i32, i32, i32, f32, i32, i32, vp]),
     "maed_attn_temporal_fwd": (i32, [vp, vp, vp, i32, i32, i32, i32, f32, i32, vp]),
+    "maed_attn_st_fwd": (i32, [vp, vp, vp, vp, vp, i32, i32, i32, i32, f32, i32, vp]),
     "maed_attn_temporal_bwd": (i32, [vp, vp, vp, vp, vp, i32, i32, i32, i32, i32, f32, i32, vp]),
     "maed_st_colmean": (i32, [vp, vp, vp, vp, i32, i32, i32, i32, vp]),
     "maed_st_mix_fwd": (i32, [vp, vp, vp, vp, i32, i32, i32, i32, vp]),
@@ -204,6 +205,7 @@
     OPT_CONV3X3_FRAME: int(os.environ.get("MAED_CONV3X3_FRAME", "1")),
     OPT_CONV3X3_NARROW_WGS: int(os.environ.get("MAED_CONV3X3_NARROW_WGS", "0")),
     OPT_TN_SK: int(os.environ.get("MAED_TN_SK", "1")),
+    OPT_ATTN_MERGE: int(os.environ.get("MAED_ATTN_MERGE", "1")),
     OPT_X3_PLANES_LN: int(os.environ.get("MAED_X3_PLANES_LN", "0")),
 }
 
diff --git a/maed_amd/csrc/attn_long.hip b/maed_amd/csrc/attn_long.hip
--- a/maed_amd/csrc/attn_long.hip
+++ b/maed_amd/csrc/attn_long.hip
@@ -1,4 +1,5 @@
 #include "attn_mfma.cuh"
+#include "attn_tm_fwd.cuh"
 
 #define D HEAD_DIM
 
@@ -41,11 +42,10 @@
     tile_store1(t.b, rows, tr, tid + 256);
 }
 
-__global__ __launch_bounds__(256, 4) void attn_long_fwd_mfma(const bf16* __restrict__ qkv, bf16* __restrict__ o, float* __restrict__ lse,
-                                                          int L, int H, int ntile, float scale_log2e) {
-    __shared__ __attribute__((aligned(16))) unsigned short Ks[LT * KLD];
-    __shared__ __attribute__((aligned(16))) unsigned short Vs[LT * KLD];
-    const int bid = long_xcd_remap(blockIdx.x, gridDim.x);
+__device__ __forceinline__ void attn_long_fwd_body(unsigned short* Ks, unsigned short* Vs , int wg, int nwg,
+                                                   const bf16* __restrict__ qkv, bf16* __restrict__ o, float* __restrict__ lse,
+                                                   int L, int H, int ntile, float scale_log2e) {
+    const int bid = long_xcd_remap(wg, nwg);
     const int item = bid / ntile, tile = bid - item * ntile;
     const int f = item / H, h = item - f * H, C = H * D;
     const int64_t ld = 3 * (int64_t)C;
@@ -128,13 +128,18 @@
         if (hi == 0) lse[((int64_t)f * H + h) * L + q] = (m + log2f(l)) * 0.69314718055994530942f;
     }
 }
-
-__global__ __launch_bounds__(256, 3) void attn_long_bwd_dq_mfma(const bf16* __restrict__ qkv, const bf16* __restrict__ o, const bf16* __restrict__ d_o,
-                                                             const float* __restrict__ lse, bf16* __restrict__ dqkv, int accumulate, int L, int H,
-                                                             int ntile, float scale) {
+__global__ __launch_bounds__(256, 4) void attn_long_fwd_mfma(const bf16* __restrict__ qkv, bf16* __restrict__ o, float* __restrict__ lse,
+                                                          int L, int H, int ntile, float scale_log2e) {
     __shared__ __attribute__((aligned(16))) unsigned short Ks[LT * KLD];
     __shared__ __attribute__((aligned(16))) unsigned short Vs[LT * KLD];
-    const int bid = long_xcd_remap(blockIdx.x, gridDim.x);
+    attn_long_fwd_body(Ks, Vs, blockIdx.x, gridDim.x, qkv, o, lse, L, H, ntile, scale_log2e);
+}
+
+__device__ __forceinline__ void attn_long_bwd_dq_body(unsigned short* Ks, unsigned short* Vs, int wg, int nwg,
+                                                      const bf16* __restrict__ qkv, const bf16* __restrict__ o, const bf16* __restrict__ d_o,
+                                                      const float* __restrict__ lse, bf16* __restrict__ dqkv, int accumulate, int L, int H,
+                                                      int ntile, float scale) {
+    const int bid = long_xcd_remap(wg, nwg);
     const int item = bid / ntile, tile = bid - item * ntile;
     const int f = item / H, h = item - f * H, C = H * D;
     const int64_t ld = 3 * (int64_t)C;
@@ -209,14 +214,19 @@
     __syncthreads();
     if (active) store_tile_lines((wave < 2 ? Ks : Vs) + (wave & 1) * 2048, dqkv + ((int64_t)f * L + q0) * ld + h * D, ld, L - q0, dq, lane, accumulate);
 }
-
-__global__ __launch_bounds__(256, 2) void attn_long_bwd_dkv_mfma(const bf16* __restrict__ qkv, const bf16* __restrict__ o, const bf16* __restrict__ d_o,
-                                                              const float* __restrict__ lse, bf16* __restrict__ dqkv, int accumulate, int L, int H,
-                                                              int ntile, float scale) {
-    __shared__ __attribute__((aligned(16))) unsigned short Qs[LT * KLD];
-    __shared__ __attribute__((aligned(16))) unsigned short dOs[LT * KLD];
-    __shared__ float Ls[LT], Ds[LT];
-    const int bid = long_xcd_remap(blockIdx.x, gridDim.x);
+__global__ __launch_bounds__(256, 3) void attn_long_bwd_dq_mfma(const bf16* __restrict__ qkv, const bf16* __restrict__ o, const bf16* __restrict__ d_o,
+                                                             const float* __restrict__ lse, bf16* __restrict__ dqkv, int accumulate, int L, int H,
+                                                             int ntile, float scale) {
+    __shared__ __attribute__((aligned(16))) unsigned short Ks[LT * KLD];
+    __shared__ __attribute__((aligned(16))) unsigned short Vs[LT * KLD];
+    attn_long_bwd_dq_body(Ks, Vs, blockIdx.x, gridDim.x, qkv, o, d_o, lse, dqkv, accumulate, L, H, ntile, scale);
+}
+
+__device__ __forceinline__ void attn_long_bwd_dkv_body(unsigned short* Qs, unsigned short* dOs, float* Ls, float* Ds, int wg, int nwg,
+                                                       const bf16* __restrict__ qkv, const bf16* __restrict__ o, const bf16* __restrict__ d_o,
+                                                       const float* __restrict__ lse, bf16* __restrict__ dqkv, int accumulate, int L, int H,
+                                                       int ntile, float scale) {
+    const int bid = long_xcd_remap(wg, nwg);
     const int item = bid / ntile, tile = bid - item * ntile;
     const int f = item / H, h = item - f * H, C = H * D;
     const int64_t ld = 3 * (int64_t)C;
@@ -320,6 +330,47 @@
         bf16* drow0 = dqkv + ((int64_t)f * L + k0w) * ld + h * D;
         store_tile_lines(patch, drow0 + C, ld, L - k0w, dk, lane, accumulate);
         store_tile_lines(patch, drow0 + 2 * C, ld, L - k0w, dv, lane, accumulate);
+    }
+}
+__global__ __launch_bounds__(256, 2) void attn_long_bwd_dkv_mfma(const bf16* __restrict__ qkv, const bf16* __restrict__ o, const bf16* __restrict__ d_o,
+                                                              const float* __restrict__ lse, bf16* __restrict__ dqkv, int accumulate, int L, int H,
+                                                              int ntile, float scale) {
+    __shared__ __attribute__((aligned(16))) unsigned short Qs[LT * KLD];
+    __shared__ __attribute__((aligned(16))) unsigned short dOs[LT * KLD];
+    __shared__ float Ls[LT], Ds[LT];
+    attn_long_bwd_dkv_body(Qs, dOs, Ls, Ds, blockIdx.x, gridDim.x, qkv, o, d_o, lse, dqkv, accumulate, L, H, ntile, scale);
+}
+
+__global__ __launch_bounds__(256, 2) void attn_long_bwd_merged(const bf16* __restrict__ qkv, const bf16* __restrict__ o, const bf16* __restrict__ d_o,
+                                                                  const float* __restrict__ lse, bf16* __restrict__ dqkv, int accumulate, int L, int H,
+                                                                  int ntile, int nwg, float scale) {
+    __shared__ __attribute__((aligned(16))) unsigned short A[LT * KLD];
+    __shared__ __attribute__((aligned(16))) unsigned short B[LT * KLD];
+    __shared__ float Ls[LT], Ds[LT];
+    const int g = blockIdx.x >> 3, wg = (g >> 1) * 8 + (blockIdx.x & 7);
+    if (wg >= nwg) return;
+    if (g & 1) attn_long_bwd_dkv_body(A, B, Ls, Ds, wg, nwg, qkv, o, d_o, lse, dqkv, accumulate, L, H, ntile, scale);
+    else attn_long_bwd_dq_body(A, B, wg, nwg, qkv, o, d_o, lse, dqkv, accumulate, L, H, ntile, scale);
+}
+
+constexpr int TM_SLICE = 32 * 64 + HEAD_DIM * (32 + 4);
+constexpr int ST_LDS = (4 * TM_SLICE > 2 * LT * KLD) ? 4 * TM_SLICE : 2 * LT * KLD;
+__global__ __launch_bounds__(256, 4) void attn_st_fwd_mfma(const bf16* __restrict__ qkv, bf16* __restrict__ xs, float* __restrict__ lse_s, bf16* __restrict__ xt,
+                                                           float* __restrict__ lse_t, int P, int H, int ntile, int Tn, int G, int ngroups, int ns, int ntm,
+                                                           unsigned ntg, float scale_log2e) {
+    __shared__ __attribute__((aligned(16))) unsigned short smem[ST_LDS];
+    const unsigned g = blockIdx.x >> 3, slot = blockIdx.x & 7, gt = gridDim.x >> 3;
+    const unsigned t0 = g * ntg / gt, t1 = (g + 1) * ntg / gt;
+    if (t1 > t0) {
+        const int tb = (int)(t0 * 8 + slot), wave = threadIdx.x >> 6;
+        if (tb * 4 >= ntm) return;
+        const int vb = tb * 4 + wave;
+        const bool live = vb < ntm;
+        attn_tm_fwd_mfma_body(smem + wave * TM_SLICE, threadIdx.x & 63, 64, live ? vb : 0, live, qkv, xt, lse_t, P, H, Tn, G, ngroups, scale_log2e);
+    } else {
+        const int wg = (int)((g - t0) * 8 + slot);
+        if (wg >= ns) return;
+        attn_long_fwd_body(smem, smem + LT * KLD, wg, ns, qkv, xs, lse_s, P, H, ntile, scale_log2e);
     }
 }
 
@@ -505,10 +556,28 @@
     return MAED_OK;
 }
 
+int maed_attn_long_bwd_merged_launch(const void* qkv, const void* o, const void* d_o, const float* lse, void* dqkv, int accumulate, int F, int L, int H,
+                                     float scale, hipStream_t s) {
+    const int ntile = (L + WG_ROWS - 1) / WG_ROWS;
+    const int64_t nwg = (int64_t)F * H * ntile;
+    MAED_CHECK_ARG(2 * 8 * ((nwg + 7) / 8) < (1ll << 31), MAED_ERR_SHAPE, "attn_long_bwd(merged): grid too large");
+    if (nwg == 0) return MAED_OK;
+    const dim3 grid((unsigned)(2 * 8 * ((nwg + 7) / 8)));
+    hipLaunchKernelGGL(attn_long_bwd_merged, grid, dim3(256), 0, s, (const bf16*)qkv, (const bf16*)o, (const bf16*)d_o, lse, (bf16*)dqkv, accumulate,
+                       L, H, ntile, (int)nwg, scale);
+    MAED_CHECK_LAUNCH("attn_long_bwd(merged)");
+    return MAED_OK;
+}
+
+static const bool kBwdMergeDefault = false;
 int maed_attn_long_bwd_launch(const void* qkv, const void* o, const void* d_o, const float* lse, void* dqkv, int accumulate, int F, int L, int H,
                               float scale, hipStream_t s) {
     const int ntile = (L + WG_ROWS - 1) / WG_ROWS;
     MAED_CHECK_ARG((int64_t)F * H * ntile < (1ll << 31), MAED_ERR_SHAPE, "attn_long_bwd: grid too large");
+    {
+        const int opt = maed_opt(MAED_OPT_ATTN_MERGE);
+        if (opt == 2 || (opt == 1 && kBwdMergeDefault)) return maed_attn_long_bwd_merged_launch(qkv, o, d_o, lse, dqkv, accumulate, F, L, H, scale, s);
+    }
     const dim3 grid((unsigned)(F * H * ntile));
     hipLaunchKernelGGL(attn_long_bwd_dq_mfma, grid, dim3(256), 0, s, (const bf16*)qkv, (const bf16*)o, (const bf16*)d_o, lse, (bf16*)dqkv, accumulate,
                        L, H, ntile, scale);
@@ -539,3 +608,29 @@
     MAED_CHECK_LAUNCH("attn_long_bwd(valu)");
     return MAED_OK;
 }
+
+bool maed_attn_st_fwd_merged_ok(int F, int P, int H, int T, int dtype) {
+    if (dtype != MAED_BF16 || T <= 0 || T > 32 || F <= 0 || F % T != 0 || !maed_opt(MAED_OPT_ATTN_MERGE)) return false;
+    const int G = 32 / T;
+    const int64_t ns = (int64_t)F * H * ((P + WG_ROWS - 1) / WG_ROWS), ntm = (int64_t)(F / T) * H * ((P + G - 1) / G);
+    return (ns + 7) / 8 + ((ntm + 3) / 4 + 7) / 8 <= 65535;
+}
+
+extern "C" int maed_attn_st_fwd(const void* qkv, void* xs, float* lse_s, void* xt, float* lse_t, int F, int P, int H, int T, float scale, int dtype,
+                                void* stream) {
+    MAED_CHECK_ARG(qkv && xs && lse_s && xt && lse_t, MAED_ERR_ARG, "attn_st_fwd: null pointer");
+    MAED_CHECK_ARG(T > 0 && F >= 0 && F % T == 0 && P > 0 && H > 0, MAED_ERR_SHAPE, "attn_st_fwd: F=%d must be a multiple of T=%d", F, T);
+    MAED_CHECK_ARG(is_aligned(qkv, 16) && is_aligned(xs, 16) && is_aligned(xt, 16), MAED_ERR_ALIGN, "attn_st_fwd: qkv/xs/xt must be 16-B aligned");
+    if (F == 0) return MAED_OK;
+    if (!maed_attn_st_fwd_merged_ok(F, P, H, T, dtype)) {
+        MAED_PROPAGATE(maed_attn_temporal_fwd(qkv, xt, lse_t, F, P, H, T, scale, dtype, stream));
+        return maed_attn_spatial_fwd(qkv, xs, lse_s, F, P, H, scale, dtype, MAED_IMPL_AUTO, stream);
+    }
+    const int ntile = (P + WG_ROWS - 1) / WG_ROWS, G = 32 / T, ngroups = (P + G - 1) / G;
+    const int ns = F * H * ntile, ntm = (F / T) * H * ngroups;
+    const unsigned nsg = (unsigned)((ns + 7) / 8), ntg = (unsigned)(((ntm + 3) / 4 + 7) / 8);
+    hipLaunchKernelGGL(attn_st_fwd_mfma, dim3(8 * (nsg + ntg)), dim3(256), 0, (hipStream_t)stream, (const bf16*)qkv, (bf16*)xs, lse_s, (bf16*)xt, lse_t, P, H,
+                       ntile, T, G, ngroups, ns, ntm, ntg, scale * 1.44269504088896340736f);
+    MAED_CHECK_LAUNCH("attn_st_fwd");
+    return MAED_OK;
+}
diff --git a/maed_amd/csrc/attn_temporal.hip b/maed_amd/csrc/attn_temporal.hip
--- a/maed_amd/csrc/attn_temporal.hip
+++ b/maed_amd/csrc/attn_temporal.hip
@@ -1,5 +1,6 @@
 #include "common.cuh"
 #include "attn_mfma.cuh"
+#include "attn_tm_fwd.cuh"
 #include "gemm_x3.h"
 #include <stdlib.h>
 
@@ -322,128 +323,7 @@
 __global__ __launch_bounds__(1024) void attn_tm_fwd_mfma(const bf16* __restrict__ qkv, bf16* __restrict__ o, float* __restrict__ lse,
                                                          int P, int H, int Tn, int G, int ngroups, float scale_log2e) {
     MAED_DYN_SHARED(unsigned short, smem);
-    const int L = G * Tn, Lk = (L + 31) & ~31, VLD = Lk + 4;
-    unsigned short* Ks = smem;
-    unsigned short* Vt = smem + (size_t)Lk * 64;
-    const int C = H * D;
-    const int64_t ld = 3 * (int64_t)C;
-    const int tid = threadIdx.x, nthr = blockDim.x;
-    const int lane = tid & 63, wave = tid >> 6, l31 = lane & 31, hi = lane >> 5;
-    int bid = blockIdx.x;
-    const int tg = bid % ngroups; bid /= ngroups;
-    const int h = bid % H, n = bid / H;
-    const int p0 = tg * G;
-#define TM_ROW_OK(r) ((r) < L && p0 + (r) / Tn < P)
-#define TM_ROW_OFF(r) ((((int64_t)n * Tn + (r) % Tn) * P + p0 + (r) / Tn) * ld + h * D)
-    const int q = wave * 32 + l31;
-    const bool q_ok = TM_ROW_OK(q);
-    const int qg = q / Tn;
-    bf16x8_t qf[4];
-    {
-        const int qc = q_ok ? q : 0;
-        const bf16* qp = qkv + TM_ROW_OFF(qc);
-#pragma unroll
-        for (int t = 0; t < 4; ++t) qf[t] = *reinterpret_cast<const bf16x8_t*>(qp + t * 16 + hi * 8);
-    }
-    for (int idx = tid; idx < Lk * 8; idx += nthr) {
-        const int r = idx >> 3, c8 = (idx & 7) * 8;
-        uint4 kv = make_uint4(0u, 0u, 0u, 0u), vv = kv;
-        if (TM_ROW_OK(r)) {
-            const bf16* rp = qkv + TM_ROW_OFF(r);
-            kv = *reinterpret_cast<const uint4*>(rp + C + c8);
-            vv = *reinterpret_cast<const uint4*>(rp + 2 * C + c8);
-        }
-        *reinterpret_cast<uint4*>(Ks + r * 64 + (((c8 >> 3) ^ ((r >> 1) & 7)) << 3)) = kv;
-        const uint32_t w[4] = {vv.x, vv.y, vv.z, vv.w};
-#pragma unroll
-        for (int j = 0; j < 4; ++j) {
-            Vt[(c8 + 2 * j) * VLD + r] = (unsigned short)(w[j] & 0xffffu);
-            Vt[(c8 + 2 * j + 1) * VLD + r] = (unsigned short)(w[j] >> 16);
-        }
-    }
-    for (int i = tid; i < D * 4; i += nthr) Vt[(i >> 2) * VLD + Lk + (i & 3)] = 0;
-    __syncthreads();
-
-    f32x16_t oacc[2];
-#pragma unroll
-    for (int r = 0; r < 16; ++r) { oacc[0][r] = 0.f; oacc[1][r] = 0.f; }
-    float m = -INFINITY, l = 0.f;
-    const int nkt = Lk / 32;
-    for (int kt = 0; kt < nkt; ++kt) {
-        f32x16_t s;
-#pragma unroll
-        for (int r = 0; r < 16; ++r) s[r] = 0.f;
-        const int krow = kt * 32 + l31;
-        const unsigned short* kp = Ks + krow * 64;
-        const int swz = (krow >> 1) & 7;
-#pragma unroll
-        for (int t = 0; t < 4; ++t) {
-            const bf16x8_t kf = *reinterpret_cast<const bf16x8_t*>(kp + (((2 * t + hi) ^ swz) << 3));
-            s = __builtin_amdgcn_mfma_f32_32x32x16_bf16(kf, qf[t], s, 0, 0, 0);
-        }
-        bool any = false;
-#pragma unroll
-        for (int r = 0; r < 16; ++r) {
-            const int k = kt * 32 + (r & 3) + 8 * (r >> 2) + 4 * hi;
-            const bool ok = TM_ROW_OK(k) && (k / Tn == qg);
-            s[r] = ok ? s[r] : -INFINITY;
-            any |= ok;
-        }
-        float mt = s[0];
-#pragma unroll
-        for (int r = 1; r < 16; ++r) mt = fmaxf(mt, s[r]);
-        mt = fmaxf(mt, __shfl_xor(mt, 32, 64)) * scale_log2e;
-        const float mn = fmaxf(m, mt);
-        const float msafe = (mn == -INFINITY) ? 0.f : mn;
-        const float alpha = (m == -INFINITY) ? 0.f : __builtin_amdgcn_exp2f(m - msafe);
-        float ps = 0.f;
-#pragma unroll
-        for (int r = 0; r < 16; ++r) { s[r] = __builtin_amdgcn_exp2f(fmaf(s[r], scale_log2e, -msafe)); ps += s[r]; }
-        l = l * alpha + ps;
-        m = mn;
-#pragma unroll
-        for (int r = 0; r < 16; ++r) { oacc[0][r] *= alpha; oacc[1][r] *= alpha; }
-#pragma unroll
-        for (int st = 0; st < 2; ++st) {
-            union { bf16x8_t v; uint32_t u[4]; } pf;
-#pragma unroll
-            for (int j = 0; j < 4; ++j) pf.u[j] = pack_bf2(s[8 * st + 2 * j], s[8 * st + 2 * j + 1]);
-#pragma unroll
-            for (int et = 0; et < 2; ++et) {
-                const unsigned short* vp = Vt + (et * 32 + l31) * VLD + kt * 32 + 16 * st + 4 * hi;
-                union { bf16x8_t v; uint2 u[2]; } vf;
-                vf.u[0] = *reinterpret_cast<const uint2*>(vp);
-                vf.u[1] = *reinterpret_cast<const uint2*>(vp + 8);
-                oacc[et] = __builtin_amdgcn_mfma_f32_32x32x16_bf16(vf.v, pf.v, oacc[et], 0, 0, 0);
-            }
-        }
-        (void)any;
-    }
-    l += __shfl_xor(l, 32, 64);
-    if (Lk == 32) {
-        const float inv = q_ok ? 1.f / l : 0.f;
-#pragma unroll
-        for (int r = 0; r < 16; ++r) { oacc[0][r] *= inv; oacc[1][r] *= inv; }
-        store_tile_lines_at(Ks, [&](int r) -> bf16* { return TM_ROW_OK(r) ? o + (((int64_t)n * Tn + r % Tn) * P + p0 + r / Tn) * C + h * D : nullptr; }, oacc, lane, 0);
-        if (q_ok && hi == 0) lse[(((int64_t)n * Tn + q % Tn) * H + h) * P + p0 + qg] = (m + log2f(l)) * 0.69314718055994530942f;
-    } else if (q_ok) {
-        const float inv = 1.f / l;
-        const int t = q % Tn, p = p0 + qg;
-        const int64_t f = (int64_t)n * Tn + t;
-        bf16* orow = o + (f * P + p) * C + h * D;
-#pragma unroll
-        for (int et = 0; et < 2; ++et)
-#pragma unroll
-            for (int g = 0; g < 4; ++g) {
-                const int e0 = et * 32 + 8 * g + 4 * hi;
-                const uint2 w = make_uint2(pack_bf2(oacc[et][4 * g] * inv, oacc[et][4 * g + 1] * inv),
-                                           pack_bf2(oacc[et][4 * g + 2] * inv, oacc[et][4 * g + 3] * inv));
-                *reinterpret_cast<uint2*>(orow + e0) = w;
-            }
-        if (hi == 0) lse[(f * H + h) * P + p] = (m + log2f(l)) * 0.69314718055994530942f;
-    }
-#undef TM_ROW_OK
-#undef TM_ROW_OFF
+    attn_tm_fwd_mfma_body(smem, threadIdx.x, blockDim.x, blockIdx.x, true, qkv, o, lse, P, H, Tn, G, ngroups, scale_log2e);
 }
 
 template <int MAX_THREADS, int MIN_BLOCKS>
diff --git a/maed_amd/csrc/attn_tm_fwd.cuh b/maed_amd/csrc/attn_tm_fwd.cuh
--- /dev/null
+++ b/maed_amd/csrc/attn_tm_fwd.cuh
@@ -0,0 +1,127 @@
+#pragma once
+#include "attn_mfma.cuh"
+
+__device__ __forceinline__ void attn_tm_fwd_mfma_body(unsigned short* smem, const int tid, const int nthr, int bid, const bool live,
+                                                      const bf16* __restrict__ qkv, bf16* __restrict__ o, float* __restrict__ lse,
+                                                      int P, int H, int Tn, int G, int ngroups, float scale_log2e) {
+    const int L = G * Tn, Lk = (L + 31) & ~31, VLD = Lk + 4;
+    unsigned short* Ks = smem;
+    unsigned short* Vt = smem + (size_t)Lk * 64;
+    const int C = H * HEAD_DIM;
+    const int64_t ld = 3 * (int64_t)C;
+    const int lane = tid & 63, wave = tid >> 6, l31 = lane & 31, hi = lane >> 5;
+    const int tg = bid % ngroups; bid /= ngroups;
+    const int h = bid % H, n = bid / H;
+    const int p0 = tg * G;
+#define TM_ROW_OK(r) (live && (r) < L && p0 + (r) / Tn < P)
+#define TM_ROW_OFF(r) ((((int64_t)n * Tn + (r) % Tn) * P + p0 + (r) / Tn) * ld + h * HEAD_DIM)
+    const int q = wave * 32 + l31;
+    const bool q_ok = TM_ROW_OK(q);
+    const int qg = q / Tn;
+    bf16x8_t qf[4];
+    {
+        const int qc = q_ok ? q : 0;
+        const bf16* qp = qkv + TM_ROW_OFF(qc);
+#pragma unroll
+        for (int t = 0; t < 4; ++t) qf[t] = *reinterpret_cast<const bf16x8_t*>(qp + t * 16 + hi * 8);
+    }
+    for (int idx = tid; idx < Lk * 8; idx += nthr) {
+        const int r = idx >> 3, c8 = (idx & 7) * 8;
+        uint4 kv = make_uint4(0u, 0u, 0u, 0u), vv = kv;
+        if (TM_ROW_OK(r)) {
+            const bf16* rp = qkv + TM_ROW_OFF(r);
+            kv = *reinterpret_cast<const uint4*>(rp + C + c8);
+            vv = *reinterpret_cast<const uint4*>(rp + 2 * C + c8);
+        }
+        *reinterpret_cast<uint4*>(Ks + r * 64 + (((c8 >> 3) ^ ((r >> 1) & 7)) << 3)) = kv;
+        const uint32_t w[4] = {vv.x, vv.y, vv.z, vv.w};
+#pragma unroll
+        for (int j = 0; j < 4; ++j) {
+            Vt[(c8 + 2 * j) * VLD + r] = (unsigned short)(w[j] & 0xffffu);
+            Vt[(c8 + 2 * j + 1) * VLD + r] = (unsigned short)(w[j] >> 16);
+        }
+    }
+    for (int i = tid; i < HEAD_DIM * 4; i += nthr) Vt[(i >> 2) * VLD + Lk + (i & 3)] = 0;
+    __syncthreads();
+
+    f32x16_t oacc[2];
+#pragma unroll
+    for (int r = 0; r < 16; ++r) { oacc[0][r] = 0.f; oacc[1][r] = 0.f; }
+    float m = -INFINITY, l = 0.f;
+    const int nkt = Lk / 32;
+    for (int kt = 0; kt < nkt; ++kt) {
+        f32x16_t s;
+#pragma unroll
+        for (int r = 0; r < 16; ++r) s[r] = 0.f;
+        const int krow = kt * 32 + l31;
+        const unsigned short* kp = Ks + krow * 64;
+        const int swz = (krow >> 1) & 7;
+#pragma unroll
+        for (int t = 0; t < 4; ++t) {
+            const bf16x8_t kf = *reinterpret_cast<const bf16x8_t*>(kp + (((2 * t + hi) ^ swz) << 3));
+            s = __builtin_amdgcn_mfma_f32_32x32x16_bf16(kf, qf[t], s, 0, 0, 0);
+        }
+        bool any = false;
+#pragma unroll
+        for (int r = 0; r < 16; ++r) {
+            const int k = kt * 32 + (r & 3) + 8 * (r >> 2) + 4 * hi;
+            const bool ok = TM_ROW_OK(k) && (k / Tn == qg);
+            s[r] = ok ? s[r] : -INFINITY;
+            any |= ok;
+        }
+        float mt = s[0];
+#pragma unroll
+        for (int r = 1; r < 16; ++r) mt = fmaxf(mt, s[r]);
+        mt = fmaxf(mt, __shfl_xor(mt, 32, 64)) * scale_log2e;
+        const float mn = fmaxf(m, mt);
+        const float msafe = (mn == -INFINITY) ? 0.f : mn;
+        const float alpha = (m == -INFINITY) ? 0.f : __builtin_amdgcn_exp2f(m - msafe);
+        float ps = 0.f;
+#pragma unroll
+        for (int r = 0; r < 16; ++r) { s[r] = __builtin_amdgcn_exp2f(fmaf(s[r], scale_log2e, -msafe)); ps += s[r]; }
+        l = l * alpha + ps;
+        m = mn;
+#pragma unroll
+        for (int r = 0; r < 16; ++r) { oacc[0][r] *= alpha; oacc[1][r] *= alpha; }
+#pragma unroll
+        for (int st = 0; st < 2; ++st) {
+            union { bf16x8_t v; uint32_t u[4]; } pf;
+#pragma unroll
+            for (int j = 0; j < 4; ++j) pf.u[j] = pack_bf2(s[8 * st + 2 * j], s[8 * st + 2 * j + 1]);
+#pragma unroll
+            for (int et = 0; et < 2; ++et) {
+                const unsigned short* vp = Vt + (et * 32 + l31) * VLD + kt * 32 + 16 * st + 4 * hi;
+                union { bf16x8_t v; uint2 u[2]; } vf;
+                vf.u[0] = *reinterpret_cast<const uint2*>(vp);
+                vf.u[1] = *reinterpret_cast<const uint2*>(vp + 8);
+                oacc[et] = __builtin_amdgcn_mfma_f32_32x32x16_bf16(vf.v, pf.v, oacc[et], 0, 0, 0);
+            }
+        }
+        (void)any;
+    }
+    l += __shfl_xor(l, 32, 64);
+    if (Lk == 32) {
+        const float inv = q_ok ? 1.f / l : 0.f;
+#pragma unroll
+        for (int r = 0; r < 16; ++r) { oacc[0][r] *= inv; oacc[1][r] *= inv; }
+        store_tile_lines_at(Ks, [&](int r) -> bf16* { return TM_ROW_OK(r) ? o + (((int64_t)n * Tn + r % Tn) * P + p0 + r / Tn) * C + h * HEAD_DIM : nullptr; }, oacc, lane, 0);
+        if (q_ok && hi == 0) lse[(((int64_t)n * Tn + q % Tn) * H + h) * P + p0 + qg] = (m + log2f(l)) * 0.69314718055994530942f;
+    } else if (q_ok) {
+        const float inv = 1.f / l;
+        const int t = q % Tn, p = p0 + qg;
+        const int64_t f = (int64_t)n * Tn + t;
+        bf16* orow = o + (f * P + p) * C + h * HEAD_DIM;
+#pragma unroll
+        for (int et = 0; et < 2; ++et)
+#pragma unroll
+            for (int g = 0; g < 4; ++g) {
+                const int e0 = et * 32 + 8 * g + 4 * hi;
+                const uint2 w = make_uint2(pack_bf2(oacc[et][4 * g] * inv, oacc[et][4 * g + 1] * inv),
+                                           pack_bf2(oacc[et][4 * g + 2] * inv, oacc[et][4 * g + 3] * inv));
+                *reinterpret_cast<uint2*>(orow + e0) = w;
+            }
+        if (hi == 0) lse[(f * H + h) * P + p] = (m + log2f(l)) * 0.69314718055994530942f;
+    }
+#undef TM_ROW_OK
+#undef TM_ROW_OFF
+}
diff --git a/maed_amd/csrc/block.hip b/maed_amd/csrc/block.hip
--- a/maed_amd/csrc/block.hip
+++ b/maed_amd/csrc/block.hip
@@ -182,6 +182,7 @@
                          uint32_t* sync, float* ex, int F, int P, int C, int dtype, bool clear_sync, uint32_t arrive_base, void* stream);
 int maed_st_fused_bwd_ws(const void* dmix, const void* x_s, const void* x_t, const float* logits, const void* wt_ts, void* dlogits, void* dx_s,
                          void* dx_t, uint32_t* sync, float* ex, int F, int P, int C, int dtype, bool clear_sync, uint32_t arrive_base, void* stream);
+bool maed_attn_st_fwd_merged_ok(int F, int P, int H, int T, int dtype);
 namespace {
 
 int check_dims(const maed_block_dims* d, const char* who) {
@@ -260,7 +261,9 @@
                                          piggy ? (uint32_t*)(B.st_sync) : nullptr, piggy ? d->F * 16 : 0, stream));
     PROF(PROF_GEMM_QKV, maed_gemm_nt_twin(B.ln1, C, p->w_qkv, C, M, 3 * C, C, dt, MAED_EPI_STORE, p->b_qkv, B.qkv, 3 * C, nullptr, nullptr, 0, 1, gi, stream, B.tw_qkv, false, nullptr));
     }
-    {
+    if (d->impl == MAED_IMPL_AUTO && maed_attn_st_fwd_merged_ok(d->F, d->P, d->H, d->T, dt)) {
+        PROF(PROF_ATTN_SP_FWD, maed_attn_st_fwd(B.qkv, B.xs, (float*)(B.lse_s), B.xt, (float*)(B.lse_t), d->F, d->P, d->H, d->T, scale, dt, stream));
+    } else {
         SideStream* ss = (d->impl != MAED_IMPL_VALU && (dt == MAED_BF16 || maed_x3_planes())) ? side_stream() : nullptr;
         void* tst = ss ? (void*)ss->s : stream;
         if (ss) ss->fence((hipStream_t)stream, ss->s);
diff --git a/maed_amd/csrc/options.hip b/maed_amd/csrc/options.hip
--- a/maed_amd/csrc/options.hip
+++ b/maed_amd/csrc/options.hip
@@ -21,6 +21,7 @@
     {0},
     {1},
     {0},
+    {1},
     {1},
 };
 
@@ -93,6 +94,7 @@
     if (key == MAED_OPT_SK) MAED_CHECK_ARG(value >= 0 && value <= 3, MAED_ERR_ARG, "set_option: MAED_OPT_SK takes 0 (off), 1 (heuristic), 2 (no K cuts) or 3 (always)");
     if (key == MAED_OPT_TN_SK) MAED_CHECK_ARG(value == 0 || value == 1, MAED_ERR_ARG, "set_option: MAED_OPT_TN_SK takes 0 or 1");
     if (key == MAED_OPT_SK_GRID) MAED_CHECK_ARG(value >= 0 && value <= 512, MAED_ERR_ARG, "set_option: MAED_OPT_SK_GRID takes 0 (one workgroup per CU) or a workgroup count <= 512");
+    if (key == MAED_OPT_ATTN_MERGE) MAED_CHECK_ARG(value >= 0 && value <= 2, MAED_ERR_ARG, "set_option: MAED_OPT_ATTN_MERGE takes 0 (off), 1 (default) or 2 (merged wherever the shape allows)");
     g_opt[key].store(value, std::memory_order_relaxed);
     return MAED_OK;
 }
diff --git a/maed_amd/ops.py b/maed_amd/ops.py
--- a/maed_amd/ops.py
+++ b/maed_amd/ops.py
@@ -377,6 +377,17 @@
     check(L.lib().maed_attn_temporal_fwd(_p(qkv), _p(o), _p(lse), F_, P, H, T, 1.0 / math.sqrt(C_ // H), mm_code(qkv.dtype, prec), _stream()),
           "attn_temporal_fwd")
     return o, lse
+
+
+def attn_st_fwd(qkv, H, T):
+    F_, P, C3 = qkv.shape
+    C_ = C3 // 3
+    qkv = _c(qkv)
+    xs, xt = (torch.empty(F_, P, C_, dtype=qkv.dtype, device=qkv.device) for _ in range(2))
+    lse_s, lse_t = (torch.empty(F_, H, P, dtype=torch.float32, device=qkv.device) for _ in range(2))
+    check(L.lib().maed_attn_st_fwd(_p(qkv), _p(xs), _p(lse_s), _p(xt), _p(lse_t), F_, P, H, T, 1.0 / math.sqrt(C_ // H), dt_code(qkv.dtype), _stream()),
+          "attn_st_fwd")
+    return xs, lse_s, xt, lse_t
 
 
 def attn_temporal_bwd(qkv, o, d_o, lse, H, T, dqkv=None, accumulate=False, prec=None):
```

After: 418.7, median of 6. About the same (+0.6%).
